# gonewest818/raytrace-clj

Measured on AMD Instinct MI355X. Metric: Msamples/sec (nx*ny*ns), higher is better.
Workload: dtype f64; 1 GPU; C3: 1920x1080x256spp Shirley cover scene n=50 (10001 spheres), depth 50, thin-lens camera, seeded counter RNG; accel=bvh; 8x8 tiles dealt round-robin to 1 GPU(s); nx=1920, ny=1080, ns=256, spheres=10001, depth=50, accel=bvh, accel_ran=bvh, frames_in_flight=1, launch_form=one GPU

## Files before the change

### include/rtmi.h

```cpp
#ifndef RTMI_H
#define RTMI_H

#include <stdint.h>

#ifdef __cplusplus
extern "C" {
#endif

#define RTMI_OK 0
#define RTMI_E_ARG (-1)
#define RTMI_E_DEVICE (-2)
#define RTMI_E_UNSUPPORTED (-3)
#define RTMI_E_NOMEM (-4)
#define RTMI_E_STATE (-5)

enum { RTMI_PRIM_SPHERE = 0, RTMI_PRIM_UVSPHERE = 1, RTMI_PRIM_MOVING = 2,
       RTMI_PRIM_RECT_XY = 3, RTMI_PRIM_RECT_XZ = 4, RTMI_PRIM_RECT_YZ = 5, RTMI_PRIM_TRIANGLE = 6,
       RTMI_PRIM_MEDIUM = 7, RTMI_PRIM_BOUNDARY = 16 };
enum { RTMI_XFORM_TRANSLATE = 0, RTMI_XFORM_ROTATE_Y = 1 };
enum { RTMI_MAT_LAMBERTIAN = 0, RTMI_MAT_METAL = 1, RTMI_MAT_DIELECTRIC = 2, RTMI_MAT_DIFFUSE_LIGHT = 3,
       RTMI_MAT_ISOTROPIC = 4  };
enum { RTMI_TEX_CONSTANT = 0, RTMI_TEX_UVGRADIENT = 1, RTMI_TEX_CHECKER = 2,
       RTMI_TEX_PERLIN_NOISE = 3, RTMI_TEX_PERLIN_TURB = 4, RTMI_TEX_MARBLE = 5, RTMI_TEX_FLIP_U = 6, RTMI_TEX_FLIP_V = 7,
       RTMI_TEX_IMAGE = 8 };
// ... 174 lines not shown
                         const double *rays, const uint64_t *keys, uint64_t seed, uint32_t ctr0, int32_t depth,
                         int32_t n_lights, const int32_t *light_prims,
                         double *state, double *out_mean, double *out_stderr, double *out_rays, uint64_t *out_counters);
int rtmi_render_rays_nee_device(rtmi_scene *scene, int32_t precision, int32_t n_groups, int32_t group, int32_t g_first,
                                const void *d_rays, const void *d_keys, uint64_t seed, uint32_t ctr0, int32_t depth,
                                int32_t n_lights, const int32_t *light_prims,
                                void *d_state, void *d_out_mean, void *d_out_stderr, void *d_out_rays, void *d_out_counters, void *stream);
int rtmi_probe_paths_nee(rtmi_scene *scene, int32_t precision, int32_t n, const double *rays, const uint64_t *keys, uint64_t ctr0, int32_t depth,
                         int32_t n_lights, const int32_t *light_prims, double *out_rgb, uint64_t *out_nseg, int32_t *out_dropped,
                         double *log, int32_t max_seg, int32_t *out_nlog);

#define RTMI_MIS_REC 28
int rtmi_render_rays_mis(rtmi_scene *scene, int32_t precision, int32_t n_groups, int32_t group, int32_t g_first,
                         const double *rays, const uint64_t *keys, uint64_t seed, uint32_t ctr0, int32_t depth,
                         int32_t n_lights, const int32_t *light_prims, int32_t light_choice,
                         double *state, double *out_mean, double *out_stderr, double *out_rays, uint64_t *out_counters);
int rtmi_render_rays_mis_device(rtmi_scene *scene, int32_t precision, int32_t n_groups, int32_t group, int32_t g_first,
                                const void *d_rays, const void *d_keys, uint64_t seed, uint32_t ctr0, int32_t depth,
                                int32_t n_lights, const int32_t *light_prims, int32_t light_choice,
                                void *d_state, void *d_out_mean, void *d_out_stderr, void *d_out_rays, void *d_out_counters, void *stream);
int rtmi_probe_paths_mis(rtmi_scene *scene, int32_t precision, int32_t n, const double *rays, const uint64_t *keys, uint64_t ctr0, int32_t depth,
                         int32_t n_lights, const int32_t *light_prims, int32_t light_choice, double *out_rgb, uint64_t *out_nseg, double *out_weight,
                         double *log, int32_t max_seg, int32_t *out_nlog);

int rtmi_assemble_device(rtmi_ctx *ctx, int32_t nx, int32_t ny, int32_t world, int32_t tiles_per_rank,
                         const void *d_gathered, void *d_out_linear, void *d_out_rgb8, void *stream);

#define RTMI_PROG_REC 5
int rtmi_render_adaptive_tiles_device(rtmi_scene *scene, int32_t nx, int32_t ny, int32_t s_first, int32_t s_count,
                                      int32_t retire, double eps, int32_t depth, uint64_t seed, int32_t precision,
                                      int32_t tile_first, int32_t tile_stride, void *d_tiles_rec, void *d_out_counters, void *stream);
int rtmi_assemble_progressive_device(rtmi_ctx *ctx, int32_t nx, int32_t ny, int32_t world, int32_t tiles_per_rank,
                                     const void *d_gathered_rec, void *d_out_linear, void *d_out_rgb8, void *d_out_stderr, void *d_out_samples, void *stream);

int rtmi_scene_clone(rtmi_scene *scene, rtmi_ctx *ctx, rtmi_scene **out_scene);
int rtmi_render_multi(int32_t n, rtmi_scene *const *scenes, int32_t nx, int32_t ny, int32_t ns, int32_t depth, uint64_t seed,
                      int32_t precision, double *out_linear, uint8_t *out_rgb8, uint64_t *out_counters);
int rtmi_render_multi_device(int32_t n, rtmi_scene *const *scenes, int32_t nx, int32_t ny, int32_t ns, int32_t depth, uint64_t seed,
                             int32_t precision, void *d_out_linear, void *d_out_rgb8, void *d_out_counters);
int rtmi_render_multi_adaptive(int32_t n, rtmi_scene *const *scenes, int32_t nx, int32_t ny, int32_t s_first, int32_t s_count,
                               int32_t retire, double eps, int32_t depth, uint64_t seed, int32_t precision,
                               double *out_linear, uint8_t *out_rgb8, double *out_stderr, int32_t *out_samples, uint64_t *out_counters);
int rtmi_render_multi_adaptive_device(int32_t n, rtmi_scene *const *scenes, int32_t nx, int32_t ny, int32_t s_first, int32_t s_count,
                                      int32_t retire, double eps, int32_t depth, uint64_t seed, int32_t precision,
                                      void *d_out_linear, void *d_out_rgb8, void *d_out_stderr, void *d_out_samples, void *d_out_counters);
enum { RTMI_GATHER_NONE = 0,
       RTMI_GATHER_SAME_DEVICE = 1,
       RTMI_GATHER_PEER_COPY = 2,
       RTMI_GATHER_RCCL = 3 };
int rtmi_last_gather_path(rtmi_ctx *ctx0, int32_t *path);
int rtmi_rccl_probe(const char *soname);
int rtmi_stream_idle(rtmi_ctx *ctx, int32_t *idle);
int rtmi_last_passes(rtmi_ctx *ctx, int32_t *passes);
int rtmi_last_accel(rtmi_ctx *ctx, int32_t *accel);
int rtmi_last_gather_ms(rtmi_ctx *ctx0, double *ms);

int rtmi_last_traversal_counters(rtmi_ctx *ctx, uint64_t *out_aabb_tests, uint64_t *out_prim_tests);

int rtmi_last_trace_ms(rtmi_ctx *ctx, double *ms, int32_t *launches);
int rtmi_last_reduce_ms(rtmi_ctx *ctx, double *ms, int32_t *launches);

int rtmi_probe_hit(rtmi_scene *scene, int32_t precision, int32_t n, const double *rays, double t_min, double t_max, double *out);
int rtmi_probe_paths(rtmi_scene *scene, int32_t precision, int32_t n, const double *rays, const uint64_t *keys, uint64_t ctr0,
                     int32_t depth, double *out_rgb, uint64_t *out_nseg, double *log, int32_t max_seg, int32_t *out_nlog);
int rtmi_probe_camera(rtmi_scene *scene, int32_t precision, int32_t n, const double *uv, const uint64_t *keys, double *out);
int rtmi_probe_texture(rtmi_scene *scene, int32_t precision, int32_t tex, int32_t n, const double *uvp, double *out);
int rtmi_probe_scatter(rtmi_scene *scene, int32_t precision, int32_t mat, int32_t n, const double *rays, const double *hits,
                       const uint64_t *keys, double *out);
int rtmi_probe_rng(rtmi_ctx *ctx, int32_t precision, uint64_t key, uint64_t d0, int32_t n, uint64_t *out_bits, double *out_real);
uint64_t rtmi_sample_key(uint64_t seed, uint64_t pixel, uint64_t sample);
int rtmi_probe_arith(rtmi_ctx *ctx, int32_t n, const double *abc, double *out);
#define RTMI_PROBE_MATH_SLOTS 12
int rtmi_probe_math2(rtmi_ctx *ctx, int32_t n, const double *abc, double tmin, double tmax, int32_t n_slots, double *out);
int rtmi_probe_math(rtmi_ctx *ctx, int32_t n, const double *abc, double tmin, double tmax, double *out);

int rtmi_test_build_tree(int32_t n, const double *geom, const double *cam, int32_t threads, uint64_t *out_hash, int32_t *out_info, double *out_ms);
int rtmi_test_camera_fixed(int32_t cam_kind, const double *cam);
int rtmi_test_half_outward(double x, int32_t up);
int rtmi_test_pack_materials(int32_t n_prims, const int32_t *prim_kind, const double *prim_geom, const int32_t *prim_mat,
                             int32_t n_mats, const int32_t *mat_kind, const int32_t *mat_tex, const double *mat_param,
                             int32_t n_tex, const int32_t *tex_kind, const double *tex_param, const int32_t *tex_child,
                             int32_t cam_kind, const double *cam, const int32_t *prim_flip, const int32_t *prim_xform,
                             int32_t n_xforms, const int32_t *xform_kind, const double *xform_param, int32_t through_creation,
                             uint64_t *out_hash, int32_t *out_facts);
int rtmi_test_pack_geometry(int32_t n_prims, const int32_t *prim_kind, const double *prim_geom, const int32_t *prim_mat,
                            int32_t n_mats, const int32_t *mat_kind, const int32_t *mat_tex, const double *mat_param,
                            int32_t n_tex, const int32_t *tex_kind, const double *tex_param, const int32_t *tex_child,
                            int32_t cam_kind, const double *cam, const int32_t *prim_flip, const int32_t *prim_xform,
                            int32_t n_xforms, const int32_t *xform_kind, const double *xform_param, int32_t through_creation, uint64_t *out_hash);
int rtmi_test_refit(int32_t n_prims, const int32_t *prim_kind, const int32_t *prim_flip, const int32_t *prim_xform, int32_t n_xforms, const int32_t *xform_kind,
                    int32_t cam_kind, const double *cam, int32_t n_steps, const double *geoms, const double *xforms,
                    void *out_nodes, int64_t capacity, int64_t *out_bytes, int32_t *out_info, int32_t *out_big,
                    int32_t *out_cells, int64_t cells_capacity, void *out_leaf_box);
int rtmi_test_refit_half(double x, int32_t up);
int rtmi_test_scene_nodes(rtmi_scene *scene, void *buf, int64_t capacity, int64_t *out_bytes);
int rtmi_test_stage_layout(int32_t n, const uint64_t *elem_bytes, const uint64_t *counts, const int32_t *present, uint64_t *out_offsets, uint64_t *out_total);

#ifdef __cplusplus
}
#endif
#endif
```

### raytrace_clj_amd/_ffi.py

```python
import ctypes as C
import os

import numpy as np

try:
    import torch
except ImportError:
    torch = None

_HERE = os.path.dirname(os.path.abspath(__file__))
LIB_PATH = os.environ.get("RTMI_LIB") or os.path.join(_HERE, "lib", "librtmi.so")

SYMBOLS = [
    "rtmi_last_error", "rtmi_backend_name", "rtmi_version", "rtmi_init", "rtmi_shutdown", "rtmi_set_option",
    "rtmi_device_info", "rtmi_scene_create", "rtmi_scene_create_ex", "rtmi_scene_set_perlin", "rtmi_scene_set_images", "rtmi_scene_set_media_calls", "rtmi_scene_set_media_mode", "rtmi_scene_set_media_calls_narrowed", "rtmi_scene_device_bytes", "rtmi_scene_destroy", "rtmi_render", "rtmi_render_device",
    "rtmi_render_tiles_device", "rtmi_local_tiles", "rtmi_assemble_device", "rtmi_last_trace_ms", "rtmi_last_reduce_ms", "rtmi_probe_hit",
    "rtmi_probe_paths", "rtmi_probe_camera", "rtmi_probe_texture", "rtmi_probe_scatter", "rtmi_probe_rng",
    "rtmi_sample_key", "rtmi_test_half_outward", "rtmi_test_camera_fixed", "rtmi_test_build_tree", "rtmi_probe_arith", "rtmi_probe_math", "rtmi_probe_math2", "rtmi_last_traversal_counters",
    "rtmi_scene_clone", "rtmi_render_multi", "rtmi_render_multi_device", "rtmi_last_gather_ms",
    "rtmi_last_gather_path", "rtmi_rccl_probe", "rtmi_stream_idle", "rtmi_last_passes", "rtmi_last_accel",
    "rtmi_render_progressive", "rtmi_render_progressive_device", "rtmi_progressive_samples", "rtmi_progressive_release",
    "rtmi_render_adaptive", "rtmi_render_adaptive_device", "rtmi_adaptive_status", "rtmi_adaptive_active_tiles",
    "rtmi_render_features", "rtmi_render_features_device", "rtmi_denoise", "rtmi_denoise_device",
    "rtmi_adaptive_retire", "rtmi_adaptive_retire_device",
    "rtmi_render_adaptive_tiles_device", "rtmi_assemble_progressive_device", "rtmi_render_multi_adaptive", "rtmi_render_multi_adaptive_device",
    "rtmi_scene_set_camera", "rtmi_scene_set_camera_stream", "rtmi_scene_camera",
    "rtmi_reproject", "rtmi_reproject_device",
    "rtmi_scene_tree_info",
    "rtmi_scene_set_materials", "rtmi_scene_set_materials_stream", "rtmi_test_pack_materials",
    "rtmi_scene_set_geometry", "rtmi_scene_last_refit_ms", "rtmi_test_pack_geometry", "rtmi_test_refit", "rtmi_test_refit_half", "rtmi_test_scene_nodes",
    "rtmi_render_rays", "rtmi_render_rays_device",
    "rtmi_test_stage_layout",
    "rtmi_query_hits", "rtmi_query_hits_device", "rtmi_query_occluded", "rtmi_query_occluded_device",
    "rtmi_occlusion_hemisphere", "rtmi_occlusion_hemisphere_device", "rtmi_occlusion_targets", "rtmi_occlusion_targets_device",
    "rtmi_ambient_occlusion", "rtmi_ambient_occlusion_device",
    "rtmi_scene_lights", "rtmi_test_scene_lights", "rtmi_direct_irradiance", "rtmi_direct_irradiance_device", "rtmi_render_direct", "rtmi_render_direct_device",
    "rtmi_render_rays_nee", "rtmi_render_rays_nee_device", "rtmi_probe_paths_nee",
    "rtmi_render_rays_mis", "rtmi_render_rays_mis_device", "rtmi_probe_paths_mis",
]

F64, F32 = 0, 1
ACCEL_FLAT, ACCEL_BVH = 0, 1
FLAG_TIMING = 1
GATHER_PATHS = {0: "none", 1: "same-device", 2: "peer-copy", 3: "rccl"}
SEG_REC = 12
TILE = 8
PROG_REC = 5
FEATURES = 8
HIT_REC = 12
RAYS_REC = 10
DIRECT_REC = 4
NEE_REC = 24
MIS_REC = 28
DIRECT_MAX_LIGHTS = 32
EDIT_STREAM_MAX_BYTES = 32768


class RtmiError(RuntimeError):
    def __init__(self, code, msg):
        super().__init__("rtmi error %d: %s" % (code, msg))
        self.code = code


_lib = None


def lib():
    global _lib
    if _lib is not None:
        return _lib
    if not os.path.exists(LIB_PATH):
        raise RtmiError(-2, "HIP extension %s is missing; build it with `make -C raytrace_clj_amd/csrc` "
                            "(there is no CPU fallback)" % LIB_PATH)
    L = C.CDLL(LIB_PATH)
    vp, i32, i64, u64, dbl = C.c_void_p, C.c_int32, C.c_int64, C.c_uint64, C.c_double
    L.rtmi_last_error.restype = C.c_char_p
    L.rtmi_backend_name.restype = C.c_char_p
    L.rtmi_version.restype = C.c_int
    L.rtmi_init.argtypes = [C.c_int, C.c_uint32, C.POINTER(vp)]
    L.rtmi_shutdown.argtypes = [vp]
    L.rtmi_set_option.argtypes = [vp, C.c_char_p, i64]
    L.rtmi_device_info.argtypes = [vp, C.POINTER(i32), C.POINTER(i32), C.POINTER(i64), C.c_char_p, i32]
    L.rtmi_scene_create.argtypes = [vp, i32, vp, vp, vp, i32, vp, vp, vp, i32, vp, vp, vp, i32, vp, C.POINTER(vp)]
    L.rtmi_scene_create_ex.argtypes = [vp, i32, vp, vp, vp, i32, vp, vp, vp, i32, vp, vp, vp, i32, vp, vp, vp, i32, vp, vp, C.POINTER(vp)]
    L.rtmi_scene_set_perlin.argtypes = [vp, vp, vp]
    L.rtmi_scene_set_images.argtypes = [vp, i32, vp, vp]
    L.rtmi_scene_set_media_calls.argtypes = [vp, i32, vp]
    L.rtmi_scene_set_media_mode.argtypes = [vp, i32]
    L.rtmi_scene_set_media_calls_narrowed.argtypes = [vp, i32, vp, vp]
    L.rtmi_scene_device_bytes.argtypes = [vp, C.POINTER(C.c_int64)]
    L.rtmi_scene_destroy.argtypes = [vp]
    L.rtmi_render.argtypes = [vp, i32, i32, i32, i32, u64, i32, i32, i32, i32, i32, vp, vp, vp]
    L.rtmi_render_device.argtypes = [vp, i32, i32, i32, i32, u64, i32, vp, vp, vp, vp]
    L.rtmi_render_tiles_device.argtypes = [vp, i32, i32, i32, i32, u64, i32, i32, i32, vp, vp, vp]
    L.rtmi_local_tiles.argtypes = [i32, i32, i32, i32]
    L.rtmi_local_tiles.restype = i32
    L.rtmi_assemble_device.argtypes = [vp, i32, i32, i32, i32, vp, vp, vp, vp]
    L.rtmi_last_trace_ms.argtypes = [vp, C.POINTER(dbl), C.POINTER(i32)]
    L.rtmi_last_reduce_ms.argtypes = [vp, C.POINTER(dbl), C.POINTER(i32)]
    L.rtmi_probe_hit.argtypes = [vp, i32, i32, vp, dbl, dbl, vp]
    L.rtmi_probe_paths.argtypes = [vp, i32, i32, vp, vp, u64, i32, vp, vp, vp, i32, vp]
    L.rtmi_probe_camera.argtypes = [vp, i32, i32, vp, vp, vp]
    L.rtmi_probe_texture.argtypes = [vp, i32, i32, i32, vp, vp]
    L.rtmi_probe_scatter.argtypes = [vp, i32, i32, i32, vp, vp, vp, vp]
    L.rtmi_probe_rng.argtypes = [vp, i32, u64, u64, i32, vp, vp]
    L.rtmi_sample_key.argtypes = [u64, u64, u64]
    L.rtmi_sample_key.restype = u64
    L.rtmi_probe_arith.argtypes = [vp, i32, vp, vp]
    L.rtmi_test_build_tree.argtypes = [i32, vp, vp, i32, vp, vp, vp]
    L.rtmi_test_half_outward.argtypes = [C.c_double, i32]
    L.rtmi_test_camera_fixed.argtypes = [i32, vp]
    L.rtmi_probe_math.argtypes = [vp, i32, vp, C.c_double, C.c_double, vp]
    L.rtmi_probe_math2.argtypes = [vp, i32, vp, C.c_double, C.c_double, i32, vp]
    L.rtmi_last_traversal_counters.argtypes = [vp, C.POINTER(u64), C.POINTER(u64)]
    L.rtmi_scene_clone.argtypes = [vp, vp, C.POINTER(vp)]
    L.rtmi_render_multi.argtypes = [i32, C.POINTER(vp), i32, i32, i32, i32, u64, i32, vp, vp, vp]
    L.rtmi_render_multi_device.argtypes = [i32, C.POINTER(vp), i32, i32, i32, i32, u64, i32, vp, vp, vp]
    L.rtmi_last_gather_ms.argtypes = [vp, C.POINTER(dbl)]
    L.rtmi_last_gather_path.argtypes = [vp, C.POINTER(i32)]
    L.rtmi_rccl_probe.argtypes = [C.c_char_p]
    L.rtmi_stream_idle.argtypes = [vp, C.POINTER(i32)]
    L.rtmi_last_passes.argtypes = [vp, C.POINTER(i32)]
    L.rtmi_last_accel.argtypes = [vp, C.POINTER(i32)]
    L.rtmi_render_progressive.argtypes = [vp, i32, i32, i32, i32, i32, u64, i32, i32, i32, i32, i32, vp, vp, vp, vp]
    L.rtmi_render_progressive_device.argtypes = [vp, i32, i32, i32, i32, i32, u64, i32, vp, vp, vp, vp, vp]
    L.rtmi_progressive_samples.argtypes = [vp, C.POINTER(i32)]
    L.rtmi_progressive_release.argtypes = [vp]
    L.rtmi_render_adaptive.argtypes = [vp, i32, i32, i32, i32, dbl, i32, u64, i32, i32, i32, i32, i32, vp, vp, vp, vp, vp]
    L.rtmi_render_adaptive_device.argtypes = [vp, i32, i32, i32, i32, dbl, i32, u64, i32, vp, vp, vp, vp, vp, vp]
    L.rtmi_adaptive_status.argtypes = [vp, C.POINTER(i32), C.POINTER(i32), C.POINTER(i64)]
    L.rtmi_adaptive_active_tiles.argtypes = [vp, i32, vp, C.POINTER(i32)]
    L.rtmi_adaptive_retire.argtypes = [vp, i32, i32, vp, dbl, C.POINTER(i32)]
    L.rtmi_adaptive_retire_device.argtypes = [vp, i32, i32, vp, dbl, C.POINTER(i32), vp]
    L.rtmi_render_features.argtypes =[vp, i32, i32, i32, u64, i32, i32, i32, i32, i32, vp, vp]
    L.rtmi_render_features_device.argtypes = [vp, i32, i32, i32, u64, i32, vp, vp, vp]
    L.rtmi_denoise.argtypes = [vp, i32, i32, vp, vp, vp, i32, dbl, dbl, dbl, dbl, vp, vp, vp]
    L.rtmi_denoise_device.argtypes = [vp, i32, i32, vp, vp, vp, i32, dbl, dbl, dbl, dbl, vp, vp, vp, vp]
    L.rtmi_render_adaptive_tiles_device.argtypes = [vp, i32, i32, i32, i32, i32, dbl, i32, u64, i32, i32, i32, vp, vp, vp]
    L.rtmi_assemble_progressive_device.argtypes = [vp, i32, i32, i32, i32, vp, vp, vp, vp, vp, vp]
    L.rtmi_render_multi_adaptive.argtypes = [i32, C.POINTER(vp), i32, i32, i32, i32, i32, dbl, i32, u64, i32, vp, vp, vp, vp, vp]
    L.rtmi_render_multi_adaptive_device.argtypes = [i32, C.POINTER(vp), i32, i32, i32, i32, i32, dbl, i32, u64, i32, vp, vp, vp, vp, vp]
    L.rtmi_scene_set_camera.argtypes = [vp, i32, vp, C.POINTER(i32)]
    L.rtmi_scene_set_camera_stream.argtypes = [vp, i32, vp, vp]
    L.rtmi_scene_camera.argtypes = [vp, C.POINTER(i32), vp, C.POINTER(dbl), C.POINTER(dbl)]
    L.rtmi_scene_tree_info.argtypes = [vp, vp]
    L.rtmi_scene_set_materials.argtypes = [vp, i32, vp, vp, vp, i32, vp, vp, vp, vp, C.POINTER(i32)]
    L.rtmi_scene_set_materials_stream.argtypes = [vp, i32, vp, vp, vp, i32, vp, vp, vp, vp, vp]
    L.rtmi_test_pack_materials.argtypes = [i32, vp, vp, vp, i32, vp, vp, vp, i32, vp, vp, vp, i32, vp, vp, vp, i32, vp, vp, i32, vp, vp]
    L.rtmi_scene_set_geometry.argtypes = [vp, i32, vp, i32, vp, i32, vp]
    L.rtmi_scene_last_refit_ms.argtypes = [vp, C.POINTER(dbl)]
    L.rtmi_test_pack_geometry.argtypes = [i32, vp, vp, vp, i32, vp, vp, vp, i32, vp, vp, vp, i32, vp, vp, vp, i32, vp, vp, i32, vp]
    L.rtmi_test_refit.argtypes = [i32, vp, vp, vp, i32, vp, i32, vp, i32, vp, vp, vp, i64, vp, vp, vp, vp, i64, vp]
    L.rtmi_test_refit_half.argtypes = [C.c_double, i32]
    L.rtmi_test_scene_nodes.argtypes = [vp, vp, i64, C.POINTER(i64)]
    L.rtmi_reproject.argtypes = [vp, i32, i32, i32, vp, i32, vp] + [vp] * 7 + [dbl] * 5 + [vp] * 5
    L.rtmi_reproject_device.argtypes = [vp, i32, i32, i32, vp, i32, vp] + [vp] * 7 + [dbl] * 5 + [vp] * 6
    L.rtmi_render_rays.argtypes = [vp, i32, i32, i32, i32, vp, vp, u64, C.c_uint32, i32, vp, vp, vp, vp, vp]
    L.rtmi_render_rays_device.argtypes = [vp, i32, i32, i32, i32, vp, vp, u64, C.c_uint32, i32, vp, vp, vp, vp, vp, vp]
    L.rtmi_test_stage_layout.argtypes = [i32, vp, vp, vp, vp, vp]
    L.rtmi_query_hits.argtypes = [vp, i32, i32, vp, vp, dbl, dbl, vp, C.c_uint32, vp, vp]
    L.rtmi_query_hits_device.argtypes = [vp, i32, i32, vp, vp, dbl, dbl, vp, C.c_uint32, vp, vp, vp]
    L.rtmi_query_occluded.argtypes = [vp, i32, i32, i32, vp, vp, dbl, dbl, vp, C.c_uint32, vp, vp, vp]
    L.rtmi_query_occluded_device.argtypes = [vp, i32, i32, i32, vp, vp, dbl, dbl, vp, C.c_uint32, vp, vp, vp, vp]
    L.rtmi_occlusion_hemisphere.argtypes = [vp, i32, i32, vp, vp, i32, i32, u64, dbl, dbl, dbl, vp, vp, vp, vp]
    L.rtmi_occlusion_hemisphere_device.argtypes = [vp, i32, i32, vp, vp, i32, i32, u64, dbl, dbl, dbl, vp, vp, vp, vp, vp]
    L.rtmi_occlusion_targets.argtypes = [vp, i32, i32, vp, vp, i32, vp, dbl, dbl, dbl, vp, vp, vp, vp]
    L.rtmi_occlusion_targets_device.argtypes = [vp, i32, i32, vp, vp, i32, vp, dbl, dbl, dbl, vp, vp, vp, vp, vp]
    L.rtmi_ambient_occlusion.argtypes = [vp, i32, i32, i32, i32, i32, dbl, u64, vp, vp, vp, vp]
    L.rtmi_ambient_occlusion_device.argtypes = [vp, i32, i32, i32, i32, i32, dbl, u64, vp, vp, vp, vp, vp]
    L.rtmi_scene_lights.argtypes = [vp, i32, vp, vp]
    L.rtmi_test_scene_lights.argtypes = [i32, vp, vp, vp, i32, vp, vp, i32, vp, vp, i32, vp, vp]
    L.rtmi_direct_irradiance.argtypes = [vp, i32, i32, vp, vp, i32, vp, i32, i32, u64, dbl, i32, vp, vp, vp, vp, vp, vp]
    L.rtmi_direct_irradiance_device.argtypes = [vp, i32, i32, vp, vp, i32, vp, i32, i32, u64, dbl, i32, vp, vp, vp, vp, vp, vp, vp]
    L.rtmi_render_direct.argtypes = [vp, i32, i32, i32, i32, i32, u64, vp, vp, vp, vp, vp]
    L.rtmi_render_direct_device.argtypes = [vp, i32, i32, i32, i32, i32, u64, vp, vp, vp, vp, vp, vp]
# ... 30 lines not shown
```

### raytrace_clj_amd/csrc/rtmi.hip

```cpp
#include <hip/hip_runtime.h>
#include <rccl/rccl.h>
#include <dlfcn.h>

#include <algorithm>
#include <atomic>
#include <chrono>
#include <condition_variable>
#include <functional>
#include <thread>
#include <cmath>
#include <cmath>
#include <cstdarg>
#include <cstdio>
#include <cstdlib>
#include <cstring>
#include <array>
#include <map>
#include <mutex>
#include <new>
#include <string>
#include <vector>

#include "rtmi.h"
#include "rtmi_device.h"

using namespace rtmi;

#define RTMI_EXPORT extern "C" __attribute__((visibility("default")))

namespace {

constexpr int kBlock = RTMI_TRACE_BLOCK;
constexpr int kTraceBlock = RTMI_TRACE_BLOCK;
#ifdef RTMI_STAMPS
__device__ unsigned long long g_wg_t[2][4096];
__device__ inline unsigned long long real_now() { unsigned long long t; asm volatile("s_memrealtime %0\n\ts_waitcnt lgkmcnt(0)" : "=s"(t)::"memory"); return t; }
#define RTMI_STAMP_DECL const unsigned long long st_wg0 = real_now(); \
    if (lane == 0) for (int k_ = 0; k_ < 3 * PH_SLOTS + 2; ++k_) g_ph[threadIdx.x >> 6][k_] = 0; \
    ph_stamp(-1); for (int k_ = 0; k_ < 32; ++k_) ph_stamp(PH_CAL);
#define RTMI_STAMP_FLUSH(cnt) if (lane == 0) for (int k_ = 0; k_ < 3 * PH_SLOTS; ++k_) if (g_ph[threadIdx.x >> 6][k_]) atomicAdd(&g_phase[k_], g_ph[threadIdx.x >> 6][k_]); \
    __syncthreads(); if (threadIdx.x == 0 && blockIdx.x < 4096) { g_wg_t[0][blockIdx.x] = st_wg0; g_wg_t[1][blockIdx.x] = real_now(); }
#else
#define RTMI_STAMP_DECL
#define RTMI_STAMP_FLUSH(cnt)
#endif
#ifndef RTMI_MIN_WAVES
#define RTMI_MIN_WAVES 4
#endif
#ifndef RTMI_EXT_MIN_WAVES
#define RTMI_EXT_MIN_WAVES RTMI_MIN_WAVES
#endif

struct TraceParams {
    int nx, ny, depth;
    u64 seed;
    int tiles_x;
    int n_local_tiles;
    const int *tile_ids;
    int s_begin, s_count;
    void *samples;
    u64 *counters;
    int prims_per_tile;
    int n_ptiles;
    unsigned *queue;
    unsigned total_items;
    unsigned qblock;
    int suspend_lanes;
    int rx0, ry0, rx1, ry1;
    u64 *trav;
    int susp_off;
    int stash_off;
    double rnx, rny;
    int fixed_rays;
};
#ifndef RTMI_QUEUE_BLOCK
#define RTMI_QUEUE_BLOCK 256
#endif
#ifndef RTMI_EXT_NO_STASH
#define RTMI_EXT_NO_STASH 0
#endif
#ifndef RTMI_EXT_LDS_STASH
#define RTMI_EXT_LDS_STASH 1
#endif
#ifndef RTMI_STASH
#define RTMI_STASH 1
#endif
constexpr unsigned kQueueBlock = RTMI_QUEUE_BLOCK;

template <typename R> __device__ inline const R *stat4_of(SceneRef sc);
template <typename R> __device__ inline void stage_prims(SceneRef sc, Prim4<R> *lds, int first, int count) {
    for (int i = threadIdx.x; i < count; i += blockDim.x) {
        const R *g = stat4_of<R>(sc) + (size_t)(first + i) * 4;
        Prim4<R> p;
        p.cx = g[0]; p.cy = g[1]; p.cz = g[2]; p.r2 = g[3];
        lds[i] = p;
    }
}

template <typename R> __device__ inline const R *stat4_of(SceneRef sc);
template <> __device__ inline const double *stat4_of<double>(SceneRef sc) { return sc.stat4_d; }
template <> __device__ inline const float *stat4_of<float>(SceneRef sc) { return sc.stat4_f; }

template <bool ANY = false>
__device__ inline void scan_cull_dispatch(SceneRef sc, const Path<double> &P, double a, double tmin, double &best_t, int &best_i) {
    scan_all_cull<ANY>(sc, P, a, tmin, best_t, best_i);
}
template <bool ANY = false>
__device__ inline void scan_cull_dispatch(SceneRef sc, const Path<float> &P, float a, float tmin, float &best_t, int &best_i) {
    scan_static_pipe<float, false, ANY>(ScalarPrims<float>(sc.stat4_f), sc.n_static, 0, P, a, tmin, best_t, best_i);
    if (best_i >= 0) best_i = sc.stat_orig[best_i];
    if (ANY && best_i >= 0) return;
    if (sc.n_moving > 0) {
        int best_orig = best_i >= 0 ? best_i : 0x7fffffff, scan_i = -1;
        scan_moving<float>(sc, P, a, tmin, best_t, scan_i, best_orig);
        if (scan_i >= 0) best_i = best_orig;
    }
}


template <bool SLICED = false, bool COUNT = false, int MSEQ = 0, bool ANY = false>
__device__ inline void intersect_ext(SceneRef sc, int *stack, bool bvh, Path<double> &P, bool active, double tmin, double tmax, double &best_t, int &best_i,
                                     bool *mid = nullptr, int min_lanes = 0, unsigned *cnt = nullptr, int susp_off = RTMI_BVH_STACK * RTMI_BVH_STRIDE) {
    best_t = tmax; best_i = -1;
    if (!active) return;
    const double a = dot3(P.dx, P.dy, P.dz, P.dx, P.dy, P.dz);
    ExtHit H = {tmax, 0x7fffffff, -1};
    if (MSEQ == 2) {
        MediumChord chord = medium_chord_begin(P);
        ExtHit Hrun = {tmax, 0x7fffffff, -1};
        int cur_lo = -1, scanned_to = 0;
        for (int k = 0; k < sc.n_media; ++k) {
            const int m = sc.media_idx[k], lo = sc.media_lo[k];
            if (lo >= m) { ext_medium_test(sc, m, P, tmin, tmax, H, chord, COUNT ? cnt : nullptr); continue; }
            if (lo != cur_lo) { Hrun.t = tmax; Hrun.F = 0x7fffffff; Hrun.W = -1; cur_lo = lo; scanned_to = lo; }
            if (m > scanned_to) scan_all_cull_ext(sc, P, a, tmin, Hrun, scanned_to, m);
            double tm = 0.0;
            if (ext_medium_test(sc, m, P, tmin, Hrun.any() ? Hrun.t : tmax, Hrun, chord, COUNT ? cnt : nullptr, &tm)) ext_update(H, tm, m, true);
            scanned_to = m + 1;
        }
        if (bvh) scan_bvh_ext<false, COUNT>(sc, stack, P, a, tmin, H, nullptr, false, 0, cnt);
// ... 90 lines not shown
            int best_orig = best_i >= 0 ? best_i : 0x7fffffff, scan_i = -1;
            scan_moving<R>(sc, P, a, tmin, best_t, scan_i, best_orig);
            if (scan_i >= 0) best_i = best_orig;
        }
    }
}

template <typename R> __device__ inline void start_sample(SceneRef sc, const TraceParams &tp, int i, int j, int s, Path<R> &P) {
    seed_stream(P, sample_key(tp.seed, (u64)j * (u64)tp.nx + (u64)i, (u64)s), 0u);
    const R u = ((R)(float)i + next_uniform(P)) / (R)tp.nx;
    const R v = ((R)(float)j + next_uniform(P)) / (R)tp.ny;
    RTMI_PH(PH_GEN_KEY)
    get_ray<R>(sc, u, v, P);
    P.ar = P.ag = P.ab = R(1);
    P.depth = tp.depth;
}

__device__ inline double pixel_quot(double x, int n, double rn) { return div_const(x, (double)n, rn); }
__device__ inline float pixel_quot(float x, int n, double) { return x / (float)n; }

#ifndef RTMI_GEN_PLAIN
#define RTMI_GEN_PLAIN 0
#endif
struct GenTile { int tile, x0, y0; u64 hpix; };
template <typename R, bool KEEP> __device__ inline bool generate_camera_rays(SceneRef sc, const TraceParams &tp, unsigned chunk, int lane, GenTile &g, Path<R> &Q) {
    const int tile_local = (int)(chunk / (unsigned)tp.s_count);
    const int s = tp.s_begin + (int)(chunk - (unsigned)tile_local * (unsigned)tp.s_count);
#if RTMI_GEN_PLAIN
    const int gtile = tp.tile_ids[tile_local];
    const int x = (gtile % tp.tiles_x) * RTMI_TILE + (lane & 7), y = (gtile / tp.tiles_x) * RTMI_TILE + (lane >> 3);
    const bool has = x >= tp.rx0 && x < tp.rx1 && y >= tp.ry0 && y < tp.ry1;
    if (has) start_sample<R>(sc, tp, x, tp.ny - 1 - y, s, Q);
    return has;
#else
    if (!KEEP || tile_local != g.tile) {
        const int gtile = tp.tile_ids[tile_local];
        g.x0 = (gtile % tp.tiles_x) * RTMI_TILE; g.y0 = (gtile / tp.tiles_x) * RTMI_TILE;
        const int i = g.x0 + (lane & 7), j = tp.ny - 1 - (g.y0 + (lane >> 3));
        g.hpix = mix64(tp.seed ^ (RTMI_GOLD * ((u64)j * (u64)tp.nx + (u64)i + 1)));
        g.tile = tile_local;
    }
    const int x = g.x0 + (lane & 7), y = g.y0 + (lane >> 3), j = tp.ny - 1 - y;
    const bool has = x >= tp.rx0 && x < tp.rx1 && y >= tp.ry0 && y < tp.ry1;
    seed_stream(Q, mix64(g.hpix + 0xD1B54A32D192ED03ULL * ((u64)s + 1)), 0u);
    const R ju = next_uniform(Q), jv = next_uniform(Q);
    const R u = pixel_quot((R)(float)x + ju, tp.nx, tp.rnx);
    const R v = pixel_quot((R)(float)j + jv, tp.ny, tp.rny);
    RTMI_PH(PH_GEN_KEY)
    get_ray_wave<R>(sc, tp.fixed_rays != 0, has, u, v, Q);
    return has;
#endif
}

template <typename R, bool MULTI, int VARIANT, bool EXT = false, bool COUNT = false, bool SLICE = true, int MSEQ = 0, bool LST = false>
__global__ void __launch_bounds__(kTraceBlock, EXT ? ((MSEQ != 0 || COUNT) ? 3 : RTMI_EXT_MIN_WAVES) : RTMI_MIN_WAVES) trace_kernel(ScenePtr scp, TraceParams tp) {
    SceneRef sc = *scp;
    extern __shared__ __attribute__((aligned(16))) char smem[];
    Prim4<R> *lds = reinterpret_cast<Prim4<R> *>(smem);
    const int lane = threadIdx.x & 63;
    if (!MULTI && VARIANT < SCAN_SGPR) stage_prims<R>(sc, lds, 0, sc.n_static);
    __syncthreads();

    const unsigned total_items = tp.total_items;
    unsigned w_cur = 0, w_end = 0;
    Path<R> P;
    P.ox = P.oy = P.oz = P.dx = P.dy = P.dz = P.time = R(0);
    P.ar = P.ag = P.ab = R(0);
    seed_stream(P, 0ull, 0u); P.depth = 0;
    bool alive = false;
    bool exhausted = (total_items == 0);
    unsigned out_item = 0;
    constexpr bool LSTASH = (EXT && RTMI_STASH && RTMI_EXT_LDS_STASH && !RTMI_EXT_NO_STASH) || LST;
    constexpr bool STASH = RTMI_STASH && !(EXT && RTMI_EXT_NO_STASH) && !LSTASH;
    int *const lst = reinterpret_cast<int *>(smem) + tp.stash_off + (threadIdx.x & ~63);
    R st_ox = R(0), st_oy = R(0), st_oz = R(0), st_dx = R(0), st_dy = R(0), st_dz = R(0), st_time = R(0);
    u64 st_rs = 0;
    unsigned st_item = 0xffffffffu;
    unsigned s_head = 64u;
    constexpr bool KEEP = LST;
    GenTile gen = {-1, 0, 0, 0ull};
    unsigned nrays = 0;
    unsigned ntrav[2] = {0u, 0u};
    const R tmin = R(0.001), tmax = Real<R>::tmax();
    constexpr bool SLICED = SLICE && VARIANT == SCAN_BVH && !MULTI;
    bool mid = false;

    RTMI_STAMP_DECL
    for (;;) {
        RTMI_PH(PH_LOOP)
        if (LSTASH) {
        for (;;) {
            const u64 dead = __ballot(!alive);
            if (dead == 0) break;
            if (s_head == 64u) {
                if (exhausted) break;
                if (w_cur == w_end) {
                    unsigned base = 0;
                    if (lane == 0) base = atomicAdd(tp.queue, tp.qblock);
                    base = __builtin_amdgcn_readfirstlane(base);
                    if (base >= total_items) { exhausted = true; break; }
                    w_cur = base;
                    w_end = min(base + tp.qblock, total_items);
                }
                const unsigned m = w_cur + (unsigned)lane;
                Path<R> Q;
                const bool has = generate_camera_rays<R, KEEP>(sc, tp, w_cur >> 6, lane, gen, Q);
                w_cur += 64u;
// ... 76 lines not shown
            const unsigned f_item = __shfl(st_item, src);
            if (take && f_item != 0xffffffffu) {
                P.ox = f_ox; P.oy = f_oy; P.oz = f_oz; P.dx = f_dx; P.dy = f_dy; P.dz = f_dz; P.time = f_time; P.rs = f_rs;
                P.ar = P.ag = P.ab = R(1);
                P.depth = tp.depth;
                out_item = f_item;
                alive = true;
            }
            s_head += min(nd, avail);
        }
        } else
        while (!exhausted) {
            const u64 dead = __ballot(!alive);
            if (dead == 0) break;
            if (w_cur == w_end) {
                unsigned base = 0;
                if (lane == 0) base = atomicAdd(tp.queue, kQueueBlock);
                base = __builtin_amdgcn_readfirstlane(base);
                if (base >= total_items) { exhausted = true; break; }
                w_cur = base;
                w_end = min(base + kQueueBlock, total_items);
            }
            const unsigned avail = w_end - w_cur;
            const unsigned rank = (unsigned)__popcll(dead & ((1ull << lane) - 1ull));
            if (!alive && rank < avail) {
                const unsigned m = w_cur + rank;
                const unsigned chunk = m >> 6;
                const int l = (int)(m & 63u);
                const int tile_local = (int)(chunk / (unsigned)tp.s_count);
                const int s = tp.s_begin + (int)(chunk - (unsigned)tile_local * (unsigned)tp.s_count);
                const int gtile = tp.tile_ids[tile_local];
                const int x = (gtile % tp.tiles_x) * RTMI_TILE + (l & 7);
                const int y = (gtile / tp.tiles_x) * RTMI_TILE + (l >> 3);
                if (x >= tp.rx0 && x < tp.rx1 && y >= tp.ry0 && y < tp.ry1) {
                    start_sample<R>(sc, tp, x, tp.ny - 1 - y, s, P);
                    out_item = m;
                    alive = true;
                }
            }
            w_cur += min((unsigned)__popcll(dead), avail);
        }
        if (MULTI) { if (!__syncthreads_or(alive ? 1 : 0)) break; }
        else { if (!__any(alive ? 1 : 0)) break; }
        RTMI_PH(PH_REFILL_DEAL)

        R best_t; int best_i;
        intersect_world<R, MULTI, VARIANT, EXT, COUNT, SLICED, MSEQ, !SLICED>(sc, lds, tp.prims_per_tile, tp.n_ptiles, P, alive, tmin, tmax, best_t, best_i, ntrav,
                                                                     &mid, exhausted ? 0 : tp.suspend_lanes, (EXT || LST) ? tp.susp_off : RTMI_BVH_STACK * RTMI_BVH_STRIDE);
        RTMI_PH(PH_BVH_POST)
        if (!SLICED || __any(alive && !mid)) {
        if (alive) {
            if (!mid) ++nrays;
            R emit[3];
            const bool scat = shade_segment<R, EXT>(sc, P, best_t, best_i, nullptr, emit, mid);
            if (!mid && !scat) {
                R *out = reinterpret_cast<R *>(tp.samples) + (size_t)out_item * 3;
                out[0] = emit[0]; out[1] = emit[1]; out[2] = emit[2];
                alive = false;
                RTMI_PH(PH_STORE)
            }
        }
        }
        RTMI_PH(PH_STORE)
    }
    RTMI_STAMP_FLUSH(tp.counters)
    unsigned n = nrays;
    for (int off = 32; off > 0; off >>= 1) n += __shfl_down(n, off);
    if (lane == 0 && n) atomicAdd(tp.counters, (u64)n);
    if (COUNT) {
        u64 a = ntrav[0], b = ntrav[1];
        for (int off = 32; off > 0; off >>= 1) { a += __shfl_down(a, off); b += __shfl_down(b, off); }
        if (lane == 0) { atomicAdd(tp.trav, a); atomicAdd(tp.trav + 1, b); }
    }
}

template <typename R>
__global__ void __launch_bounds__(kBlock) reduce_kernel(const R *__restrict__ samples, R *__restrict__ accum, double *__restrict__ tiles_linear,
                                                        const int *__restrict__ tile_ids, int tiles_x, int nx, int ny, int n_local_tiles,
                                                        int s_begin, int s_count, int ns, u64 *counters, u64 n_valid_pixels,
                                                        int rx0, int ry0, int rx1, int ry1) {
    const long long gid = (long long)blockIdx.x * blockDim.x + threadIdx.x;
    if (gid == 0 && counters && s_begin + s_count >= ns) counters[1] = n_valid_pixels;
    if (gid >= (long long)n_local_tiles * 64) return;
    const int tile_local = (int)(gid >> 6), l = (int)(gid & 63);
    const int gtile = tile_ids[tile_local];
    const int tx = (gtile % tiles_x) * RTMI_TILE, ty = (gtile / tiles_x) * RTMI_TILE;
    R acc[3];
    bool valid[3];
    const size_t tile_base = (size_t)tile_local * 192;
#pragma unroll
    for (int k = 0; k < 3; ++k) {
        const int p = (l + 64 * k) / 3;
        const int x = tx + (p & 7), y = ty + (p >> 3);
        valid[k] = x >= rx0 && x < rx1 && y >= ry0 && y < ry1;
        acc[k] = (valid[k] && s_begin > 0) ? accum[tile_base + l + 64 * k] : R(0);
    }
    const R *row = samples + (size_t)tile_local * s_count * 192 + l;
    for (int s = 0; s < s_count; ++s, row += 192) {
        const R v0 = row[0], v1 = row[64], v2 = row[128];
        if (s_begin + s == 0) { acc[0] = v0; acc[1] = v1; acc[2] = v2; }
        else { acc[0] = acc[0] + v0; acc[1] = acc[1] + v1; acc[2] = acc[2] + v2; }
    }
#pragma unroll
    for (int k = 0; k < 3; ++k) {
        const size_t o = tile_base + l + 64 * k;
        if (s_begin + s_count < ns) accum[o] = valid[k] ? acc[k] : R(0);
        else tiles_linear[o] = valid[k] ? (double)(acc[k] * (R(1.0) / (R)ns)) : 0.0;
    }
}

template <typename R>
__global__ void __launch_bounds__(kBlock) assemble_kernel(const double *__restrict__ gathered, int world, size_t rank_stride, int tiles_x,
                                                          int nx, int ny, double *__restrict__ out_linear, unsigned char *__restrict__ out_rgb8) {
    const long long gid = (long long)blockIdx.x * blockDim.x + threadIdx.x;
    if (gid >= (long long)nx * ny) return;
    const int x = (int)(gid % nx), y = (int)(gid / nx);
    const int gtile = (y / RTMI_TILE) * tiles_x + (x / RTMI_TILE);
    const int r = gtile % world, k = gtile / world;
    const int l = (y % RTMI_TILE) * RTMI_TILE + (x % RTMI_TILE);
    const double *p = gathered + (size_t)r * rank_stride + ((size_t)k * 64 + l) * 3;
    for (int c = 0; c < 3; ++c) {
        const double m = p[c];
        if (out_linear) out_linear[gid * 3 + c] = m;
        if (out_rgb8) {
            const R q = Real<R>::sqrt_((R)m) * R(255.99);
            unsigned char o = 0;
            if (q == q) { const R mq = q < R(255.99) ? q : R(255.99); o = (unsigned char)(int)mq; }
            out_rgb8[gid * 3 + c] = o;
        }
    }
}

template <typename R>
__global__ void __launch_bounds__(kBlock) assemble_region_kernel(const double *__restrict__ tiles, int tx0, int ty0, int wtx, int x0, int y0, int w, int h,
                                                                 double *__restrict__ out_linear, unsigned char *__restrict__ out_rgb8) {
    const long long gid = (long long)blockIdx.x * blockDim.x + threadIdx.x;
    if (gid >= (long long)w * h) return;
    const int x = x0 + (int)(gid % w), y = y0 + (int)(gid / w);
    const int k = (y / RTMI_TILE - ty0) * wtx + (x / RTMI_TILE - tx0);
    const int l = (y % RTMI_TILE) * RTMI_TILE + (x % RTMI_TILE);
    const double *p = tiles + ((size_t)k * 64 + l) * 3;
    for (int c = 0; c < 3; ++c) {
        const double m = p[c];
        if (out_linear) out_linear[gid * 3 + c] = m;
        if (out_rgb8) {
            const R q = Real<R>::sqrt_((R)m) * R(255.99);
            unsigned char o = 0;
            if (q == q) { const R mq = q < R(255.99) ? q : R(255.99); o = (unsigned char)(int)mq; }
            out_rgb8[gid * 3 + c] = o;
        }
    }
}

__global__ void sum_counters_kernel(const u64 *gathered, int world, size_t rank_stride_u64, size_t off_u64, u64 *out) {
    if (threadIdx.x < 2) {
        u64 acc = 0;
        for (int r = 0; r < world; ++r) acc += gathered[(size_t)r * rank_stride_u64 + off_u64 + threadIdx.x];
        out[threadIdx.x] = acc;
// ... 118 lines not shown
}

}

#include "scene_build.h"

namespace {

thread_local std::string g_err;

int fail(int code, const char *fmt, ...) {
    char buf[512];
    va_list ap;
    va_start(ap, fmt);
    vsnprintf(buf, sizeof buf, fmt, ap);
    va_end(ap);
    g_err = buf;
    return code;
}

#define HIP_TRY(expr)                                                                      \
    do {                                                                                   \
        hipError_t e_ = (expr);                                                            \
        if (e_ != hipSuccess) return fail(RTMI_E_DEVICE, "%s: %s", #expr, hipGetErrorString(e_)); \
    } while (0)

struct DeviceGuard {
    int prev = -1;
    DeviceGuard() { if (hipGetDevice(&prev) != hipSuccess) prev = -1; }
    ~DeviceGuard() { if (prev >= 0) (void)hipSetDevice(prev); }
};

struct DevBuf {
    void *p = nullptr;
    size_t bytes = 0;
    int ensure(size_t need) {
        if (need <= bytes) return RTMI_OK;
        if (p) { (void)hipFree(p); p = nullptr; bytes = 0; }
        if (hipMalloc(&p, need) != hipSuccess) { p = nullptr; return fail(RTMI_E_NOMEM, "hipMalloc(%zu bytes) failed", need); }
        bytes = need;
        return RTMI_OK;
    }
    void release() { if (p) (void)hipFree(p); p = nullptr; bytes = 0; }
};


struct FoldRetire {
    const int *act_slots = nullptr;
    int last = 0;
    double eps = 0.0;
    int *keep = nullptr, *n_t = nullptr;
};

template <typename R, bool RETIRE>
__global__ void __launch_bounds__(kBlock) frame_fold_kernel(const R *__restrict__ samples, R *__restrict__ sums, double *__restrict__ mean,
                                                            double *__restrict__ m2, const int *__restrict__ tiles, int tiles_x, int n_entries, int s_begin,
                                                            int s_count, u64 *counters, u64 n_valid_pixels, int rx0, int ry0, int rx1, int ry1, FoldRetire rt) {
    const long long gid = (long long)blockIdx.x * blockDim.x + threadIdx.x;
    if (gid == 0) counters[1] = n_valid_pixels;
    if (gid >= (long long)n_entries * 64) return;
    const int entry = (int)(gid >> 6), l = (int)(gid & 63);
    const int gtile = tiles[entry];
    int slot = entry;
    if constexpr (RETIRE) slot = rt.act_slots[entry];
    const int tx = (gtile % tiles_x) * RTMI_TILE, ty = (gtile / tiles_x) * RTMI_TILE;
    R acc[3];
    double mu[3], q[3];
    bool valid[3];
    const size_t tile_base = (size_t)slot * 192;
#pragma unroll
    for (int k = 0; k < 3; ++k) {
        const int p = (l + 64 * k) / 3;
        const int x = tx + (p & 7), y = ty + (p >> 3);
        valid[k] = x >= rx0 && x < rx1 && y >= ry0 && y < ry1;
        const bool carry = valid[k] && s_begin > 0;
        const size_t o = tile_base + l + 64 * k;
        acc[k] = carry ? sums[o] : R(0);
        mu[k] = carry ? mean[o] : 0.0;
        q[k] = carry ? m2[o] : 0.0;
    }
    const R *row = samples + (size_t)entry * s_count * 192 + l;
    for (int s = 0; s < s_count; ++s, row += 192) {
        const R v[3] = {row[0], row[64], row[128]};
        if (s_begin + s == 0) {
#pragma unroll
            for (int k = 0; k < 3; ++k) { acc[k] = v[k]; mu[k] = (double)v[k]; q[k] = 0.0; }
        } else {
            const double n = (double)(s_begin + s + 1);
#pragma unroll
            for (int k = 0; k < 3; ++k) {
                acc[k] = acc[k] + v[k];
                const double x = (double)v[k], d = x - mu[k];
                mu[k] = mu[k] + d / n;
                q[k] = q[k] + d * (x - mu[k]);
            }
        }
    }
#pragma unroll
    for (int k = 0; k < 3; ++k) {
        const size_t o = tile_base + l + 64 * k;
        sums[o] = valid[k] ? acc[k] : R(0);
        mean[o] = valid[k] ? mu[k] : 0.0;
        m2[o] = valid[k] ? q[k] : 0.0;
    }
    if constexpr (RETIRE) {
        if (!rt.last) return;
        const int kk = s_begin + s_count;
        bool noisy = false;
        if (kk > 1) {
#pragma unroll
            for (int k = 0; k < 3; ++k) {
                const double se = ::sqrt((q[k] / (double)(kk - 1)) / (double)kk);
                noisy = noisy || (valid[k] && !(se <= rt.eps));
            }
        }
        const u64 any = __ballot(noisy);
        if (l == 0) { rt.keep[entry] = (kk < 2 || any != 0ull) ? 1 : 0; rt.n_t[slot] = kk; }
    }
}

struct PixelEstimate { double m[3], err; int k; };
template <typename R>
__device__ inline PixelEstimate pixel_estimate(const R *__restrict__ sums, const double *__restrict__ m2, size_t e, int k) {
    PixelEstimate p;
    p.k = k;
    p.err = k > 1 ? 0.0 : INFINITY;
    for (int c = 0; c < 3; ++c) {
        p.m[c] = (double)(sums[e + c] * (R(1.0) / (R)k));
        if (k > 1) {
            const double se = ::sqrt((m2[e + c] / (double)(k - 1)) / (double)k);
            p.err = se > p.err ? se : p.err;
        }
    }
    return p;
}

__device__ inline unsigned char quantise8(double m) {
    const double q = Real<double>::sqrt_(m) * 255.99;
    unsigned char o = 0;
    if (q == q) { const double mq = q < 255.99 ? q : 255.99; o = (unsigned char)(int)mq; }
    return o;
}

template <typename R>
__global__ void __launch_bounds__(kBlock) frame_resolve_kernel(const R *__restrict__ sums, const double *__restrict__ m2, const int *__restrict__ n_t,
                                                               int k_uniform, int tx0, int ty0, int wtx, int x0, int y0, int w, int h,
                                                               double *__restrict__ out_linear, unsigned char *__restrict__ out_rgb8,
                                                               double *__restrict__ out_stderr, int *__restrict__ out_samples) {
    const long long gid = (long long)blockIdx.x * blockDim.x + threadIdx.x;
    if (gid >= (long long)w * h) return;
    const int x = x0 + (int)(gid % w), y = y0 + (int)(gid / w);
    const int t = (y / RTMI_TILE - ty0) * wtx + (x / RTMI_TILE - tx0);
    const int l = (y % RTMI_TILE) * RTMI_TILE + (x % RTMI_TILE);
// ... 1086 lines not shown
    int first = 0, stride = 1;
};

struct ProgFrame {
    DevBuf sums, mean, m2, counters;
    DevBuf act_tiles[2], act_slots[2], n_t, keep, meta;
    ProgKey key;
    int k = 0;
    bool adaptive = false;
    int cur = 0, n_tiles = 0, n_active = 0;
    long long valid_pixels = 0, active_pixels = 0, pixel_samples = 0;
    int *meta_host = nullptr;
    bool meta_pending = false;
    void release() {
        sums.release(); mean.release(); m2.release(); counters.release();
        for (int i = 0; i < 2; ++i) { act_tiles[i].release(); act_slots[i].release(); }
        n_t.release(); keep.release(); meta.release();
        if (meta_host) (void)hipHostFree(meta_host);
        meta_host = nullptr; meta_pending = false;
        k = 0; adaptive = false; cur = n_tiles = n_active = 0; valid_pixels = active_pixels = pixel_samples = 0;
    }
};

struct AdaptiveCall {
    double eps = 0.0;
    int k_before = 0;
};

}

struct rtmi_ctx {
    uint32_t magic = 0x52544d49u;
    int device = 0;
    uint32_t flags = 0;
    hipStream_t stream = nullptr;
    int cus = 0;
    int lds_per_cu = 0;
    size_t hbm = 0;
    std::string arch;
    int blocks_per_cu = 8;
    int64_t workspace_bytes = (int64_t)64 << 30;
    int accel = RTMI_ACCEL_BVH;
    int scan_variant = SCAN_SGPR_CULL;
    int max_lds_bytes = 64 * 1024 - 64;
    DevBuf samples, accum, tiles, tile_ids, counters;
    DevBuf io;
    DevBuf multi;
    hipEvent_t ev_done = nullptr, ev_g0 = nullptr, ev_g1 = nullptr;
    bool have_gather = false;
    int last_gather_path = RTMI_GATHER_NONE;
    hipEvent_t ev_consumed = nullptr;
    int ev_consumed_device = -1;
    bool consume_pending = false;
    int fail_next_render = 0;
    int fail_allocs = 0;
    int last_accel = -1;
    int last_passes = 0;
    int last_grid = 0;
    std::map<std::pair<const void *, size_t>, int> occupancy;
    std::vector<int> tile_ids_host;
    int tile_key[8] = {-1, -1, -1, -1, -1, -1, -1, -1};
    std::vector<hipEvent_t> events_r;
    double last_reduce_ms = 0.0;
    int last_reduce_launches = 0;
    int count_traversal = 0;
    int flat_below = 24;
    bool suspend_lanes_set = false;
    int suspend_lanes = 8;
    hipStream_t last_stream = nullptr;
    long long tile_valid_pixels = 0;
    ProgFrame prog;
    DevBuf feat_cnt;
    DevBuf dn_planes;
    DevBuf rays_ws;
    DevBuf occ_ws;
    DevBuf nee_ws;
    DevBuf direct_ws;
    std::vector<std::pair<hipEvent_t, hipEvent_t>> events;
    int events_used = 0;
};

struct rtmi_scene {
    uint32_t magic = 0x52545343u;
    rtmi_ctx *ctx = nullptr;
    DevScene dev{};
    ScenePtr d_dev = nullptr;
    std::vector<void *> allocs;
    std::vector<void *> table_allocs;
    size_t table_bytes = 0;
    size_t device_bytes = 0;
    int n_prims = 0, n_mats = 0, n_tex = 0;
    int bvh_node_count = 0;
    int bvh_depth = 0;
    bool uses_perlin = false;
    int max_image = -1;
    bool have_perlin = false;
    uint64_t serial = 0;
    uint64_t revision = 0;
    std::vector<int> host_kind;
    bool has_moving = false;
    std::map<int, std::array<double, 5>> media_fast_of;
    PackedMaterials mat;
    bool geom_ext = false;
    TreeBuild tree;
    struct GeoEdit {
        bool ready = false;
        PackedScene tab;
        GeomExtras X;
        std::vector<char> displaced;
        std::vector<int> level_off;
// ... 103 lines not shown
    *e1 = nullptr;
    if (!(c->flags & RTMI_FLAG_TIMING) || c->events_used >= 8192) return RTMI_OK;
    const int rc = next_event_pair(c, &e0, e1);
    if (rc) return rc;
    HIP_TRY(hipEventRecord(e0, st));
    return RTMI_OK;
}
int close_timed_fold(rtmi_ctx *c, hipStream_t st) {
    const size_t k = (size_t)c->events_used - 1;
    while (c->events_r.size() <= k) { hipEvent_t e; HIP_TRY(hipEventCreate(&e)); c->events_r.push_back(e); }
    HIP_TRY(hipEventRecord(c->events_r[k], st));
    return RTMI_OK;
}

int resident_blocks(rtmi_ctx *c, const void *kern, int block, size_t lds_bytes, int *resident) {
    const std::pair<const void *, size_t> key(kern, lds_bytes);
    auto it = c->occupancy.find(key);
    if (it == c->occupancy.end()) {
        HIP_TRY(hipOccupancyMaxActiveBlocksPerMultiprocessor(resident, kern, block, lds_bytes));
        c->occupancy.emplace(key, *resident);
    } else *resident = it->second;
    return RTMI_OK;
}

struct NoFold { void operator()() const {} };
template <typename Launch, typename Fold = NoFold>
int queue_launch(rtmi_ctx *c, hipStream_t st, const void *kern, size_t lds, unsigned *queue, long long items, Launch launch, Fold fold = Fold{}) {
    int resident = 0;
    const int rc = resident_blocks(c, kern, kBlock, lds, &resident);
    if (rc) return rc;
    const long long persistent = (long long)c->cus * std::max(1, std::min(c->blocks_per_cu, resident));
    const long long per_wave = items / std::max(1, c->cus * 16);
    unsigned qb = 64u;
    while (qb < 1024u && per_wave >= (long long)qb * 16) qb *= 2;
    hipEvent_t e1 = nullptr;
    const int rce = open_timed(c, st, &e1);
    if (rce) return rce;
    HIP_TRY(hipMemsetAsync(queue, 0, sizeof(unsigned), st));
    launch(dim3((unsigned)std::max<long long>(1, std::min<long long>(persistent, (items + kBlock - 1) / kBlock))), (unsigned)items, qb);
    HIP_TRY(hipGetLastError());
    if (e1) HIP_TRY(hipEventRecord(e1, st));
    fold();
    HIP_TRY(hipGetLastError());
    return e1 ? close_timed_fold(c, st) : RTMI_OK;
}

hipStream_t stream_of(const rtmi_ctx *c, void *stream) { return stream ? reinterpret_cast<hipStream_t>(stream) : c->stream; }

int check_region(int nx, int ny, int x0, int y0, int x1, int y1) {
    if (x0 < 0 || y0 < 0 || x1 > nx || y1 > ny || x1 <= x0 || y1 <= y0) return fail(RTMI_E_ARG, "region [%d,%d)x[%d,%d) outside %dx%d", x0, x1, y0, y1, nx, ny);
    return RTMI_OK;
}

struct LaunchKnobs { const char *flat_below, *suspend_lanes, *sphere_stash; };
LaunchKnobs read_launch_knobs() { return {std::getenv("RTMI_FLAT_BELOW"), std::getenv("RTMI_SUSPEND_LANES"), std::getenv("RTMI_SPHERE_LDS_STASH")}; }

struct LdsLayout { int susp_off, stash_off; size_t bytes; };
LdsLayout lds_layout(int levels, int susp_words, int stash_words) {
    return {levels * RTMI_BVH_STRIDE, (levels + susp_words) * RTMI_BVH_STRIDE, (size_t)(levels + susp_words + stash_words) * kTraceBlock * sizeof(int)};
}

struct TracePlan {
    void (*kern)(ScenePtr, TraceParams) = nullptr;
    LdsLayout lds{RTMI_BVH_STACK * RTMI_BVH_STRIDE, 0, 0};
    int suspend_lanes = 0;
    int accel = RTMI_ACCEL_BVH;
};

template <typename R>
TracePlan choose_trace_kernel(const rtmi_scene *s, const rtmi_ctx *c, const LaunchKnobs &k, bool multi, size_t lds_bytes) {
    const DevScene &d = s->dev;
    TracePlan p;
    int variant = c->accel == RTMI_ACCEL_BVH ? SCAN_BVH : c->scan_variant;
    const int below = k.flat_below ? std::atoi(k.flat_below) : c->flat_below;
    if (variant == SCAN_BVH && d.has_ext && !c->count_traversal && d.n_all < below) variant = SCAN_SGPR_CULL;
    p.accel = variant == SCAN_BVH ? RTMI_ACCEL_BVH : RTMI_ACCEL_FLAT;
    const bool bvh = variant == SCAN_BVH, count = c->count_traversal != 0;
    p.suspend_lanes = c->suspend_lanes;
    if (d.has_ext && !c->suspend_lanes_set) p.suspend_lanes = 12;
    if (k.suspend_lanes) p.suspend_lanes = std::max(0, std::min(64, std::atoi(k.suspend_lanes)));
    const int levels = std::max(4, std::min(RTMI_BVH_STACK, s->bvh_depth + 2));
    const int stash_words = d.cam_fixed_origin ? 11 : 17;
    constexpr bool kExtLdsStash = RTMI_STASH && RTMI_EXT_LDS_STASH && !RTMI_EXT_NO_STASH;
    if (d.has_ext && d.media_seq) {
        const bool nar = d.media_seq == 2;
        if (bvh && nar) p.kern = count ? trace_kernel<double, false, SCAN_BVH, true, true, false, 2> : trace_kernel<double, false, SCAN_BVH, true, false, false, 2>;
        else if (bvh) p.kern = count ? trace_kernel<double, false, SCAN_BVH, true, true, false, 1> : trace_kernel<double, false, SCAN_BVH, true, false, false, 1>;
        else p.kern = nar ? trace_kernel<double, false, SCAN_SGPR_CULL, true, false, true, 2> : trace_kernel<double, false, SCAN_SGPR_CULL, true, false, true, 1>;
        p.lds = lds_layout(bvh ? levels : 0, 0, kExtLdsStash ? stash_words : 0);
    } else if (d.has_ext) {
        const bool slice = bvh && s->bvh_node_count >= 128 && p.suspend_lanes > 0;
        if (bvh && count) p.kern = slice ? trace_kernel<double, false, SCAN_BVH, true, true> : trace_kernel<double, false, SCAN_BVH, true, true, false>;
        else if (bvh) p.kern = slice ? trace_kernel<double, false, SCAN_BVH, true> : trace_kernel<double, false, SCAN_BVH, true, false, false>;
        else p.kern = trace_kernel<double, false, SCAN_SGPR_CULL, true>;
        p.lds = lds_layout(bvh ? levels : 0, slice ? RTMI_BVH_SUSPEND_WORDS_EXT : 0, kExtLdsStash ? stash_words : 0);
    } else if (bvh) {
        const bool slice = (p.suspend_lanes > 0 && s->bvh_node_count >= 128) || d.grid_n > 0;
        p.lds.bytes = (size_t)(RTMI_BVH_STACK + RTMI_BVH_SUSPEND_WORDS) * kTraceBlock * sizeof(int);
        const LdsLayout stash = lds_layout(levels, RTMI_BVH_SUSPEND_WORDS, stash_words);
        if (slice) p.kern = count ? trace_kernel<R, false, SCAN_BVH, false, true> : trace_kernel<R, false, SCAN_BVH>;
        else p.kern = count ? trace_kernel<R, false, SCAN_BVH, false, true, false> : trace_kernel<R, false, SCAN_BVH, false, false, false>;
        if (slice && !count && !(k.sphere_stash && k.sphere_stash[0] == '0') && stash.bytes <= 40 * 1024) { p.kern = trace_kernel<R, false, SCAN_BVH, false, false, true, false, true>; p.lds = stash; }
    } else if (variant == SCAN_SGPR_CULL) p.kern = trace_kernel<R, false, SCAN_SGPR_CULL>;
    else if (variant == SCAN_SGPR) p.kern = trace_kernel<R, false, SCAN_SGPR>;
    else {
        p.kern = variant == SCAN_LDS_PIPE ? (multi ? trace_kernel<R, true, SCAN_LDS_PIPE> : trace_kernel<R, false, SCAN_LDS_PIPE>)
                                          : (multi ? trace_kernel<R, true, SCAN_LDS_LITERAL> : trace_kernel<R, false, SCAN_LDS_LITERAL>);
        p.lds.bytes = lds_bytes;
    }
    return p;
}

#ifdef RTMI_STAMPS
int report_phase_stamps(rtmi_ctx *c, hipStream_t st) {
    const int grid_trace_dbg = c->last_grid;
    HIP_TRY(hipStreamSynchronize(st));
    unsigned long long h[3 * PH_SLOTS] = {0}, z[3 * PH_SLOTS] = {0};
    HIP_TRY(hipMemcpyFromSymbol(h, HIP_SYMBOL(g_phase), sizeof(h)));
    HIP_TRY(hipMemcpyToSymbol(HIP_SYMBOL(g_phase), z, sizeof(z)));
    {
        static unsigned long long wt[2][4096];
        HIP_TRY(hipMemcpyFromSymbol(wt, HIP_SYMBOL(g_wg_t), sizeof(wt)));
        const int g = std::min(4096, grid_trace_dbg);
        unsigned long long t0 = ~0ull; for (int k = 0; k < g; ++k) t0 = std::min(t0, wt[0][k]);
        std::vector<double> e(g), b(g); for (int k = 0; k < g; ++k) { e[k] = (wt[1][k] - t0) * 1e-5; b[k] = (wt[0][k] - t0) * 1e-5; }
        std::sort(e.begin(), e.end()); std::sort(b.begin(), b.end());
        fprintf(stderr, "[stamps] workgroup start (ms after first): median %.3f max %.3f | end: min %.3f p10 %.3f median %.3f p90 %.3f max %.3f (last pass, %d workgroups)\n",
                b[g / 2], b[g - 1], e[0], e[g / 10], e[g / 2], e[g * 9 / 10], e[g - 1], g);
    }
    static const char *names[PH_N] = {"loop/tail", "refill: generate (stash write)", "refill: claim + deal", "bvh: ray setup / resume", "bvh: big primitives (exact)",
                                      "bvh: descent (node visits)", "bvh: leaf exact tests", "bvh: loop control / park", "shade: hit record", "shade: |d| normalise",
                                      "shade: rand-in-unit-sphere", "shade: material record + directions", "shade: texture", "shade: store / rest", "shade: sphere uv", "(stamp calibration)",
                                      "bvh: grid entry / next piece of the walk", "media: chords, draws, log", "generate: key, jitter, u v", "generate: lens disk rounds",
                                      "generate: camera arithmetic"};
    const double per_stamp = h[2 * PH_SLOTS + PH_CAL] ? (double)h[PH_CAL] / (double)h[2 * PH_SLOTS + PH_CAL] : 0.0;
    double tk[PH_N], lk[PH_N], tot = 0, totl = 0, raw = 0;
    for (int k = 0; k < PH_N; ++k) {
        raw += (double)h[k];
        const double t = (double)h[k], c = std::min(t, per_stamp * (double)h[2 * PH_SLOTS + k]);
        tk[k] = k == PH_CAL ? 0.0 : t - c;
        lk[k] = t > 0 ? (double)h[PH_SLOTS + k] * (tk[k] / t) : 0.0;
        tot += tk[k]; totl += lk[k];
    }
    fprintf(stderr, "[phases] one stamp = %.0f ticks; stamps took %.1f %% of the %.4g wave-ticks of this (diagnostic) launch and are subtracted below\n", per_stamp, 100 * (raw - tot) / raw, raw);
    fprintf(stderr, "[phases] %-36s %8s %8s %10s %10s %12s\n", "phase", "ticks %", "lanes", "masked %", "useful %", "stamps");
    for (int k = 0; k < PH_N; ++k) {
        if (!h[k] || k == PH_CAL) continue;
        const double t = tk[k], l = lk[k];
        fprintf(stderr, "[phases] %-36s %8.2f %8.1f %10.2f %10.2f %12llu\n", names[k], 100 * t / tot, t > 0 ? l / t : 0.0, 100 * (64 * t - l) / (64 * tot), 100 * l / (64 * tot), h[2 * PH_SLOTS + k]);
    }
    fprintf(stderr, "[phases] %-36s %8.2f %8.1f %10.2f %10.2f   (%.4g wave-ticks)\n", "total", 100.0, totl / tot, 100 * (64 * tot - totl) / (64 * tot), 100 * totl / (64 * tot), tot);
    return RTMI_OK;
}
#endif

// ... 2 lines not shown
struct Region { int x0, y0, x1, y1; };
Region clip_region(const int *rg, int nx, int ny) { return {std::max(rg[0], 0), std::max(rg[1], 0), std::min(rg[2], nx), std::min(rg[3], ny)}; }

hipError_t launch_compact(ProgFrame &f, const int *tile_ids, int n, int init_n_t, int tiles_x, const Region &r, hipStream_t st) {
    const bool start = tile_ids != nullptr;
    const int to = start ? 0 : 1 - f.cur;
    hipLaunchKernelGGL(adaptive_compact_kernel, dim3(1), dim3(kCompactBlock), 0, st, start ? nullptr : reinterpret_cast<const int *>(f.keep.p),
                       start ? tile_ids : reinterpret_cast<const int *>(f.act_tiles[f.cur].p),
                       start ? nullptr : reinterpret_cast<const int *>(f.act_slots[f.cur].p), n, reinterpret_cast<int *>(f.act_tiles[to].p),
                       reinterpret_cast<int *>(f.act_slots[to].p), reinterpret_cast<int *>(f.meta.p), start ? init_n_t : -1,
                       start ? reinterpret_cast<int *>(f.n_t.p) : nullptr, tiles_x, r.x0, r.y0, r.x1, r.y1);
    const hipError_t e = hipGetLastError();
    if (e == hipSuccess) f.cur = to;
    return e;
}

int ensure_tile_state(ProgFrame &f, const int *tile_ids, int n_local, int k, int tiles_x, const Region &r, hipStream_t st, const char *what) {
    const size_t ints = (size_t)std::max(n_local, 1) * sizeof(int);
    int rc = RTMI_OK;
    for (int i = 0; i < 2 && !rc; ++i) { rc = f.act_tiles[i].ensure(ints); if (!rc) rc = f.act_slots[i].ensure(ints); }
    if (!rc) rc = f.n_t.ensure(ints);
    if (!rc) rc = f.keep.ensure(ints);
    if (!rc) rc = f.meta.ensure(2 * sizeof(int));
    if (rc) return rc;
    const hipError_t e = launch_compact(f, tile_ids, n_local, k, tiles_x, r, st);
    if (e != hipSuccess) return fail(RTMI_E_DEVICE, "%s: %s", what, hipGetErrorString(e));
    f.adaptive = true;
    f.n_active = n_local; f.active_pixels = f.valid_pixels;
    f.pixel_samples = f.valid_pixels * (long long)k;
    return RTMI_OK;
}

int prepare_frame(rtmi_ctx *c, ProgFrame *prog, const AdaptiveCall *ad, int n_local, int s_first, size_t real_bytes, int tiles_x, const Region &r,
                  hipStream_t st) {
    prog->k = 0;
    const size_t elems = (size_t)std::max(n_local, 1) * 192;
    if (s_first == 0) {
        int rc = prog->sums.ensure(elems * real_bytes);
        if (!rc) rc = prog->mean.ensure(elems * sizeof(double));
        if (!rc) rc = prog->m2.ensure(elems * sizeof(double));
        if (!rc) rc = prog->counters.ensure(2 * sizeof(u64));
        if (rc) return rc;
        HIP_TRY(hipMemsetAsync(prog->counters.p, 0, 2 * sizeof(u64), st));
    } else if (prog->sums.bytes < elems * real_bytes || prog->m2.bytes < elems * sizeof(double)) {
        return fail(RTMI_E_STATE, "progressive frame buffers do not match the frame");
    }
    if (s_first == 0 || !ad) prog->adaptive = false;
    prog->n_tiles = n_local; prog->valid_pixels = c->tile_valid_pixels;
    if (ad && !prog->adaptive)
        return ensure_tile_state(*prog, reinterpret_cast<const int *>(c->tile_ids.p), n_local, ad->k_before, tiles_x, r, st, "hipGetLastError()");
    return RTMI_OK;
}

int size_sample_passes(rtmi_ctx *c, int n_local, int ns, size_t real_bytes, int *out_s_per_pass) {
    const size_t per_sample = (size_t)n_local * 64 * 3 * real_bytes;
    int s_per_pass = (int)std::max<int64_t>(1, std::min<int64_t>(ns, c->workspace_bytes / (int64_t)per_sample));
    while (s_per_pass > 1 && (long long)n_local * s_per_pass * 64 >= 0xf0000000ll) s_per_pass /= 2;
    if ((long long)n_local * s_per_pass * 64 >= 0xf0000000ll) return fail(RTMI_E_ARG, "frame too large for one pass: %d tiles per rank", n_local);
    if (per_sample * (size_t)s_per_pass > c->samples.bytes) {
        constexpr double kFreeShare = 0.8;
        size_t free_b = 0, total_b = 0;
        if (hipMemGetInfo(&free_b, &total_b) == hipSuccess) {
            const double avail = kFreeShare * (double)free_b + (double)c->samples.bytes;
            const int fit = (int)std::max<double>(1.0, std::min<double>((double)s_per_pass, avail / (double)per_sample));
            s_per_pass = std::min(s_per_pass, fit);
        }
        for (;;) {
            int rc;
            if (c->fail_allocs > 0) { c->fail_allocs--; c->samples.release(); rc = fail(RTMI_E_NOMEM, "hipMalloc(%zu bytes) failed (injected by the test hook)", per_sample * (size_t)s_per_pass); }
            else rc = c->samples.ensure(per_sample * (size_t)s_per_pass);
            if (!rc) break;
            (void)hipGetLastError();
            if (s_per_pass == 1) return rc;
            s_per_pass = (s_per_pass + 1) / 2;
        }
    }
    *out_s_per_pass = s_per_pass;
    return RTMI_OK;
}

int launch_trace_pass(rtmi_scene *s, const TracePlan &plan, TraceParams &tp, int s_begin, int s_count, hipStream_t st, hipEvent_t *out_e1) {
    rtmi_ctx *c = s->ctx;
    tp.s_begin = s_begin; tp.s_count = s_count;
    hipEvent_t e1 = nullptr;
    int rc = open_timed(c, st, &e1);
    if (rc) return rc;
    tp.total_items = (unsigned)((long long)tp.n_local_tiles * s_count * 64);
    {
        const long long per_wave = (long long)tp.total_items / std::max(1, c->cus * 16);
        unsigned qb = s->dev.has_ext ? 192u : kQueueBlock;
        while (qb < 1024u && per_wave >= (long long)qb * 128) qb *= 2;
        if (const char *e = std::getenv("RTMI_QUEUE_BLOCK_RT")) qb = std::max(64, std::atoi(e) / 64 * 64);
        tp.qblock = qb;
    }
    HIP_TRY(hipMemsetAsync(tp.queue, 0, sizeof(unsigned), st));
    int resident = 0;
    rc = resident_blocks(c, reinterpret_cast<const void *>(plan.kern), kTraceBlock, plan.lds.bytes, &resident);
    if (rc) return rc;
    const int grid_trace = std::max(1, c->cus * std::max(1, std::min(c->blocks_per_cu * (256 / kTraceBlock), resident)));
    if (c->last_grid != grid_trace && std::getenv("RTMI_DEBUG"))
        fprintf(stderr, "[rtmi] trace launch: %d workgroups of %d threads (%d resident per CU by the occupancy query, cap %d), %zu B LDS each\n",
                grid_trace, kTraceBlock, resident, c->blocks_per_cu * (256 / kTraceBlock), plan.lds.bytes);
    c->last_grid = grid_trace;
    hipLaunchKernelGGL(plan.kern, dim3(grid_trace), dim3(kTraceBlock), plan.lds.bytes, st, s->d_dev, tp);
    HIP_TRY(hipGetLastError());
    if (e1) HIP_TRY(hipEventRecord(e1, st));
    *out_e1 = e1;
    return RTMI_OK;
}

template <typename R>
int launch_fold(rtmi_ctx *c, const TraceParams &tp, int ns, int s_end, void *d_tiles_linear, bool count_pixels, ProgFrame *prog, const AdaptiveCall *ad,
                hipEvent_t e1, hipStream_t st) {
    const long long npx = (long long)tp.n_local_tiles * 64;
    const dim3 grid((unsigned)((npx + kBlock - 1) / kBlock));
    const R *samples = reinterpret_cast<const R *>(c->samples.p);
    if (ad) {
        FoldRetire rt;
        rt.act_slots = reinterpret_cast<const int *>(prog->act_slots[prog->cur].p);
        rt.last = tp.s_begin + tp.s_count == s_end ? 1 : 0; rt.eps = ad->eps;
        rt.keep = reinterpret_cast<int *>(prog->keep.p); rt.n_t = reinterpret_cast<int *>(prog->n_t.p);
        hipLaunchKernelGGL((frame_fold_kernel<R, true>), grid, dim3(kBlock), 0, st, samples, reinterpret_cast<R *>(prog->sums.p),
                           reinterpret_cast<double *>(prog->mean.p), reinterpret_cast<double *>(prog->m2.p), tp.tile_ids, tp.tiles_x, tp.n_local_tiles,
                           tp.s_begin, tp.s_count, tp.counters, (u64)c->tile_valid_pixels, tp.rx0, tp.ry0, tp.rx1, tp.ry1, rt);
    } else if (prog)
        hipLaunchKernelGGL((frame_fold_kernel<R, false>), grid, dim3(kBlock), 0, st, samples, reinterpret_cast<R *>(prog->sums.p),
                           reinterpret_cast<double *>(prog->mean.p), reinterpret_cast<double *>(prog->m2.p), tp.tile_ids, tp.tiles_x, tp.n_local_tiles,
                           tp.s_begin, tp.s_count, tp.counters, (u64)c->tile_valid_pixels, tp.rx0, tp.ry0, tp.rx1, tp.ry1, FoldRetire{});
    else
        hipLaunchKernelGGL((reduce_kernel<R>), grid, dim3(kBlock), 0, st, samples, reinterpret_cast<R *>(c->accum.p),
                           reinterpret_cast<double *>(d_tiles_linear), tp.tile_ids, tp.tiles_x, tp.nx, tp.ny, tp.n_local_tiles, tp.s_begin, tp.s_count, ns,
                           count_pixels ? tp.counters : nullptr, (u64)c->tile_valid_pixels, tp.rx0, tp.ry0, tp.rx1, tp.ry1);
    HIP_TRY(hipGetLastError());
    return e1 ? close_timed_fold(c, st) : RTMI_OK;
}

template <typename R>
int render_passes(rtmi_scene *s, int nx, int ny, int s_first, int s_end, int depth, uint64_t seed, int first, int stride, const int *rg, void *d_tiles_linear,
                  void *d_counters, hipStream_t st, ProgFrame *prog, const AdaptiveCall *ad = nullptr) {
    rtmi_ctx *c = s->ctx;
    int n_local = 0;
    const int whole[4] = {0, 0, nx, ny};
    if (!rg) rg = whole;
    const Region region = clip_region(rg, nx, ny);
    int rc = ensure_tile_ids(c, nx, ny, first, stride, rg, st, &n_local);
    if (rc) return rc;
    c->last_stream = st;
    if (c->fail_next_render) { c->fail_next_render = 0; return fail(RTMI_E_DEVICE, "render failed (injected by the test hook test_fail_next_render)"); }
    if (prog) {
        rc = prepare_frame(c, prog, ad, n_local, s_first, sizeof(R), tiles_x_of(nx), region, st);
        if (rc) return rc;
        d_counters = prog->counters.p;
    }
    rc = c->counters.ensure(8 * sizeof(u64));
    if (rc) return rc;
    if (d_counters && !prog) HIP_TRY(hipMemsetAsync(d_counters, 0, 2 * sizeof(u64), st));
    HIP_TRY(hipMemsetAsync(reinterpret_cast<u64 *>(c->counters.p) + 3, 0, 2 * sizeof(u64), st));
    if (n_local == 0) { if (prog) { prog->k = s_end; c->last_passes = 0; } return RTMI_OK; }
    if (ad) n_local = prog->n_active;
    if (n_local == 0) { prog->k = s_end; c->last_passes = 0; return RTMI_OK; }

    const int ns = s_end - s_first;
    int s_per_pass = 0;
    rc = size_sample_passes(c, n_local, ns, sizeof(R), &s_per_pass);
    if (rc) return rc;
    c->last_passes = (ns + s_per_pass - 1) / s_per_pass;
    if (!prog && s_per_pass < ns) {
        rc = c->accum.ensure((size_t)n_local * 64 * 3 * sizeof(R));
        if (rc) return rc;
    }
    int ppt, nptiles;
    size_t lds_bytes;
    lds_plan(c, s->dev.n_static, sizeof(R), &ppt, &nptiles, &lds_bytes);
    const TracePlan plan = choose_trace_kernel<R>(s, c, read_launch_knobs(), nptiles > 1, lds_bytes);
    c->last_accel = plan.accel;

    TraceParams tp;
    tp.nx = nx; tp.ny = ny; tp.depth = depth; tp.seed = seed; tp.tiles_x = tiles_x_of(nx);
    tp.n_local_tiles = n_local;
    tp.tile_ids = ad ? reinterpret_cast<const int *>(prog->act_tiles[prog->cur].p) : reinterpret_cast<const int *>(c->tile_ids.p);
    tp.samples = c->samples.p;
    tp.counters = d_counters ? reinterpret_cast<u64 *>(d_counters) : reinterpret_cast<u64 *>(c->counters.p);
    tp.prims_per_tile = (c->scan_variant >= SCAN_SGPR || s->dev.has_ext) ? 0 : ppt; tp.n_ptiles = nptiles;
    tp.queue = reinterpret_cast<unsigned *>(reinterpret_cast<u64 *>(c->counters.p) + 2);
    tp.rx0 = region.x0; tp.ry0 = region.y0; tp.rx1 = region.x1; tp.ry1 = region.y1;
    tp.trav = reinterpret_cast<u64 *>(c->counters.p) + 3;
    tp.suspend_lanes = plan.suspend_lanes; tp.susp_off = plan.lds.susp_off; tp.stash_off = plan.lds.stash_off;
    tp.rnx = 1.0 / (double)nx; tp.rny = 1.0 / (double)ny; tp.fixed_rays = camera_fixed_rays(s->dev.cam_kind, s->dev.cam_fixed_origin, s->dev.cam);
    for (int s_begin = s_first; s_begin < s_end; s_begin += s_per_pass) {
        hipEvent_t e1 = nullptr;
        rc = launch_trace_pass(s, plan, tp, s_begin, std::min(s_per_pass, s_end - s_begin), st, &e1);
        if (!rc) rc = launch_fold<R>(c, tp, ns, s_end, d_tiles_linear, d_counters != nullptr, prog, ad, e1, st);
        if (rc) return rc;
    }
#ifdef RTMI_STAMPS
    rc = report_phase_stamps(c, st);
#endif
    if (!rc && ad)
        HIP_TRY(launch_compact(*prog, nullptr, n_local, -1, tiles_x_of(nx), region, st));
    if (!rc && prog) prog->k = s_end;
    return rc;
}

template <typename R>
int render_tiles_impl(rtmi_scene *s, int nx, int ny, int ns, int depth, uint64_t seed, int first, int stride, const int *rg, void *d_tiles_linear,
                      void *d_counters, hipStream_t st) {
    return render_passes<R>(s, nx, ny, 0, ns, depth, seed, first, stride, rg, d_tiles_linear, d_counters, st, nullptr);
}

int check_render_args(rtmi_scene *s, int nx, int ny, int ns, int depth, int precision) {
    if (!scene_ok(s)) return fail(RTMI_E_STATE, "invalid scene handle");
    if (nx <= 0 || ny <= 0 || ns <= 0 || depth < 0) return fail(RTMI_E_ARG, "nx, ny, ns must be > 0 and depth >= 0 (got %d %d %d %d)", nx, ny, ns, depth);
    if ((long long)nx * ny > (1ll << 30)) return fail(RTMI_E_ARG, "frame too large");
    if (precision != RTMI_F64 && precision != RTMI_F32) return fail(RTMI_E_ARG, "precision must be RTMI_F64 or RTMI_F32");
    if (precision == RTMI_F32 && s->dev.has_ext) return fail(RTMI_E_UNSUPPORTED, "rectangles / triangles / instances / procedural textures are rendered by the FP64 kernels only");
    if (s->uses_perlin && !s->have_perlin) return fail(RTMI_E_STATE, "the scene holds a Perlin texture: call rtmi_scene_set_perlin first");
    if (s->max_image >= s->dev.n_images) return fail(RTMI_E_STATE, "the scene holds an ImageMap with index %d: call rtmi_scene_set_images first", s->max_image);
    return RTMI_OK;
}

struct IoPlane { size_t elem, count; bool present; const void *up; void *down; void **dev; size_t off; };

size_t io_layout(IoPlane *pl, int n) {
    size_t at = 0;
    for (int i = 0; i < n; ++i) { pl[i].off = at; if (pl[i].present) at += (pl[i].elem * pl[i].count + 15) & ~(size_t)15; }
    return at;
}

struct HostIo {
    rtmi_ctx *c;
    IoPlane pl[16];
    int n = 0;
    explicit HostIo(rtmi_ctx *ctx) : c(ctx) {}
    template <typename T> void plane(T **dev, size_t count, bool present, const void *up, void *down) { pl[n++] = {sizeof(T), count, present, up, down, reinterpret_cast<void **>(dev), 0}; }
    template <typename T> void in(T **dev, size_t count, const void *host) { plane(dev, count, host != nullptr, host, nullptr); }
    template <typename T> void out(T **dev, size_t count, void *host) { plane(dev, count, host != nullptr, nullptr, host); }
    template <typename T> void work(T **dev, size_t count, void *host) { plane(dev, count, true, nullptr, host); }
    int reserve() {
        const int rc = c->io.ensure(io_layout(pl, n));
        for (int i = 0; i < n && !rc; ++i) *pl[i].dev = pl[i].present ? static_cast<char *>(c->io.p) + pl[i].off : nullptr;
        return rc;
    }
    hipError_t copy(bool up) const {
        hipError_t e = hipStreamSynchronize(c->stream);
        for (int i = 0; i < n && e == hipSuccess; ++i) {
// ... 89 lines not shown
    int ndev = 0;
    if (hipGetDeviceCount(&ndev) != hipSuccess || ndev <= 0) return fail(RTMI_E_DEVICE, "no HIP device visible (this library has no CPU fallback)");
    if (device < 0 || device >= ndev) return fail(RTMI_E_ARG, "device %d out of range (0..%d)", device, ndev - 1);
    HIP_TRY(hipSetDevice(device));
    hipDeviceProp_t prop;
    HIP_TRY(hipGetDeviceProperties(&prop, device));
    if (std::strncmp(prop.gcnArchName, "gfx950", 6) != 0)
        return fail(RTMI_E_DEVICE, "device %d is %s; this library carries gfx950 (MI355X) code objects only", device, prop.gcnArchName);
    rtmi_ctx *c = new (std::nothrow) rtmi_ctx();
    if (!c) return fail(RTMI_E_NOMEM, "out of host memory");
    c->device = device;
    c->flags = flags;
    c->cus = prop.multiProcessorCount;
    c->lds_per_cu = (int)prop.maxSharedMemoryPerMultiProcessor;
    c->hbm = prop.totalGlobalMem;
    c->arch = prop.gcnArchName;
    if (const char *e = std::getenv("RTMI_BLOCKS_PER_CU")) c->blocks_per_cu = std::max(1, std::atoi(e));
    if (const char *e = std::getenv("RTMI_SCAN_VARIANT")) c->scan_variant = std::min(3, std::max(0, std::atoi(e)));
    if (const char *e = std::getenv("RTMI_LDS_TILE_BYTES")) c->max_lds_bytes = std::min(64 * 1024 - 64, std::max(1024, std::atoi(e)));
    if (hipStreamCreateWithFlags(&c->stream, hipStreamNonBlocking) != hipSuccess) { delete c; return fail(RTMI_E_DEVICE, "hipStreamCreate failed"); }
    *out_ctx = c;
    return RTMI_OK;
}

RTMI_EXPORT int rtmi_shutdown(rtmi_ctx *c) {
    if (!ctx_ok(c)) return fail(RTMI_E_STATE, "invalid context handle");
    (void)hipSetDevice(c->device);
    (void)hipStreamSynchronize(c->stream);
#ifdef RTMI_HIST
    { unsigned long long h[200]; if (hipMemcpyFromSymbol(h, HIP_SYMBOL(rtmi::g_hist), sizeof h) == hipSuccess) { for (int k = 0; k < 3; ++k) { fprintf(stderr, "HIST%d", k); for (int i = 0; i <= 64; ++i) fprintf(stderr, " %llu", h[64 * k + i]); fprintf(stderr, "\n"); } } }
#endif
    c->samples.release(); c->accum.release(); c->tiles.release(); c->tile_ids.release(); c->counters.release(); c->io.release(); c->multi.release();
    c->prog.release();
    c->feat_cnt.release(); c->dn_planes.release(); c->rays_ws.release(); c->occ_ws.release(); c->direct_ws.release(); c->nee_ws.release();
    for (hipEvent_t e : {c->ev_done, c->ev_g0, c->ev_g1}) if (e) (void)hipEventDestroy(e);
    if (c->ev_consumed) { (void)hipSetDevice(c->ev_consumed_device); (void)hipEventDestroy(c->ev_consumed); (void)hipSetDevice(c->device); }
    for (auto &e : c->events) { (void)hipEventDestroy(e.first); (void)hipEventDestroy(e.second); }
    for (hipEvent_t e : c->events_r) (void)hipEventDestroy(e);
    (void)hipStreamDestroy(c->stream);
    c->magic = 0;
    delete c;
    return RTMI_OK;
}

RTMI_EXPORT int rtmi_set_option(rtmi_ctx *c, const char *name, int64_t value) {
    if (!ctx_ok(c)) return fail(RTMI_E_STATE, "invalid context handle");
    if (!name) return fail(RTMI_E_ARG, "name is NULL");
    if (!std::strcmp(name, "blocks_per_cu")) { if (value < 1 || value > 64) return fail(RTMI_E_ARG, "blocks_per_cu must be 1..64"); c->blocks_per_cu = (int)value; return RTMI_OK; }
    if (!std::strcmp(name, "workspace_bytes")) { if (value < (1 << 20)) return fail(RTMI_E_ARG, "workspace_bytes must be >= 1 MiB"); c->workspace_bytes = value; return RTMI_OK; }
    if (!std::strcmp(name, "lds_tile_bytes")) { if (value < 1024 || value > 64 * 1024 - 64) return fail(RTMI_E_ARG, "lds_tile_bytes out of range"); c->max_lds_bytes = (int)value; return RTMI_OK; }
    if (!std::strcmp(name, "timing")) { if (value) c->flags |= RTMI_FLAG_TIMING; else c->flags &= ~RTMI_FLAG_TIMING; return RTMI_OK; }
    if (!std::strcmp(name, "scan_variant")) { if (value < 0 || value > 3) return fail(RTMI_E_ARG, "scan_variant must be 0..3"); c->scan_variant = (int)value; return RTMI_OK; }
    if (!std::strcmp(name, "count_traversal")) { c->count_traversal = value ? 1 : 0; return RTMI_OK; }
    if (!std::strcmp(name, "test_fail_next_render")) { c->fail_next_render = value ? 1 : 0; return RTMI_OK; }
    if (!std::strcmp(name, "test_fail_allocs")) { c->fail_allocs = (int)std::max<int64_t>(0, std::min<int64_t>(value, 64)); return RTMI_OK; }
    if (!std::strcmp(name, "flat_below")) { if (value < 0 || value > (1 << 20)) return fail(RTMI_E_ARG, "flat_below must be 0..2^20"); c->flat_below = (int)value; return RTMI_OK; }
    if (!std::strcmp(name, "suspend_lanes")) { if (value < 0 || value > 64) return fail(RTMI_E_ARG, "suspend_lanes must be 0..64"); c->suspend_lanes = (int)value; c->suspend_lanes_set = true; return RTMI_OK; }
    if (!std::strcmp(name, "accel")) {
        if (value == RTMI_ACCEL_FLAT || value == RTMI_ACCEL_BVH) { c->accel = (int)value; return RTMI_OK; }
        return fail(RTMI_E_UNSUPPORTED, "accel %lld is not available in this build", (long long)value);
    }
    return fail(RTMI_E_ARG, "unknown option '%s'", name);
}

RTMI_EXPORT int rtmi_device_info(rtmi_ctx *c, int32_t *cus, int32_t *lds, int64_t *hbm, char *arch, int32_t arch_len) {
    if (!ctx_ok(c)) return fail(RTMI_E_STATE, "invalid context handle");
    if (cus) *cus = c->cus;
    if (lds) *lds = c->lds_per_cu;
    if (hbm) *hbm = (int64_t)c->hbm;
    if (arch && arch_len > 0) { std::strncpy(arch, c->arch.c_str(), (size_t)arch_len - 1); arch[arch_len - 1] = 0; }
    return RTMI_OK;
}

RTMI_EXPORT int rtmi_scene_create(rtmi_ctx *c, int32_t n_prims, const int32_t *prim_kind, const double *prim_geom, const int32_t *prim_mat,
                                  int32_t n_mats, const int32_t *mat_kind, const int32_t *mat_tex, const double *mat_param,
                                  int32_t n_tex, const int32_t *tex_kind, const double *tex_param, const int32_t *tex_child,
                                  int32_t cam_kind, const double *cam, rtmi_scene **out_scene) {
    return rtmi_scene_create_ex(c, n_prims, prim_kind, prim_geom, prim_mat, n_mats, mat_kind, mat_tex, mat_param, n_tex, tex_kind, tex_param, tex_child,
                                cam_kind, cam, nullptr, nullptr, 0, nullptr, nullptr, out_scene);
}

static void fill_media_fast(DevScene &d, const std::map<int, std::array<double, 5>> &media_fast_of) {
    for (int k = 0; k < 8; ++k) {
        double *q = d.media_fast[k];
        for (int j = 0; j < 8; ++j) q[j] = 0.0;
        if (k >= d.n_media) continue;
        const auto it = media_fast_of.find(d.media_idx[k]);
        if (it == media_fast_of.end()) continue;
        q[0] = 1.0;
        for (int j = 0; j < 5; ++j) q[1 + j] = it->second[(size_t)j];
    }
}
static void fill_media_fast(rtmi_scene *s) { fill_media_fast(s->dev, s->media_fast_of); }
namespace {
int check_material_tables(const SceneArrays &a) {
    const int n_mats = a.n_mats, n_tex = a.n_tex;
    const int32_t *mat_kind = a.mat_kind, *mat_tex = a.mat_tex, *tex_kind = a.tex_kind, *tex_child = a.tex_child;
    for (int t = 0; t < n_tex; ++t) {
        if (tex_kind[t] < RTMI_TEX_CONSTANT || tex_kind[t] > RTMI_TEX_IMAGE) return fail(RTMI_E_UNSUPPORTED, "texture %d: kind %d unsupported on GPU path", t, tex_kind[t]);
        if (tex_kind[t] == RTMI_TEX_FLIP_U || tex_kind[t] == RTMI_TEX_FLIP_V) {
            const int ch = tex_child[2 * t];
            if (ch < 0 || ch >= n_tex || ch == t) return fail(RTMI_E_ARG, "texture %d: wrapped texture %d invalid", t, ch);
        }
        if (tex_kind[t] == RTMI_TEX_CHECKER)
            for (int k = 0; k < 2; ++k) {
                const int ch = tex_child[2 * t + k];
// ... 359 lines not shown
constexpr int kMatTables = 11;
std::array<MatTable, kMatTables> material_tables(const PackedMaterials &M, const DevScene &d) {
    auto tab = [](const auto &v, size_t row_elems, const void *dev) { return MatTable{v.data(), v.size() * sizeof(v[0]), row_elems * sizeof(v[0]), dev}; };
    return {tab(M.mat_rec, 12, d.mat_rec), tab(M.mat_grad, 12, d.mat_grad), tab(M.mat_kind, 1, d.mat_kind), tab(M.mat_tex, 1, d.mat_tex),
            tab(M.mat_param, 1, d.mat_param), tab(M.tex_kind, 1, d.tex_kind), tab(M.tex_param, RTMI_TEX_STRIDE, d.tex_param), tab(M.tex_child, 2, d.tex_child),
            tab(M.prim_mat, 1, d.prim_mat), tab(M.prim_kind, 1, d.prim_kind), tab(M.prim_km, 2, d.prim_km)};
}

constexpr int kPatchRows = 64, kPatchWords = 704;
struct PatchRow { unsigned *dst; unsigned short src, n; unsigned pad; };
struct PatchArgs { PatchRow row[kPatchRows]; unsigned word[kPatchWords]; int n_rows, pad; };
static_assert(sizeof(PatchArgs) <= 4096, "one launch's rows fit the kernel-argument space");
static_assert(RTMI_EDIT_STREAM_MAX_BYTES % 4 == 0 && 96 / 4 <= kPatchWords, "the largest row (MatRec, a texture's parameters: twelve doubles) fits one launch");

__global__ void __launch_bounds__(64) set_materials_kernel(PatchArgs a) {
    const int l = (int)threadIdx.x;
    if (l >= a.n_rows) return;
    unsigned *dst = a.row[l].dst;
    const int src = a.row[l].src, n = a.row[l].n;
    for (int k = 0; k < n; ++k) dst[k] = a.word[src + k];
}

int check_material_arrays(int n_mats, const int32_t *mat_kind, const int32_t *mat_tex, const double *mat_param, int n_tex, const int32_t *tex_kind,
                          const double *tex_param, const int32_t *tex_child) {
    if (n_mats < 0 || n_tex < 0) return fail(RTMI_E_ARG, "negative count");
    if (n_mats > 0 && (!mat_kind || !mat_tex || !mat_param)) return fail(RTMI_E_ARG, "material arrays are NULL");
    if (n_tex > 0 && (!tex_kind || !tex_param || !tex_child)) return fail(RTMI_E_ARG, "texture arrays are NULL");
    return RTMI_OK;
}
int check_material_edit(const SceneArrays &a) {
    int rc = check_material_tables(a);
    for (int i = 0; i < a.n_prims && !rc; ++i) {
        rc = check_prim_material(a, i);
        if (!rc && (a.prim_kind[i] & ~RTMI_PRIM_BOUNDARY) == RTMI_PRIM_MEDIUM) rc = check_medium_material(a, i);
    }
    return rc;
}
bool materials_fit(const rtmi_scene *s, const SceneArrays &a, const PackedMaterials &M, std::string *why) {
    char buf[160] = "";
    const int has_ext = (s->geom_ext || M.has_ext) ? 1 : 0;
    if (a.n_mats != s->n_mats) snprintf(buf, sizeof buf, "the edit has %d materials, the scene %d", a.n_mats, s->n_mats);
    else if (a.n_tex != s->n_tex) snprintf(buf, sizeof buf, "the edit has %d textures, the scene %d", a.n_tex, s->n_tex);
    else if (has_ext != s->dev.has_ext)
        snprintf(buf, sizeof buf, "the edit %s a texture or material that only the EXT kernels hold (has_ext %d -> %d)", has_ext ? "brings in" : "removes the last use of", s->dev.has_ext, has_ext);
    else {
        const auto was = material_tables(s->mat, s->dev), now = material_tables(M, s->dev);
        for (int t = 0; t < kMatTables; ++t) if (was[(size_t)t].bytes != now[(size_t)t].bytes) snprintf(buf, sizeof buf, "table %d changes its size", t);
    }
    if (why) *why = buf;
    return buf[0] == 0;
}
void adopt_materials(rtmi_scene *s, const SceneArrays &a, PackedMaterials *M) {
    rtmi_scene::Args &A = s->args;
    if (M) { s->uses_perlin = M->uses_perlin; s->max_image = M->max_image; s->mat = std::move(*M); }
    if (a.prim_mat != A.prim_mat.data()) A.prim_mat.assign(a.prim_mat, a.prim_mat + a.n_prims);
    A.mat_kind.assign(a.mat_kind, a.mat_kind + a.n_mats); A.mat_tex.assign(a.mat_tex, a.mat_tex + a.n_mats); A.mat_param.assign(a.mat_param, a.mat_param + a.n_mats);
    A.tex_kind.assign(a.tex_kind, a.tex_kind + a.n_tex); A.tex_param.assign(a.tex_param, a.tex_param + (size_t)a.n_tex * RTMI_TEX_STRIDE);
    A.tex_child.assign(a.tex_child, a.tex_child + 2 * (size_t)a.n_tex);
    s->revision++;
}
int prepare_material_edit(rtmi_scene *s, int n_mats, const int32_t *mat_kind, const int32_t *mat_tex, const double *mat_param, int n_tex, const int32_t *tex_kind,
                          const double *tex_param, const int32_t *tex_child, const int32_t *prim_mat, SceneArrays &a, PackedMaterials &M) {
    int rc = check_material_arrays(n_mats, mat_kind, mat_tex, mat_param, n_tex, tex_kind, tex_param, tex_child);
    if (rc) return rc;
    if (!scene_ok(s)) return fail(RTMI_E_STATE, "invalid scene handle");
    a = kept_arrays(s);
    a.n_mats = n_mats; a.mat_kind = mat_kind; a.mat_tex = mat_tex; a.mat_param = mat_param;
    a.n_tex = n_tex; a.tex_kind = tex_kind; a.tex_param = tex_param; a.tex_child = tex_child;
    if (prim_mat) a.prim_mat = prim_mat;
    rc = check_material_edit(a);
    if (rc) return rc;
    M = pack_materials(a);
    return RTMI_OK;
}
}

RTMI_EXPORT int rtmi_scene_set_materials(rtmi_scene *s, int32_t n_mats, const int32_t *mat_kind, const int32_t *mat_tex, const double *mat_param,
                                         int32_t n_tex, const int32_t *tex_kind, const double *tex_param, const int32_t *tex_child,
                                         const int32_t *prim_mat, int32_t *out_rebuilt) {
    SceneArrays a;
    PackedMaterials M;
    int rc = prepare_material_edit(s, n_mats, mat_kind, mat_tex, mat_param, n_tex, tex_kind, tex_param, tex_child, prim_mat, a, M);
    if (rc) return rc;
    HIP_TRY(hipSetDevice(s->ctx->device));
    if (!materials_fit(s, a, M, nullptr)) {
        rc = rebuild_scene(s, a, "rtmi_scene_set_materials");
        if (rc) return rc;
        adopt_materials(s, a, nullptr);
        if (out_rebuilt) *out_rebuilt = 1;
        return RTMI_OK;
    }
    HIP_TRY(hipStreamSynchronize(s->ctx->stream));
    const auto was = material_tables(s->mat, s->dev), now = material_tables(M, s->dev);
    for (int t = 0; t < kMatTables; ++t) {
        const MatTable &o = was[(size_t)t], &n = now[(size_t)t];
        if (n.bytes == 0 || std::memcmp(o.host, n.host, n.bytes) == 0) continue;
        HIP_TRY(hipMemcpy(const_cast<void *>(n.dev), n.host, n.bytes, hipMemcpyHostToDevice));
    }
    adopt_materials(s, a, &M);
    if (out_rebuilt) *out_rebuilt = 0;
    return RTMI_OK;
}

RTMI_EXPORT int rtmi_scene_set_materials_stream(rtmi_scene *s, int32_t n_mats, const int32_t *mat_kind, const int32_t *mat_tex, const double *mat_param,
                                                int32_t n_tex, const int32_t *tex_kind, const double *tex_param, const int32_t *tex_child,
                                                const int32_t *prim_mat, void *stream) {
    SceneArrays a;
    PackedMaterials M;
    int rc = prepare_material_edit(s, n_mats, mat_kind, mat_tex, mat_param, n_tex, tex_kind, tex_param, tex_child, prim_mat, a, M);
    if (rc) return rc;
    std::string why;
    if (!materials_fit(s, a, M, &why))
        return fail(RTMI_E_UNSUPPORTED, "%s: rtmi_scene_set_materials rebuilds the scene for such an edit, the stream form does not", why.c_str());
    const auto was = material_tables(s->mat, s->dev), now = material_tables(M, s->dev);
    std::vector<PatchArgs> batches;
    size_t payload = 0;
    int words_used = 0;
    for (int t = 0; t < kMatTables; ++t) {
        const MatTable &o = was[(size_t)t], &n = now[(size_t)t];
        const char *ob = (const char *)o.host, *nb = (const char *)n.host;
        for (size_t off = 0; off + n.row <= n.bytes; off += n.row) {
            if (std::memcmp(ob + off, nb + off, n.row) == 0) continue;
            payload += n.row;
            if (payload > RTMI_EDIT_STREAM_MAX_BYTES)
                return fail(RTMI_E_UNSUPPORTED, "the edit changes more than RTMI_EDIT_STREAM_MAX_BYTES = %d bytes of table rows: rtmi_scene_set_materials copies whole tables, "
                                                "the stream form is for the few records an interactive edit touches", RTMI_EDIT_STREAM_MAX_BYTES);
            const int nw = (int)(n.row / 4);
            if (batches.empty() || batches.back().n_rows == kPatchRows || words_used + nw > kPatchWords) {
                batches.emplace_back();
                std::memset(&batches.back(), 0, sizeof(PatchArgs));
                words_used = 0;
            }
            PatchArgs &b = batches.back();
            PatchRow &r = b.row[b.n_rows++];
            r.dst = reinterpret_cast<unsigned *>(const_cast<char *>((const char *)n.dev + off));
            r.src = (unsigned short)words_used; r.n = (unsigned short)nw;
            std::memcpy(&b.word[words_used], nb + off, n.row);
            words_used += nw;
        }
    }
    HIP_TRY(hipSetDevice(s->ctx->device));
    hipStream_t st = stream ? (hipStream_t)stream : s->ctx->stream;
    for (const PatchArgs &b : batches) {
        hipLaunchKernelGGL(set_materials_kernel, dim3(1), dim3(64), 0, st, b);
        HIP_TRY(hipGetLastError());
    }
    adopt_materials(s, a, &M);
    return RTMI_OK;
}

RTMI_EXPORT int rtmi_test_pack_materials(int32_t n_prims, const int32_t *prim_kind, const double *prim_geom, const int32_t *prim_mat,
                                         int32_t n_mats, const int32_t *mat_kind, const int32_t *mat_tex, const double *mat_param,
                                         int32_t n_tex, const int32_t *tex_kind, const double *tex_param, const int32_t *tex_child,
                                         int32_t cam_kind, const double *cam, const int32_t *prim_flip, const int32_t *prim_xform,
                                         int32_t n_xforms, const int32_t *xform_kind, const double *xform_param, int32_t through_creation,
                                         uint64_t *out_hash, int32_t *out_facts) {
    if (!out_hash || !out_facts) return fail(RTMI_E_ARG, "bad arguments");
    const SceneArrays a{n_prims, prim_kind, prim_geom, prim_mat, n_mats, mat_kind, mat_tex, mat_param, n_tex, tex_kind, tex_param, tex_child,
                        cam_kind, cam, prim_flip, prim_xform, n_xforms, xform_kind, xform_param};
    PackedMaterials M;
    if (through_creation) {
        rtmi_scene *none = nullptr;
        const int rc = check_scene_args(a, &none);
        if (rc) return rc;
        M = pack_scene(a, read_build_knobs()).M;
    } else {
        int rc = check_material_arrays(n_mats, mat_kind, mat_tex, mat_param, n_tex, tex_kind, tex_param, tex_child);
        if (!rc && (n_prims < 0 || (n_prims > 0 && (!prim_kind || !prim_mat)))) rc = fail(RTMI_E_ARG, "primitive arrays are NULL");
        if (!rc) rc = check_material_edit(a);
        if (rc) return rc;
        M = pack_materials(a);
    }
    uint64_t h = 1469598103934665603ull;
    DevScene none{};
    for (const MatTable &t : material_tables(M, none)) {
        const unsigned char *q = (const unsigned char *)t.host;
        for (size_t k = 0; k < t.bytes; ++k) { h ^= q[k]; h *= 1099511628211ull; }
        h ^= (uint64_t)t.bytes; h *= 1099511628211ull;
    }
    *out_hash = h;
    out_facts[0] = M.has_ext ? 1 : 0; out_facts[1] = M.uses_perlin ? 1 : 0; out_facts[2] = M.max_image;
    return RTMI_OK;
}

namespace {
__host__ __device__ inline int refit_key32(unsigned u) { const int v = (int)u; return v ^ ((v >> 31) & 0x7fffffff); }
__host__ __device__ inline int refit_key16(unsigned h) { const int v = (int)(short)(unsigned short)h; return v ^ ((v >> 31) & 0x7fff); }
__host__ __device__ inline unsigned refit_half_outward(unsigned u, bool up) {
    const unsigned sign = u >> 31, a = u & 0x7fffffffu;
    if (a > 0x7f800000u) return 0x7e00u | (sign << 15);
    const bool away = up != (sign != 0);
    unsigned m;
    bool inexact;
    if (a >= 0x47800000u) { m = a == 0x7f800000u ? 0x7c00u : 0x7bffu; inexact = a != 0x7f800000u; }
    else if (a >= 0x38800000u) { m = (((a >> 23) - 112u) << 10) | ((a & 0x7fffffu) >> 13); inexact = (a & 0x1fffu) != 0; }
    else {
        const unsigned e = a >> 23, mant = (a & 0x7fffffu) | 0x800000u, sh = 126u - e;
        if (e == 0 || sh >= 25u) { m = 0; inexact = a != 0; }
        else { m = mant >> sh; inexact = (mant & ((1u << sh) - 1u)) != 0; }
    }
    if (inexact && away) m += 1;
    return m | (sign << 15);
}
template <bool H> __host__ __device__ inline unsigned refit_get(const unsigned *w, int side, int k, int hi) {
    if (H) { const int h = side * 6 + k * 2 + hi; return (w[h >> 1] >> ((h & 1) * 16)) & 0xffffu; }
    return k < 2 ? w[side * 4 + hi * 2 + k] : w[8 + side * 2 + hi];
}
template <bool H> __host__ __device__ inline void refit_put(unsigned *w, int side, int k, int hi, unsigned v) {
    if (H) { const int h = side * 6 + k * 2 + hi; w[h >> 1] = (h & 1) ? ((w[h >> 1] & 0xffffu) | (v << 16)) : ((w[h >> 1] & 0xffff0000u) | v); }
    else w[k < 2 ? side * 4 + hi * 2 + k : 8 + side * 2 + hi] = v;
}
template <bool H> __host__ __device__ inline void refit_load(const unsigned *p, unsigned *w) {
#if defined(__HIP_DEVICE_COMPILE__)
    const uint4 *q = reinterpret_cast<const uint4 *>(p);
#pragma unroll
    for (int k = 0; k < (H ? 2 : 4); ++k) { const uint4 v = q[k]; w[4 * k] = v.x; w[4 * k + 1] = v.y; w[4 * k + 2] = v.z; w[4 * k + 3] = v.w; }
#else
    for (int k = 0; k < (H ? 8 : 16); ++k) w[k] = p[k];
#endif
}
template <bool H> __host__ __device__ inline void refit_node(unsigned *nodes, const float *leaf_box, int n) {
    constexpr int REC = H ? 8 : 16, CODE = H ? 6 : 12;
    unsigned own[16], out[12];
    refit_load<H>(nodes + (size_t)n * REC, own);
// ... 1249 lines not shown
                           reinterpret_cast<u64 *>(d_out_counters));
        HIP_BAIL(hipGetLastError());
    }
#undef HIP_BAIL
    for (int r = n - 1; r >= 0; --r) {
        rtmi_ctx *cr = scenes[r]->ctx;
        if (hipSetDevice(cr->device) != hipSuccess) return bail(fail(RTMI_E_DEVICE, "hipSetDevice(%d) failed", cr->device), true);
        rc = dealt_finish(cr, s_count, retire, cr->stream);
        if (rc) return bail(rc, true);
    }
    for (int r = 1; r < n; ++r) scenes[r]->ctx->consume_pending = false;
    return RTMI_OK;
}

RTMI_EXPORT int rtmi_render_multi_adaptive(int32_t n, rtmi_scene *const *scenes, int32_t nx, int32_t ny, int32_t s_first, int32_t s_count, int32_t retire,
                                           double eps, int32_t depth, uint64_t seed, int32_t precision, double *out_linear, uint8_t *out_rgb8,
                                           double *out_stderr, int32_t *out_samples, uint64_t *out_counters) {
    if (n <= 0 || !scenes || !scene_ok(scenes[0])) return fail(RTMI_E_ARG, "bad replica list");
    if (nx <= 0 || ny <= 0 || (long long)nx * ny > (1ll << 30)) return fail(RTMI_E_ARG, "nx, ny must be > 0 and the frame at most 2^30 pixels (got %d %d)", nx, ny);
    DeviceGuard guard;
    rtmi_ctx *c0 = scenes[0]->ctx;
    HIP_TRY(hipSetDevice(c0->device));
    HostIo io(c0);
    FramePlanes d;
    int rc = d.reserve(io, (size_t)nx * (size_t)ny, true, true, true, out_linear, out_rgb8, out_stderr, out_samples, out_counters);
    if (rc) return rc;
    rc = rtmi_render_multi_adaptive_device(n, scenes, nx, ny, s_first, s_count, retire, eps, depth, seed, precision, d.lin, d.q, d.err, d.smp, d.cnt);
    if (rc) return rc;
    HIP_TRY(hipSetDevice(c0->device));
    const hipError_t e = io.download();
    if (e != hipSuccess) {
        for (int r = 0; r < n; ++r) scenes[r]->ctx->prog.k = 0;
        return fail(RTMI_E_DEVICE, "multi-device adaptive render: %s", hipGetErrorString(e));
    }
    return RTMI_OK;
}

RTMI_EXPORT int rtmi_last_gather_path(rtmi_ctx *c, int32_t *path) {
    if (!ctx_ok(c)) return fail(RTMI_E_STATE, "invalid context handle");
    if (!c->have_gather) return fail(RTMI_E_STATE, "no multi-device render on this context yet");
    if (path) *path = c->last_gather_path;
    return RTMI_OK;
}

RTMI_EXPORT int rtmi_stream_idle(rtmi_ctx *c, int32_t *idle) {
    if (!ctx_ok(c)) return fail(RTMI_E_STATE, "invalid context handle");
    HIP_TRY(hipSetDevice(c->device));
    const hipError_t e = hipStreamQuery(c->stream);
    if (e != hipSuccess && e != hipErrorNotReady) return fail(RTMI_E_DEVICE, "hipStreamQuery: %s", hipGetErrorString(e));
    if (idle) *idle = e == hipSuccess ? 1 : 0;
    return RTMI_OK;
}

RTMI_EXPORT int rtmi_last_passes(rtmi_ctx *c, int32_t *passes) {
    if (!ctx_ok(c)) return fail(RTMI_E_STATE, "invalid context handle");
    if (passes) *passes = c->last_passes;
    return RTMI_OK;
}

RTMI_EXPORT int rtmi_last_accel(rtmi_ctx *c, int32_t *accel) {
    if (!ctx_ok(c)) return fail(RTMI_E_STATE, "invalid context handle");
    if (c->last_accel < 0) return fail(RTMI_E_STATE, "no render on this context yet");
    if (accel) *accel = c->last_accel;
    return RTMI_OK;
}

RTMI_EXPORT int rtmi_last_gather_ms(rtmi_ctx *c, double *ms) {
    if (!ctx_ok(c)) return fail(RTMI_E_STATE, "invalid context handle");
    if (!c->have_gather) return fail(RTMI_E_STATE, "no multi-device render on this context yet");
    HIP_TRY(hipSetDevice(c->device));
    HIP_TRY(hipEventSynchronize(c->ev_g1));
    float t = 0.f;
    HIP_TRY(hipEventElapsedTime(&t, c->ev_g0, c->ev_g1));
    if (ms) *ms = t;
    return RTMI_OK;
}

RTMI_EXPORT int rtmi_last_traversal_counters(rtmi_ctx *c, uint64_t *out_aabb_tests, uint64_t *out_prim_tests) {
    if (!ctx_ok(c)) return fail(RTMI_E_STATE, "invalid context handle");
    if (!c->count_traversal) return fail(RTMI_E_STATE, "set option count_traversal = 1 before the render");
    if (!c->counters.p) return fail(RTMI_E_STATE, "no render on this context yet");
    HIP_TRY(hipSetDevice(c->device));
    HIP_TRY(hipStreamSynchronize(c->last_stream ? c->last_stream : c->stream));
    u64 v[2] = {0, 0};
    HIP_TRY(hipMemcpy(v, reinterpret_cast<u64 *>(c->counters.p) + 3, sizeof v, hipMemcpyDeviceToHost));
    if (out_aabb_tests) *out_aabb_tests = v[0];
    if (out_prim_tests) *out_prim_tests = v[1];
    return RTMI_OK;
}

RTMI_EXPORT int rtmi_last_trace_ms(rtmi_ctx *c, double *ms, int32_t *launches) {
    if (!ctx_ok(c)) return fail(RTMI_E_STATE, "invalid context handle");
    if (!(c->flags & RTMI_FLAG_TIMING)) return fail(RTMI_E_STATE, "context was not created with RTMI_FLAG_TIMING");
    double total = 0.0, reduce = 0.0;
    for (int k = 0; k < c->events_used; ++k) {
        HIP_TRY(hipEventSynchronize(c->events[(size_t)k].second));
        float t = 0.f;
        HIP_TRY(hipEventElapsedTime(&t, c->events[(size_t)k].first, c->events[(size_t)k].second));
        total += t;
        if ((size_t)k < c->events_r.size()) {
            HIP_TRY(hipEventSynchronize(c->events_r[(size_t)k]));
            HIP_TRY(hipEventElapsedTime(&t, c->events[(size_t)k].second, c->events_r[(size_t)k]));
            reduce += t;
        }
    }
    if (ms) *ms = total;
// ... 1386 lines not shown
```

### raytrace_clj_amd/csrc/rtmi_device.h

```cpp
#pragma once
#include <hip/hip_runtime.h>
#include <stdint.h>

#include "rtmi.h"

namespace rtmi {

typedef unsigned long long u64;

struct DevScene {
    int n_static;
    int n_moving;
    const double *stat_geom;
    const double *stat4_d;
    const float *stat4_f;
    int n_all;
    const float *cull20;
    const double *exact12;
    double cull_t_lo, cull_t_hi;
    const float *bvh_nodes;
    int bvh_root;
    int n_big;
    int big_idx[16];
    int bvh_node16;
    float bvh_obound;
    float bvh_cbound;
    int n_moving_all;
    const int *moving_all;
    int grid_n;
    int grid_kmax;
    int grid_walk;
    int grid_tall;
    float grid_lo_x, grid_lo_z, grid_inv_x, grid_inv_z;
    float grid_box[6];
    float grid_tall_box[6];
    float grid_eps;
    unsigned grid_box_h[3], grid_tall_box_h[3];
    const int *grid_cells;
    int has_ext;
    int small_scan;
    const double *leaf_rec;
    const int *ext_info;
    const double *ext_xf;
    int n_mloc;
    int mloc_root[4];
    float mloc_box[4][6];
    int media_lo[32];
    int media_seq;
    int n_media;
    int media_idx[32];
    double media_fast[8][8];
    const double *perlin_vec;
    const int *perlin_perm;
    int n_images;
    const int *image_wh;
    const long long *image_off;
    const unsigned char *image_rgb;
    const int *stat_orig;
    const double *mov_geom;
    const int *mov_orig;
    const int *prim_kind;
    const int *prim_mat;
    const int *prim_km;
    const double *mat_rec;
    const double *mat_grad;
    const int *mat_kind;
    const int *mat_tex;
    const double *mat_param;
    int n_tex;
    const int *tex_kind;
    const double *tex_param;
    const int *tex_child;
    int cam_kind;
    int cam_fixed_origin;
    double cam[24];
};
typedef const __attribute__((address_space(4))) DevScene &SceneRef;
typedef const __attribute__((address_space(4))) DevScene *ScenePtr;

#define RTMI_GOLD 0x9E3779B97F4A7C15ULL
__host__ __device__ inline u64 mix64(u64 z) {
    z ^= z >> 32; z *= 0xD6E8FEB86659FD93ULL;
    z ^= z >> 32; z *= 0xD6E8FEB86659FD93ULL;
    z ^= z >> 32;
    return z;
}
__host__ __device__ inline u64 sample_key(u64 seed, u64 pix, u64 s) {
    return mix64(mix64(seed ^ (RTMI_GOLD * (pix + 1))) + 0xD1B54A32D192ED03ULL * (s + 1));
}
__host__ __device__ inline u64 draw_bits(u64 key, u64 d) { return mix64(key + RTMI_GOLD * (d + 1)); }

#ifdef RTMI_STAMPS
enum { PH_LOOP = 0, PH_REFILL_GEN, PH_REFILL_DEAL, PH_BVH_SETUP, PH_BIG, PH_DESCENT, PH_LEAF, PH_BVH_POST, PH_HITREC, PH_DNORM, PH_SAMPLER, PH_DIRS, PH_TEXTURE, PH_STORE, PH_UV, PH_CAL, PH_GRID, PH_MEDIA, PH_GEN_KEY, PH_GEN_DISK, PH_GEN_CAM, PH_N };
#define PH_SLOTS 24
__shared__ unsigned long long g_ph[4][3 * PH_SLOTS + 2];
__device__ inline void ph_stamp(int k, unsigned lane_trips = 0, unsigned trips = 0) {
    __builtin_amdgcn_sched_barrier(0);
    unsigned long long t;
    asm volatile("s_memtime %0\n\ts_waitcnt lgkmcnt(0)" : "=s"(t)::"memory");
    const unsigned long long ex = __ballot(1);
    const int w = threadIdx.x >> 6;
    if ((int)(threadIdx.x & 63) == __ffsll((long long)ex) - 1) {
        const unsigned long long dt = t - g_ph[w][3 * PH_SLOTS];
        if (k >= 0) {
            g_ph[w][2 * PH_SLOTS + k] += 1;
            g_ph[w][k] += dt;
            g_ph[w][PH_SLOTS + k] += trips ? dt * (unsigned long long)lane_trips / (unsigned long long)trips : dt * (unsigned long long)__popcll(ex);
        }
        g_ph[w][3 * PH_SLOTS] = t;
    }
    __builtin_amdgcn_sched_barrier(0);
}
#define RTMI_PH(k) ph_stamp(k);
#define RTMI_PH_LANES(k, lt, tr) ph_stamp(k, lt, tr);
#elif defined(RTMI_MARKERS)
#define RTMI_PH(k) asm volatile("; PHASE_END " #k);
#define RTMI_PH_LANES(k, lt, tr) asm volatile("; PHASE_END " #k);
#else
#define RTMI_PH(k)
#define RTMI_PH_LANES(k, lt, tr)
#endif
__device__ inline double rt_sqrt(double x) {
// ... 1578 lines not shown
        sw[2 * stride] = (int)(reinterpret_cast<char *>(cur.top) - reinterpret_cast<char *>(stack));
        sw[3 * stride] = __double2loint(H.t); sw[4 * stride] = __double2hiint(H.t);
        sw[5 * stride] = H.F; sw[6 * stride] = H.W;
        return false;
    }
    if (!r.time_ok) {
        if (COUNT) cnt[1] += (unsigned)sc.n_moving_all;
        for (int k = 0; k < sc.n_moving_all; ++k) {
            if (sc.moving_all[k] >= lo && sc.moving_all[k] < hi) ext_prim_test<true>(sc, sc.moving_all[k], P, tmin, H);
            if (ANY && H.any()) break;
        }
    }
    return true;
}

template <typename R>
__device__ inline void scan_moving(SceneRef sc, const Path<R> &P, R a, R tmin, R &best_t, int &best_i, int &best_orig) {
    const R a2 = R(2.0) * a, a4 = R(4.0) * a;
    for (int m = 0; m < sc.n_moving; ++m) {
        const double *g = sc.mov_geom + (size_t)m * RTMI_PRIM_STRIDE;
        const R t0 = (R)g[7], t1 = (R)g[8];
        const R f = (P.time - t0) / (t1 - t0), omf = R(1.0) - f;
        const R cx = (R)g[0] * omf + (R)g[4] * f, cy = (R)g[1] * omf + (R)g[5] * f, cz = (R)g[2] * omf + (R)g[6] * f;
        const R rad = (R)g[3];
        const R ocx = P.ox - cx, ocy = P.oy - cy, ocz = P.oz - cz;
        const R b = R(2.0) * dot3(ocx, ocy, ocz, P.dx, P.dy, P.dz);
        const R c = dot3(ocx, ocy, ocz, ocx, ocy, ocz) - rad * rad;
        const R disc = b * b - a4 * c;
        if (disc >= R(0)) {
            const R sq = Real<R>::sqrt_(disc);
            const int orig = sc.mov_orig[m];
            R t = (-b - sq) / a2;
            bool ok = (t > tmin) && ((t < best_t) || (t == best_t && orig < best_orig));
            if (!ok) {
                t = (-b + sq) / a2;
                ok = (t > tmin) && ((t < best_t) || (t == best_t && orig < best_orig));
            }
            if (ok) { best_t = t; best_i = sc.n_static + m; best_orig = orig; }
        }
    }
}

struct SegLog { double *rec; int max_seg; int n; };

template <typename R> struct HitRec { R t, px, py, pz, nx, ny, nz, u, v; int orig, kind, mat; };

#define RTMI_TEX_CHECKER2 100
#define RTMI_TEX_GRADIENT_REC 101
struct __attribute__((aligned(16))) MatRec { int mat_kind, tex, tex_kind, pad; double param, r, g, b; double scale, c1r, c1g, c1b; double inv_ri, r0; };

#define RTMI_PRIM_NEEDS_U 32
#define RTMI_PRIM_NEEDS_V 64
#define RTMI_PRIM_NEEDS_UV (RTMI_PRIM_NEEDS_U | RTMI_PRIM_NEEDS_V)
template <typename R> __device__ inline void resolve_hit(SceneRef sc, const Path<R> &P, R t, int orig, HitRec<R> &h, bool all_uv = true) {
    const double *g = sc.exact12 + (size_t)orig * 12;
    R cx = (R)g[0], cy = (R)g[1], cz = (R)g[2];
    h.orig = orig;
    const int2 km = reinterpret_cast<const int2 *>(sc.prim_km)[orig];
    if ((km.x & 15) == RTMI_PRIM_MOVING) {
        const R t0 = (R)g[7], t1 = (R)g[8];
        const R f = (P.time - t0) / (t1 - t0), omf = R(1.0) - f;
        cx = (R)g[0] * omf + (R)g[4] * f; cy = (R)g[1] * omf + (R)g[5] * f; cz = (R)g[2] * omf + (R)g[6] * f;
    }
    const int kind_flags = km.x;
    h.kind = kind_flags & 15;
    h.mat = km.y;
    h.t = t;
    h.px = P.dx * t + P.ox; h.py = P.dy * t + P.oy; h.pz = P.dz * t + P.oz;
    R nx = h.px - cx, ny = h.py - cy, nz = h.pz - cz;
    const R len = Real<R>::sqrt_(dot3(nx, ny, nz, nx, ny, nz));
    if (len > R(0)) { const R inv = R(1.0) / len; nx = nx * inv; ny = ny * inv; nz = nz * inv; }
    h.nx = nx; h.ny = ny; h.nz = nz;
    h.u = R(0); h.v = R(0);
    RTMI_PH(PH_HITREC)
    if (h.kind == RTMI_PRIM_UVSPHERE && (all_uv || (kind_flags & RTMI_PRIM_NEEDS_UV))) {
        h.u = h.v = R(0.5);
        if (all_uv || (kind_flags & RTMI_PRIM_NEEDS_U)) h.u = Real<R>::sphere_u(nx, nz);
        if (all_uv || (kind_flags & RTMI_PRIM_NEEDS_V)) h.v = Real<R>::sphere_v(ny);
        RTMI_PH(PH_UV)
    }
}

__device__ inline void leaf_xform_back(int xk, double a, double b, double c, double &px, double &py, double &pz, double &nx, double &nz) {
    if (xk == 1) { px = px + a; py = py + b; pz = pz + c; }
    else if (xk == 2) {
        const double rx = b * px + a * pz, rz = (-(a * px)) + b * pz;
        const double mx = b * nx + a * nz, mz = (-(a * nx)) + b * nz;
        px = rx; pz = rz; nx = mx; nz = mz;
    }
}
__device__ inline void resolve_hit_ext(SceneRef sc, const Path<double> &P, double t, int orig, HitRec<double> &h, bool all_uv = true) {
#if RTMI_LEAF_RECORDS
    {
        const double2 *q = reinterpret_cast<const double2 *>(sc.leaf_rec + (size_t)orig * RTMI_LEAF_REC_DOUBLES);
        const int4 hdr = *reinterpret_cast<const int4 *>(q);
        if (!hdr.y) {
            const double2 q1 = q[1], q2 = q[2], q3 = q[3], q4 = q[4], q5 = q[5], q6 = q[6];
            const int kind = hdr.x & 0xff;
            h.orig = orig; h.kind = kind; h.mat = sc.prim_mat[orig]; h.t = t;
            const bool want_uv = all_uv || (sc.prim_kind[orig] & RTMI_PRIM_NEEDS_UV);
            LocalRay r = {P.ox, P.oy, P.oz, P.dx, P.dy, P.dz};
            if (hdr.z | hdr.w) {
                leaf_xform(hdr.z, q3.y, q4.x, q4.y, r);
                leaf_xform(hdr.w, q5.x, q5.y, q6.x, r);
            }
            double px = r.dx * t + r.ox, py = r.dy * t + r.oy, pz = r.dz * t + r.oz;
            double nx, ny, nz;
            h.u = 0.0; h.v = 0.0;
            if (kind <= RTMI_PRIM_UVSPHERE) {
                nx = px - q1.x; ny = py - q1.y; nz = pz - q2.x;
                const double len = rt_sqrt(dot3(nx, ny, nz, nx, ny, nz));
                if (len > 0.0) { const double inv = 1.0 / len; nx = nx * inv; ny = ny * inv; nz = nz * inv; }
                if (kind == RTMI_PRIM_UVSPHERE && want_uv) Real<double>::sphere_uv(nx, ny, nz, &h.u, &h.v);
            } else {
                int ax, ua, va;
                rect_axes(kind, ax, ua, va);
                if (want_uv) {
                    const double x = pick3(ua, r.ox, r.oy, r.oz) + t * pick3(ua, r.dx, r.dy, r.dz), y = pick3(va, r.ox, r.oy, r.oz) + t * pick3(va, r.dx, r.dy, r.dz);
                    h.u = (x - q1.x) / (q2.x - q1.x); h.v = (y - q1.y) / (q2.y - q1.y);
                }
                nx = ax == 0 ? 1.0 : 0.0; ny = ax == 1 ? 1.0 : 0.0; nz = ax == 2 ? 1.0 : 0.0;
            }
            if (hdr.x & 0x100) { nx = -nx; ny = -ny; nz = -nz; }
            if (hdr.z | hdr.w) {
                leaf_xform_back(hdr.w, q5.x, q5.y, q6.x, px, py, pz, nx, nz);
                leaf_xform_back(hdr.z, q3.y, q4.x, q4.y, px, py, pz, nx, nz);
            }
            h.px = px; h.py = py; h.pz = pz; h.nx = nx; h.ny = ny; h.nz = nz;
            return;
        }
    }
#endif
    const int4 info = reinterpret_cast<const int4 *>(sc.ext_info)[orig];
    const LocalRay r = ext_local_ray(sc, info.z, info.w, P);
    const double *g = sc.exact12 + (size_t)orig * 12;
    const int kind = info.x;
    h.orig = orig; h.kind = kind; h.mat = sc.prim_mat[orig]; h.t = t;
    double px = r.dx * t + r.ox, py = r.dy * t + r.oy, pz = r.dz * t + r.oz;
    double nx, ny, nz;
    h.u = 0.0; h.v = 0.0;
    if (kind <= RTMI_PRIM_MOVING) {
        double cx = g[0], cy = g[1], cz = g[2];
        if (kind == RTMI_PRIM_MOVING) {
            const double t0 = g[7], t1 = g[8];
            const double f = (P.time - t0) / (t1 - t0), omf = 1.0 - f;
            cx = g[0] * omf + g[4] * f; cy = g[1] * omf + g[5] * f; cz = g[2] * omf + g[6] * f;
        }
        nx = px - cx; ny = py - cy; nz = pz - cz;
        const double len = rt_sqrt(dot3(nx, ny, nz, nx, ny, nz));
        if (len > 0.0) { const double inv = 1.0 / len; nx = nx * inv; ny = ny * inv; nz = nz * inv; }
        if (kind == RTMI_PRIM_UVSPHERE && (all_uv || (sc.prim_kind[orig] & RTMI_PRIM_NEEDS_UV))) {
            Real<double>::sphere_uv(nx, ny, nz, &h.u, &h.v);
        }
    } else if (kind == RTMI_PRIM_MEDIUM) {
        nx = 1.0; ny = 0.0; nz = 0.0;
    } else if (kind <= RTMI_PRIM_RECT_YZ) {
        int ax, ua, va;
        rect_axes(kind, ax, ua, va);
        if (all_uv || (sc.prim_kind[orig] & RTMI_PRIM_NEEDS_UV)) {
            const double x = pick3(ua, r.ox, r.oy, r.oz) + t * pick3(ua, r.dx, r.dy, r.dz), y = pick3(va, r.ox, r.oy, r.oz) + t * pick3(va, r.dx, r.dy, r.dz);
            h.u = (x - g[0]) / (g[2] - g[0]); h.v = (y - g[1]) / (g[3] - g[1]);
        }
        nx = ax == 0 ? 1.0 : 0.0; ny = ax == 1 ? 1.0 : 0.0; nz = ax == 2 ? 1.0 : 0.0;
    } else {
        if (all_uv || (sc.prim_kind[orig] & RTMI_PRIM_NEEDS_UV)) {
            double u = 0.0, v = 0.0, tt;
            tri_mt(g[0], g[1], g[2], g[3], g[4], g[5], g[6], g[7], g[8], r, u, v, tt);
            h.u = u; h.v = v;
        }
        cross3(g[3] - g[0], g[4] - g[1], g[5] - g[2], g[6] - g[0], g[7] - g[1], g[8] - g[2], nx, ny, nz);
    }
    if (info.y) { nx = -nx; ny = -ny; nz = -nz; }
    for (int k = info.w - 1; k >= 0; --k) {
        const double *q = sc.ext_xf + (size_t)(info.z + k) * 4;
        if (q[0] == 0.0) { px = px + q[1]; py = py + q[2]; pz = pz + q[3]; }
        else {
            const double sn = q[1], cs = q[2];
            const double rx = cs * px + sn * pz, rz = (-(sn * px)) + cs * pz;
            const double mx = cs * nx + sn * nz, mz = (-(sn * nx)) + cs * nz;
            px = rx; pz = rz; nx = mx; nz = mz;
        }
    }
    h.px = px; h.py = py; h.pz = pz; h.nx = nx; h.ny = ny; h.nz = nz;
}
template <typename R, bool EXT> __device__ inline void resolve_any(SceneRef sc, const Path<R> &P, R t, int orig, HitRec<R> &h, bool all_uv = true) { resolve_hit<R>(sc, P, t, orig, h, all_uv); }
template <> __device__ inline void resolve_any<double, true>(SceneRef sc, const Path<double> &P, double t, int orig, HitRec<double> &h, bool all_uv) { resolve_hit_ext(sc, P, t, orig, h, all_uv); }

template <typename R, bool F4 = false> __device__ inline bool scatter_emit(SceneRef sc, Path<R> &P, const HitRec<R> &h, R *att, R *emit, bool passenger = false) {
    const int mat = h.mat;
    const double2 *mq = reinterpret_cast<const double2 *>(sc.mat_rec + (size_t)mat * 12);
    const double2 m0 = mq[0], m1 = mq[1], m2 = mq[2];
    const int mk = (int)__double2loint(m0.x), mtex = (int)__double2hiint(m0.x), mtk = (int)__double2loint(m0.y);
    const R mparam = (R)m1.x;
    const R px = h.px, py = h.py, pz = h.pz, nx = h.nx, ny = h.ny, nz = h.nz;
    const bool is_light = !passenger && mk == RTMI_MAT_DIFFUSE_LIGHT;
    const bool live = !passenger && !is_light && P.depth > 0;
    const bool is_lamb = live && mk == RTMI_MAT_LAMBERTIAN, is_metal = live && mk == RTMI_MAT_METAL, is_diel = live && mk == RTMI_MAT_DIELECTRIC;
    const bool is_iso = F4 && live && mk == RTMI_MAT_ISOTROPIC;
    bool scat = false;
    emit[0] = emit[1] = emit[2] = R(0);
    R sdx = R(0), sdy = R(0), sdz = R(0);
    R atr = R(1), atg = R(1), atb = R(1);

    R dmag = R(0), ux = P.dx, uy = P.dy, uz = P.dz;
    if (is_metal || is_diel) {
        dmag = Real<R>::sqrt_(dot3(ux, uy, uz, ux, uy, uz));
        if (dmag > R(0)) { const R inv = R(1.0) / dmag; ux = ux * inv; uy = uy * inv; uz = uz * inv; }
        RTMI_PH(PH_DNORM)
    }
    R rx = R(0), ry = R(0), rz = R(0);
    RTMI_PH(PH_DIRS)
    rand_in_unit_sphere_wave(P, is_lamb || is_metal || is_iso, rx, ry, rz);
    RTMI_PH(PH_SAMPLER)
    if (is_lamb) {
        const R tx = (px + nx) + rx, ty = (py + ny) + ry, tz = (pz + nz) + rz;
        sdx = tx - px; sdy = ty - py; sdz = tz - pz;
        scat = true;
        RTMI_PH(PH_DIRS)
    } else if (is_iso) {
        sdx = rx; sdy = ry; sdz = rz;
        P.time = h.t;
        scat = true;
        RTMI_PH(PH_DIRS)
    } else if (is_metal) {
        const R fuzz = mparam;
        const R k = R(2.0) * dot3(ux, uy, uz, nx, ny, nz);
        const R rfx = ux - k * nx, rfy = uy - k * ny, rfz = uz - k * nz;
        sdx = rfx + fuzz * rx; sdy = rfy + fuzz * ry; sdz = rfz + fuzz * rz;
        scat = dot3(sdx, sdy, sdz, nx, ny, nz) > R(0);
        RTMI_PH(PH_DIRS)
    } else if (is_diel) {
        const R ri = mparam;
        const R dn = dot3(P.dx, P.dy, P.dz, nx, ny, nz);
        R onx, ony, onz, eta, cosine;
        if (dn > R(0)) { onx = -nx; ony = -ny; onz = -nz; eta = ri; cosine = ri * (dn / dmag); }
        else { onx = nx; ony = ny; onz = nz; eta = sizeof(R) == sizeof(double) ? (R)mq[5].x : R(1.0) / ri; cosine = -(dn / dmag); }
        const R dt = dot3(ux, uy, uz, onx, ony, onz);
        const R disc = R(1.0) - (eta * eta) * (R(1.0) - dt * dt);
        const R k = R(2.0) * dn;
        sdx = P.dx - k * nx; sdy = P.dy - k * ny; sdz = P.dz - k * nz;
        if (disc > R(0)) {
            R r0;
            if (sizeof(R) == sizeof(double)) r0 = (R)mq[5].y;
            else { r0 = (R(1.0) - ri) / (R(1.0) + ri); r0 = r0 * r0; }
            const R prob = r0 + (R(1.0) - r0) * pow5(R(1.0) - cosine);
            if (!(next_uniform(P) < prob)) {
                const R sq = Real<R>::sqrt_(disc);
                sdx = eta * (ux - onx * dt) - onx * sq;
                sdy = eta * (uy - ony * dt) - ony * sq;
                sdz = eta * (uz - onz * dt) - onz * sq;
            }
        }
        scat = true;
        RTMI_PH(PH_DIRS)
    }
    const bool want_tex = is_light || is_lamb || is_iso || (is_metal && scat);
    double turb = 0.0, turb_p0 = 0.0;
    bool turb_done = false;
    if (F4 && sizeof(R) == sizeof(double)) {
        const bool want_turb = want_tex && (mtk == RTMI_TEX_MARBLE || mtk == RTMI_TEX_PERLIN_TURB);
        const int n_turb = __popcll(__ballot(want_turb));
        if (n_turb > 0 && n_turb <= RTMI_TURB_WAVE_MAX) {
            double p1 = 0.0;
            if (want_turb) { const double *tp = sc.tex_param + (size_t)mtex * RTMI_TEX_STRIDE; turb_p0 = tp[0]; p1 = tp[1]; }
            const double s = mtk == RTMI_TEX_PERLIN_TURB ? turb_p0 : 1.0;
            turb = perlin_turbulence_wave(sc, want_turb, s * (double)px, s * (double)py, s * (double)pz, (int)p1);
            turb_done = want_turb;
        }
    }
    if (want_tex) {
        R tr, tg, tb;
        if (mtk == RTMI_TEX_CONSTANT) { tr = (R)m1.y; tg = (R)m2.x; tb = (R)m2.y; }
        else if (F4 && turb_done) {
            if (mtk == RTMI_TEX_PERLIN_TURB) tr = tg = tb = R(0.5) * ((R)turb + R(1.0));
            else tr = tg = tb = R(0.5) * (Real<R>::sin_((R)turb_p0 * pz + R(10.0) * (R)turb) + R(1.0));
        }
        else if (mtk == RTMI_TEX_CHECKER2) {
            const double2 m3 = mq[3], m4 = mq[4];
            const R scale = (R)m3.x;
            const int sx = sin_sign<R>(scale * px), sy = sin_sign<R>(scale * py), sz = sin_sign<R>(scale * pz);
            const bool neg = sx * sy * sz < 0;
            tr = neg ? (R)m1.y : (R)m3.y; tg = neg ? (R)m2.x : (R)m4.x; tb = neg ? (R)m2.y : (R)m4.y;
        } else if (mtk == RTMI_TEX_GRADIENT_REC) {
            const double2 *gq = reinterpret_cast<const double2 *>(sc.mat_grad + (size_t)mat * 12);
            const double2 g0 = gq[0], g1 = gq[1], g2 = gq[2], g3 = gq[3], g4 = gq[4], g5 = gq[5];
            const R u = h.u, v = h.v, omu = R(1.0) - u, omv = R(1.0) - v;
            const R a0 = (R)g1.y * omu + (R)g0.x * u, a1 = (R)g2.x * omu + (R)g0.y * u, a2 = (R)g2.y * omu + (R)g1.x * u;
            const R b0 = (R)g4.y * omu + (R)g3.x * u, b1 = (R)g5.x * omu + (R)g3.y * u, b2 = (R)g5.y * omu + (R)g4.x * u;
            tr = b0 * omv + a0 * v; tg = b1 * omv + a1 * v; tb = b2 * omv + a2 * v;
        } else tex_sample<R, F4>(sc, mtex, h.u, h.v, px, py, pz, tr, tg, tb);
        if (is_light) { emit[0] = R(0) + P.ar * tr; emit[1] = R(0) + P.ag * tg; emit[2] = R(0) + P.ab * tb; }
        else { atr = tr; atg = tg; atb = tb; }
        RTMI_PH(PH_TEXTURE)
    }
    if (!scat) return false;
    if (att) { att[0] = atr; att[1] = atg; att[2] = atb; }
    P.ox = px; P.oy = py; P.oz = pz; P.dx = sdx; P.dy = sdy; P.dz = sdz;
    P.ar = P.ar * atr; P.ag = P.ag * atg; P.ab = P.ab * atb;
    P.depth -= 1;
    return true;
}

template <typename R, bool EXT = false>
__device__ inline bool shade_segment(SceneRef sc, Path<R> &P, R t, int orig, SegLog *lg, R *emit, bool passenger = false) {
    emit[0] = emit[1] = emit[2] = R(0);
    if (!passenger && orig < 0) return false;
    HitRec<R> h;
    h.px = h.py = h.pz = h.nx = h.ny = h.nz = h.u = h.v = h.t = R(0); h.mat = 0; h.orig = 0; h.kind = 0;
    if (!passenger) {
        resolve_any<R, EXT>(sc, P, t, orig, h, false);
        RTMI_PH(PH_HITREC)
    }
    const bool scat = scatter_emit<R, EXT>(sc, P, h, nullptr, emit, passenger);
    if (lg && lg->n < lg->max_seg) {
        double *q = lg->rec + (size_t)lg->n * RTMI_SEG_REC;
        q[0] = h.orig; q[1] = h.t; q[2] = h.px; q[3] = h.py; q[4] = h.pz; q[5] = h.nx; q[6] = h.ny; q[7] = h.nz;
        q[8] = scat ? P.dx : 0; q[9] = scat ? P.dy : 0; q[10] = scat ? P.dz : 0; q[11] = scat ? 1.0 : 0.0;
        lg->n++;
    }
    return scat;
}

template <typename R, bool EXT = false>
__device__ inline bool shade_segment_nee(SceneRef sc, Path<R> &P, R t, int orig, R *emit, HitRec<R> &h, bool &lamb) {
    emit[0] = emit[1] = emit[2] = R(0);
    lamb = false;
    h.px = h.py = h.pz = h.nx = h.ny = h.nz = h.u = h.v = h.t = R(0); h.mat = 0; h.orig = 0; h.kind = 0;
    if (orig < 0) return false;
    resolve_any<R, EXT>(sc, P, t, orig, h, false);
    const bool scat = scatter_emit<R, EXT>(sc, P, h, nullptr, emit);
    lamb = scat && sc.mat_kind[h.mat] == RTMI_MAT_LAMBERTIAN;
    return scat;
}

}
```

### raytrace_clj_amd/csrc/scene_build.h

```cpp
#pragma once
#include <unistd.h>

namespace {

struct BuildKnobs {
    int sah_levels = 1 << 20;
    int sweep_max = 0;
    double min_frac = 0.0;
    bool grid_off = false;
    int grid_side = 0;
    int grid_kmax = 4;
    bool grid_walk = true;
    bool mloc = false;
    int node16 = -1;
    bool box_leaf = false;
    bool small_scan = true;
    bool debug = false;
};
inline BuildKnobs read_build_knobs() {
    BuildKnobs k;
    if (const char *e = std::getenv("RTMI_BVH_SAH_LEVELS")) k.sah_levels = std::atoi(e);
    if (const char *e = std::getenv("RTMI_BVH_SWEEP_MAX")) k.sweep_max = std::atoi(e);
    if (const char *e = std::getenv("RTMI_BVH_MIN_FRAC")) k.min_frac = std::atof(e);
    if (const char *e = std::getenv("RTMI_GRID")) { k.grid_off = e[0] == '0'; k.grid_side = std::atoi(e); }
// ... 527 lines not shown
        parallel_blocks(n_nodes, 2048, [&](size_t nb, size_t ne) {
            double a32 = 0.0, a16 = 0.0;
            for (size_t n = nb; n < ne; ++n) {
                const float *q = &B.nodes[n * 16];
                uint16_t h[12];
                for (int side = 0; side < 2; ++side) {
                    const float lo[3] = {q[side * 4], q[side * 4 + 1], q[8 + side * 2]}, hi[3] = {q[side * 4 + 2], q[side * 4 + 3], q[8 + side * 2 + 1]};
                    double e32[3], e16[3];
                    for (int k = 0; k < 3; ++k) {
                        h[side * 6 + k * 2] = half_outward(lo[k], false); h[side * 6 + k * 2 + 1] = half_outward(hi[k], true);
                        e32[k] = (double)hi[k] - lo[k]; e16[k] = half_val(h[side * 6 + k * 2 + 1]) - half_val(h[side * 6 + k * 2]);
                    }
                    if (e32[0] >= 0 && std::isfinite(e32[0] + e32[1] + e32[2])) {
                        a32 += e32[0] * e32[1] + e32[1] * e32[2] + e32[2] * e32[0];
                        a16 += std::isfinite(e16[0] + e16[1] + e16[2]) ? e16[0] * e16[1] + e16[1] * e16[2] + e16[2] * e16[0] : INFINITY;
                    }
                }
                int c[2];
                std::memcpy(c, &q[12], 8);
                for (int k = 0; k < 2; ++k) if (c[k] >= 0 && c[k] != RTMI_BVH_EMPTY) c[k] /= 2;
                std::memcpy(reinterpret_cast<char *>(&out[n * 8]), h, 24);
                std::memcpy(reinterpret_cast<char *>(&out[n * 8]) + 24, c, 8);
            }
            part32[nb / 2048] = a32; part16[nb / 2048] = a16;
        });
        for (size_t k = 0; k < part32.size(); ++k) { area32 += part32[k]; area16 += part16[k]; }
        const bool use16 = K.node16 >= 0 ? K.node16 == 1 : (area16 <= 1.25 * area32);
        if (use16) {
            d.bvh_node16 = 1;
            d.bvh_root = d.bvh_root >= 0 ? d.bvh_root / 2 : d.bvh_root;
            for (int &c : grid_cells) if (c >= 0) c /= 2;
            for (int k = 0; k < d.n_mloc; ++k) if (d.mloc_root[k] >= 0) d.mloc_root[k] /= 2;
            if (d.grid_tall >= 0) d.grid_tall /= 2;
            return out;
        }
    }
    return B.nodes;
}

struct SceneArrays {
    int n_prims; const int32_t *prim_kind; const double *prim_geom; const int32_t *prim_mat;
    int n_mats; const int32_t *mat_kind; const int32_t *mat_tex; const double *mat_param;
    int n_tex; const int32_t *tex_kind; const double *tex_param; const int32_t *tex_child;
    int cam_kind; const double *cam; const int32_t *prim_flip; const int32_t *prim_xform;
    int n_xforms; const int32_t *xform_kind; const double *xform_param;
};

struct PackedMaterials {
    std::vector<double> mat_rec, mat_grad, mat_param, tex_param;
    std::vector<int> prim_kind, prim_km, prim_mat, mat_kind, mat_tex, tex_kind, tex_child;
    bool has_ext = false;
    bool uses_perlin = false;
    int max_image = -1;
};

struct PackedScene {
    DevScene d{};
    std::vector<double> stat_geom, stat4_d, exact12, ext_xf, leaf_rec, mov_geom;
    std::vector<float> stat4_f, bvh_nodes, cull20;
    std::vector<int> stat_orig, grid_cells, moving_all, ext_info, mov_orig;
    PackedMaterials M;
    std::vector<int> host_kind;
    std::map<int, std::array<double, 5>> media_fast_of;
    int bvh_node_count = 0, bvh_depth = 0;
    TreeBuild tree;
    bool geom_ext = false;
    double t_tree0 = 0.0, t_tree1 = 0.0;
};

template <typename T> void pad_last(std::vector<T> &v, size_t rec) {
    const size_t n = v.size() / rec;
    if (n == 0) return;
    const std::vector<T> last(v.end() - (long)rec, v.end());
    while (v.size() < ((n + 7) / 8 * 8 + 8) * rec) v.insert(v.end(), last.begin(), last.end());
}

std::vector<char> texture_uv_use(const SceneArrays &a) {
    std::vector<char> uses((size_t)std::max(a.n_tex, 1), 0);
    bool changed = true;
    for (int pass = 0; pass <= a.n_tex && changed; ++pass) {
        changed = false;
        for (int t = 0; t < a.n_tex; ++t) {
            const int k = a.tex_kind[t];
            char u = k == RTMI_TEX_IMAGE ? 3 : 0;
            if (k == RTMI_TEX_UVGRADIENT) {
                const double *tp = a.tex_param + (size_t)t * RTMI_TEX_STRIDE;
                bool var_u = false, var_v = false;
                auto same = [&](int x, int y) { return std::memcmp(&tp[x], &tp[y], sizeof(double)) == 0; };
                for (int c = 0; c < 3; ++c) {
                    var_u = var_u || !same(c, 3 + c) || !same(6 + c, 9 + c);
                    var_v = var_v || !same(c, 6 + c) || !same(3 + c, 9 + c);
                }
                u = (char)((var_u ? 1 : 0) | (var_v ? 2 : 0));
            }
            if (k == RTMI_TEX_CHECKER || k == RTMI_TEX_FLIP_U || k == RTMI_TEX_FLIP_V)
                for (int c = 0; c < (k == RTMI_TEX_CHECKER ? 2 : 1); ++c) {
                    const int ch = a.tex_child[2 * (size_t)t + c];
                    if (ch >= 0 && ch < a.n_tex) u |= uses[(size_t)ch];
                }
            if (uses[(size_t)t] != u) { uses[(size_t)t] = u; changed = true; }
        }
    }
    return uses;
}

inline bool camera_component_plain(double v) { return std::isfinite(v) && std::isfinite((float)v) && !(std::signbit(v) && (float)v == 0.0f); }
inline int camera_fixed_origin(int cam_kind, const double *cam) {
    bool fixed = cam_kind == RTMI_CAM_PINHOLE || cam[21] == 0.0;
    for (int k = 0; k < 3; ++k) fixed = fixed && camera_component_plain(cam[k]);
    for (int k = 12; k < 18; ++k) fixed = fixed && std::isfinite(cam[k]) && std::isfinite((float)cam[k]);
    return fixed ? 1 : 0;
}
inline int camera_fixed_rays(int cam_kind, int fixed_origin, const double *cam) {
    bool fixed = cam_kind == RTMI_CAM_THINLENS && fixed_origin;
    for (int k = 3; k < 6; ++k) fixed = fixed && camera_component_plain(cam[k]);
    return fixed ? 1 : 0;
}
inline void camera_shutter(int cam_kind, const double *cam, double &t_lo, double &t_hi) {
    t_lo = cam_kind == RTMI_CAM_THINLENS ? std::min(cam[22], cam[23]) : 0.0;
    t_hi = cam_kind == RTMI_CAM_THINLENS ? std::max(cam[22], cam[23]) : 0.0;
}

PackedMaterials pack_materials(const SceneArrays &a) {
    PackedMaterials M;
    const int n_prims = a.n_prims;
    for (int t = 0; t < a.n_tex; ++t) {
        if (a.tex_kind[t] > RTMI_TEX_CHECKER) M.has_ext = true;
        if (a.tex_kind[t] >= RTMI_TEX_PERLIN_NOISE && a.tex_kind[t] <= RTMI_TEX_MARBLE) M.uses_perlin = true;
        if (a.tex_kind[t] == RTMI_TEX_IMAGE) M.max_image = std::max(M.max_image, (int)a.tex_param[(size_t)t * RTMI_TEX_STRIDE]);
    }
    for (int i = 0; i < n_prims; ++i)
        if (a.mat_kind[a.prim_mat[i]] == RTMI_MAT_ISOTROPIC) M.has_ext = true;
    const std::vector<char> uses = texture_uv_use(a);
    M.prim_mat.assign(a.prim_mat, a.prim_mat + n_prims);
    M.prim_kind.resize((size_t)n_prims);
    for (int i = 0; i < n_prims; ++i) {
        const int kind = a.prim_kind[i] & ~RTMI_PRIM_BOUNDARY;
        M.prim_kind[(size_t)i] = kind;
        const int m = M.prim_mat[(size_t)i], t = (m >= 0 && m < a.n_mats) ? a.mat_tex[m] : -1;
        if (kind == RTMI_PRIM_UVSPHERE) {
            const int bits = (t < 0 || t >= a.n_tex) ? 3 : uses[(size_t)t];
            if (bits & 1) M.prim_kind[(size_t)i] |= RTMI_PRIM_NEEDS_U;
            if (bits & 2) M.prim_kind[(size_t)i] |= RTMI_PRIM_NEEDS_V;
        } else if (kind >= RTMI_PRIM_RECT_XY && kind <= RTMI_PRIM_TRIANGLE) {
            if (t < 0 || t >= a.n_tex || uses[(size_t)t]) M.prim_kind[(size_t)i] |= RTMI_PRIM_NEEDS_UV;
        }
    }
    M.prim_km.assign((size_t)std::max(n_prims, 1) * 2, 0);
    for (int i = 0; i < n_prims; ++i) { M.prim_km[2 * (size_t)i] = M.prim_kind[(size_t)i]; M.prim_km[2 * (size_t)i + 1] = M.prim_mat[(size_t)i]; }
    M.mat_rec.assign((size_t)std::max(a.n_mats, 1) * 12, 0.0);
    M.mat_grad.assign((size_t)std::max(a.n_mats, 1) * 12, 0.0);
    for (int m = 0; m < a.n_mats; ++m) {
        MatRec r;
        std::memset(&r, 0, sizeof(r));
        r.mat_kind = a.mat_kind[m]; r.tex = a.mat_tex[m]; r.param = a.mat_param[m];
        if (a.mat_kind[m] == RTMI_MAT_DIELECTRIC) {
            const volatile double ri = a.mat_param[m];
            const volatile double inv = 1.0 / ri, num = 1.0 - ri, den = 1.0 + ri;
            const volatile double q = num / den;
            const volatile double r0 = q * q;
            r.inv_ri = inv; r.r0 = r0;
        }
        r.tex_kind = (r.tex >= 0 && r.tex < a.n_tex) ? a.tex_kind[r.tex] : -1;
        if (r.tex_kind == RTMI_TEX_CONSTANT) { const double *tp = a.tex_param + (size_t)r.tex * RTMI_TEX_STRIDE; r.r = tp[0]; r.g = tp[1]; r.b = tp[2]; }
        if (r.tex_kind == RTMI_TEX_UVGRADIENT) {
            std::memcpy(&M.mat_grad[(size_t)m * 12], a.tex_param + (size_t)r.tex * RTMI_TEX_STRIDE, 12 * sizeof(double));
            r.tex_kind = RTMI_TEX_GRADIENT_REC;
        }
        if (r.tex_kind == RTMI_TEX_CHECKER) {
            const int c0 = a.tex_child[2 * (size_t)r.tex], c1 = a.tex_child[2 * (size_t)r.tex + 1];
            if (c0 >= 0 && c0 < a.n_tex && c1 >= 0 && c1 < a.n_tex && a.tex_kind[c0] == RTMI_TEX_CONSTANT && a.tex_kind[c1] == RTMI_TEX_CONSTANT) {
                const double *t0 = a.tex_param + (size_t)c0 * RTMI_TEX_STRIDE, *t1 = a.tex_param + (size_t)c1 * RTMI_TEX_STRIDE;
                r.tex_kind = RTMI_TEX_CHECKER2;
                r.scale = a.tex_param[(size_t)r.tex * RTMI_TEX_STRIDE];
                r.r = t0[0]; r.g = t0[1]; r.b = t0[2]; r.c1r = t1[0]; r.c1g = t1[1]; r.c1b = t1[2];
            }
        }
        static_assert(sizeof(MatRec) == 96, "MatRec is twelve doubles");
        std::memcpy(&M.mat_rec[(size_t)m * 12], &r, sizeof(r));
    }
    M.mat_kind.assign(a.mat_kind, a.mat_kind + a.n_mats); M.mat_tex.assign(a.mat_tex, a.mat_tex + a.n_mats); M.mat_param.assign(a.mat_param, a.mat_param + a.n_mats);
    M.tex_kind.assign(a.tex_kind, a.tex_kind + a.n_tex); M.tex_child.assign(a.tex_child, a.tex_child + 2 * (size_t)a.n_tex);
    M.tex_param.assign(a.tex_param, a.tex_param + (size_t)a.n_tex * RTMI_TEX_STRIDE);
    return M;
}

struct GeomExtras {
    std::vector<BvhBox> wbox;
    std::vector<char> bounded, box_first;
    int n_world = 0, n_media = 0, media[16];
};
void pack_geometry(const SceneArrays &a, bool box_leaf, double t_lo, double t_hi, PackedScene &P, GeomExtras &X) {
    DevScene &d = P.d;
    const int n_prims = a.n_prims;
    int &n_world = X.n_world, &n_media = X.n_media, *media = X.media;
    for (int k = 0; k < a.n_xforms; ++k) {
        const double *p = a.xform_param + (size_t)k * 3;
        const double rec[4] = {a.xform_kind[k] == RTMI_XFORM_TRANSLATE ? 0.0 : 1.0, p[0], p[1], p[2]};
        P.ext_xf.insert(P.ext_xf.end(), rec, rec + 4);
    }
    std::vector<float> cull;
    std::vector<BvhBox> &wbox = X.wbox;
// ... 127 lines not shown
            for (int c = 0; c < 5; ++c) q[2 + c] = P.exact12[(size_t)i * 12 + c];
            for (int k = 0; k < xf_count; ++k) {
                const double *xp = a.xform_param + (size_t)(xf_first + k) * 3;
                hdr[2 + k] = a.xform_kind[xf_first + k] == RTMI_XFORM_TRANSLATE ? 1 : 2;
                q[7 + 3 * k] = xp[0]; q[8 + 3 * k] = xp[1]; q[9 + 3 * k] = xp[2];
            }
            if (box_first[(size_t)i]) q[13] = P.exact12[(size_t)i * 12 + 5];
        }
        std::memcpy(q, hdr, sizeof hdr);
    }
    P.ext_info.insert(P.ext_info.end(), {RTMI_PRIM_MEDIUM, 0, 0, 0});
    for (int k = 0; k < n_media; ++k) {
        const int m = media[k];
        const int fb = (int)a.prim_geom[(size_t)m * RTMI_PRIM_STRIDE + 1], nb = (int)a.prim_geom[(size_t)m * RTMI_PRIM_STRIDE + 2];
        if (nb != 1 || fb < 0 || fb >= n_prims) continue;
        if (pk[(size_t)fb] != RTMI_PRIM_SPHERE && pk[(size_t)fb] != RTMI_PRIM_UVSPHERE) continue;
        if (a.prim_xform && (a.prim_xform[2 * m + 1] != 0 || a.prim_xform[2 * fb + 1] != 0)) continue;
        const double *e = &P.exact12[0];
        P.media_fast_of[m] = {e[(size_t)m * 12], e[(size_t)fb * 12], e[(size_t)fb * 12 + 1], e[(size_t)fb * 12 + 2], e[(size_t)fb * 12 + 3]};
    }
}

void build_trees(const SceneArrays &a, const BuildKnobs &K, bool has_ext, const GeomExtras &X, PackedScene &P) {
    DevScene &d = P.d;
    const double *cam = a.cam;
    const std::vector<BvhBox> &wbox = X.wbox;
    const std::vector<char> &bounded = X.bounded, &box_first = X.box_first;
    const std::vector<int> &pk = P.host_kind;
    const int n_world = X.n_world, n_media = X.n_media, *media = X.media;
    P.t_tree0 = now_ms();
    std::vector<BvhBox> media_boxes;
    for (int k = 0; k < n_media; ++k) {
        const double *mg = a.prim_geom + (size_t)media[k] * RTMI_PRIM_STRIDE;
        const int fb = (int)mg[1], nb = (int)mg[2];
        BvhBox u = box_empty();
        bool ok = true;
        for (int q = fb; q < fb + nb; ++q) { ok = ok && bounded[(size_t)q]; if (ok) box_grow(u, wbox[(size_t)q]); }
        if (ok) media_boxes.push_back(u);
    }
    P.bvh_nodes = build_bvh(d, n_world, pk.data(), wbox, bounded, cam, !has_ext, P.grid_cells, box_first, K, &P.bvh_depth, &media_boxes, &P.tree);
    P.bvh_node_count = (int)(P.bvh_nodes.size() / (d.bvh_node16 ? 8 : 16));
    if (K.debug)
        fprintf(stderr, "[rtmi] tree: %d node records of %d bytes (%.2f MB), depth %d, %d big primitives, %d box leaves; entry grid %d x %d cells, %zu rectangle trees\n", P.bvh_node_count,
                d.bvh_node16 ? 32 : 64, P.bvh_node_count * (d.bvh_node16 ? 32.0 : 64.0) / 1e6, P.bvh_depth, d.n_big, (int)std::count(box_first.begin(), box_first.end(), (char)1), d.grid_n, d.grid_n, P.grid_cells.size());
    if (K.debug && d.n_mloc) fprintf(stderr, "[rtmi] %d medium neighbourhood tree(s)\n", d.n_mloc);
    P.t_tree1 = now_ms();
}

PackedScene pack_scene(const SceneArrays &a, const BuildKnobs &K) {
    PackedScene P;
    DevScene &d = P.d;
    std::memset(&d, 0, sizeof d);
    const double *cam = a.cam;
    P.M = pack_materials(a);
    d.n_tex = a.n_tex; d.cam_kind = a.cam_kind;
    std::memcpy(d.cam, cam, 24 * sizeof(double));
    d.cam_fixed_origin = camera_fixed_origin(a.cam_kind, cam);
    double t_lo, t_hi;
    camera_shutter(a.cam_kind, cam, t_lo, t_hi);
    GeomExtras X;
    pack_geometry(a, K.box_leaf, t_lo, t_hi, P, X);
    const int n_world = X.n_world;
    const bool has_ext = P.geom_ext || P.M.has_ext;
    build_trees(a, K, has_ext, X, P);
    d.has_ext = has_ext ? 1 : 0;
    d.small_scan = (has_ext && n_world <= RTMI_SMALL_SCAN_MAX && K.small_scan) ? 1 : 0;
    return P;
}

}
```

Baseline: 7956 Msamples/s.

## Defer sky-light gradient texture lookup from trace kernel to the fold/reduce pass

For scenes with exactly one diffuse-light material whose UV-gradient texture depends only on v and is used only on UV spheres (the sky), the trace kernel no longer evaluates that texture when a path terminates. It stores the throughput plus the hit normal y in a 4-wide record, and the reduce/fold kernels finish the gradient multiply. This cuts texture and material work and divergence from the hot trace loop. In exchange the sample buffer grows from 3 to 4 reals per sample, and a NaN tag marks records that were not deferred.

```diff
diff --git a/include/rtmi.h b/include/rtmi.h
--- a/include/rtmi.h
+++ b/include/rtmi.h
@@ -250,6 +250,7 @@
 int rtmi_rccl_probe(const char *soname);
 int rtmi_stream_idle(rtmi_ctx *ctx, int32_t *idle);
 int rtmi_last_passes(rtmi_ctx *ctx, int32_t *passes);
+int rtmi_last_record_reals(rtmi_ctx *ctx, int32_t *reals);
 int rtmi_last_accel(rtmi_ctx *ctx, int32_t *accel);
 int rtmi_last_gather_ms(rtmi_ctx *ctx0, double *ms);
 
diff --git a/raytrace_clj_amd/_ffi.py b/raytrace_clj_amd/_ffi.py
--- a/raytrace_clj_amd/_ffi.py
+++ b/raytrace_clj_amd/_ffi.py
@@ -18,7 +18,7 @@
     "rtmi_probe_paths", "rtmi_probe_camera", "rtmi_probe_texture", "rtmi_probe_scatter", "rtmi_probe_rng",
     "rtmi_sample_key", "rtmi_test_half_outward", "rtmi_test_camera_fixed", "rtmi_test_build_tree", "rtmi_probe_arith", "rtmi_probe_math", "rtmi_probe_math2", "rtmi_last_traversal_counters",
     "rtmi_scene_clone", "rtmi_render_multi", "rtmi_render_multi_device", "rtmi_last_gather_ms",
-    "rtmi_last_gather_path", "rtmi_rccl_probe", "rtmi_stream_idle", "rtmi_last_passes", "rtmi_last_accel",
+    "rtmi_last_gather_path", "rtmi_rccl_probe", "rtmi_stream_idle", "rtmi_last_passes", "rtmi_last_record_reals", "rtmi_last_accel",
     "rtmi_render_progressive", "rtmi_render_progressive_device", "rtmi_progressive_samples", "rtmi_progressive_release",
     "rtmi_render_adaptive", "rtmi_render_adaptive_device", "rtmi_adaptive_status", "rtmi_adaptive_active_tiles",
     "rtmi_render_features", "rtmi_render_features_device", "rtmi_denoise", "rtmi_denoise_device",
@@ -121,6 +121,7 @@
     L.rtmi_rccl_probe.argtypes = [C.c_char_p]
     L.rtmi_stream_idle.argtypes = [vp, C.POINTER(i32)]
     L.rtmi_last_passes.argtypes = [vp, C.POINTER(i32)]
+    L.rtmi_last_record_reals.argtypes = [vp, C.POINTER(i32)]
     L.rtmi_last_accel.argtypes = [vp, C.POINTER(i32)]
     L.rtmi_render_progressive.argtypes = [vp, i32, i32, i32, i32, i32, u64, i32, i32, i32, i32, i32, vp, vp, vp, vp]
     L.rtmi_render_progressive_device.argtypes = [vp, i32, i32, i32, i32, i32, u64, i32, vp, vp, vp, vp, vp]
diff --git a/raytrace_clj_amd/csrc/rtmi.hip b/raytrace_clj_amd/csrc/rtmi.hip
--- a/raytrace_clj_amd/csrc/rtmi.hip
+++ b/raytrace_clj_amd/csrc/rtmi.hip
@@ -72,6 +72,7 @@
     int stash_off;
     double rnx, rny;
     int fixed_rays;
+    int defer_mat;
 };
 #ifndef RTMI_QUEUE_BLOCK
 #define RTMI_QUEUE_BLOCK 256
@@ -86,6 +87,32 @@
 #define RTMI_STASH 1
 #endif
 constexpr unsigned kQueueBlock = RTMI_QUEUE_BLOCK;
+
+__device__ inline void store_record4(void *samples, unsigned item, const double *rgb, double w) {
+    double2 *o = reinterpret_cast<double2 *>(samples) + (size_t)item * 2;
+    o[0] = make_double2(rgb[0], rgb[1]); o[1] = make_double2(rgb[2], w);
+}
+__device__ inline void store_record4(void *samples, unsigned item, const float *rgb, float w) {
+    reinterpret_cast<float4 *>(samples)[item] = make_float4(rgb[0], rgb[1], rgb[2], w);
+}
+__device__ inline void load_record4(const double *rec, double *rgb, double &w) {
+    const double2 a = reinterpret_cast<const double2 *>(rec)[0], b = reinterpret_cast<const double2 *>(rec)[1];
+    rgb[0] = a.x; rgb[1] = a.y; rgb[2] = b.x; w = b.y;
+}
+__device__ inline void load_record4(const float *rec, float *rgb, float &w) {
+    const float4 a = *reinterpret_cast<const float4 *>(rec);
+    rgb[0] = a.x; rgb[1] = a.y; rgb[2] = a.z; w = a.w;
+}
+template <typename R> __device__ inline void fold_record4(const R *rec, const GradientU<R> &q, bool use, R *v) {
+    R w;
+    load_record4(rec, v, w);
+    const bool deferred = use && !SampleTag<R>::is(w);
+    if (__any(deferred ? 1 : 0)) {
+        if (deferred) finish_deferred<R>(q, w, v[0], v[1], v[2]);
+    }
+}
+template <bool DEFER> __device__ inline int fold_elem(int l, int k) { return DEFER ? 3 * l + k : l + 64 * k; }
+template <bool DEFER> __device__ inline int fold_pixel(int l, int k) { return DEFER ? l : (l + 64 * k) / 3; }
 
 template <typename R> __device__ inline const R *stat4_of(SceneRef sc);
 template <typename R> __device__ inline void stage_prims(SceneRef sc, Prim4<R> *lds, int first, int count) {
@@ -282,7 +309,7 @@
 #endif
 }
 
-template <typename R, bool MULTI, int VARIANT, bool EXT = false, bool COUNT = false, bool SLICE = true, int MSEQ = 0, bool LST = false>
+template <typename R, bool MULTI, int VARIANT, bool EXT = false, bool COUNT = false, bool SLICE = true, int MSEQ = 0, bool LST = false, bool DEFER = false>
 __global__ void __launch_bounds__(kTraceBlock, EXT ? ((MSEQ != 0 || COUNT) ? 3 : RTMI_EXT_MIN_WAVES) : RTMI_MIN_WAVES) trace_kernel(ScenePtr scp, TraceParams tp) {
     SceneRef sc = *scp;
     extern __shared__ __attribute__((aligned(16))) char smem[];
@@ -465,12 +492,23 @@
         if (alive) {
             if (!mid) ++nrays;
             R emit[3];
-            const bool scat = shade_segment<R, EXT>(sc, P, best_t, best_i, nullptr, emit, mid);
-            if (!mid && !scat) {
-                R *out = reinterpret_cast<R *>(tp.samples) + (size_t)out_item * 3;
-                out[0] = emit[0]; out[1] = emit[1]; out[2] = emit[2];
-                alive = false;
-                RTMI_PH(PH_STORE)
+            if constexpr (!DEFER) {
+                const bool scat = shade_segment<R, EXT>(sc, P, best_t, best_i, nullptr, emit, mid);
+                if (!mid && !scat) {
+                    R *out = reinterpret_cast<R *>(tp.samples) + (size_t)out_item * 3;
+                    out[0] = emit[0]; out[1] = emit[1]; out[2] = emit[2];
+                    alive = false;
+                    RTMI_PH(PH_STORE)
+                }
+            } else {
+                R dny;
+                bool deferred;
+                const bool scat = shade_segment<R, EXT, true>(sc, P, best_t, best_i, nullptr, emit, mid, tp.defer_mat, &deferred, &dny);
+                if (!mid && !scat) {
+                    store_record4(tp.samples, out_item, emit, deferred ? dny : SampleTag<R>::value());
+                    alive = false;
+                    RTMI_PH(PH_STORE)
+                }
             }
         }
         }
@@ -487,11 +525,11 @@
     }
 }
 
-template <typename R>
+template <typename R, bool DEFER = false>
 __global__ void __launch_bounds__(kBlock) reduce_kernel(const R *__restrict__ samples, R *__restrict__ accum, double *__restrict__ tiles_linear,
                                                         const int *__restrict__ tile_ids, int tiles_x, int nx, int ny, int n_local_tiles,
                                                         int s_begin, int s_count, int ns, u64 *counters, u64 n_valid_pixels,
-                                                        int rx0, int ry0, int rx1, int ry1) {
+                                                        int rx0, int ry0, int rx1, int ry1, const double *__restrict__ grad) {
     const long long gid = (long long)blockIdx.x * blockDim.x + threadIdx.x;
     if (gid == 0 && counters && s_begin + s_count >= ns) counters[1] = n_valid_pixels;
     if (gid >= (long long)n_local_tiles * 64) return;
@@ -503,20 +541,31 @@
     const size_t tile_base = (size_t)tile_local * 192;
 #pragma unroll
     for (int k = 0; k < 3; ++k) {
-        const int p = (l + 64 * k) / 3;
+        const int p = fold_pixel<DEFER>(l, k);
         const int x = tx + (p & 7), y = ty + (p >> 3);
         valid[k] = x >= rx0 && x < rx1 && y >= ry0 && y < ry1;
-        acc[k] = (valid[k] && s_begin > 0) ? accum[tile_base + l + 64 * k] : R(0);
-    }
+        acc[k] = (valid[k] && s_begin > 0) ? accum[tile_base + fold_elem<DEFER>(l, k)] : R(0);
+    }
+    if constexpr (DEFER) {
+        const GradientU<R> gu = gradient_rec_u<R>(grad, R(0.5));
+        const R *rec = samples + ((size_t)tile_local * s_count * 64 + l) * 4;
+        for (int s = 0; s < s_count; ++s, rec += 256) {
+            R v[3];
+            fold_record4<R>(rec, gu, valid[0], v);
+            if (s_begin + s == 0) { acc[0] = v[0]; acc[1] = v[1]; acc[2] = v[2]; }
+            else { acc[0] = acc[0] + v[0]; acc[1] = acc[1] + v[1]; acc[2] = acc[2] + v[2]; }
+        }
+    } else {
     const R *row = samples + (size_t)tile_local * s_count * 192 + l;
     for (int s = 0; s < s_count; ++s, row += 192) {
         const R v0 = row[0], v1 = row[64], v2 = row[128];
         if (s_begin + s == 0) { acc[0] = v0; acc[1] = v1; acc[2] = v2; }
         else { acc[0] = acc[0] + v0; acc[1] = acc[1] + v1; acc[2] = acc[2] + v2; }
     }
+    }
 #pragma unroll
     for (int k = 0; k < 3; ++k) {
-        const size_t o = tile_base + l + 64 * k;
+        const size_t o = tile_base + fold_elem<DEFER>(l, k);
         if (s_begin + s_count < ns) accum[o] = valid[k] ? acc[k] : R(0);
         else tiles_linear[o] = valid[k] ? (double)(acc[k] * (R(1.0) / (R)ns)) : 0.0;
     }
@@ -741,10 +790,11 @@
     int *keep = nullptr, *n_t = nullptr;
 };
 
-template <typename R, bool RETIRE>
+template <typename R, bool RETIRE, bool DEFER = false>
 __global__ void __launch_bounds__(kBlock) frame_fold_kernel(const R *__restrict__ samples, R *__restrict__ sums, double *__restrict__ mean,
                                                             double *__restrict__ m2, const int *__restrict__ tiles, int tiles_x, int n_entries, int s_begin,
-                                                            int s_count, u64 *counters, u64 n_valid_pixels, int rx0, int ry0, int rx1, int ry1, FoldRetire rt) {
+                                                            int s_count, u64 *counters, u64 n_valid_pixels, int rx0, int ry0, int rx1, int ry1, FoldRetire rt,
+                                                            const double *__restrict__ grad) {
     const long long gid = (long long)blockIdx.x * blockDim.x + threadIdx.x;
     if (gid == 0) counters[1] = n_valid_pixels;
     if (gid >= (long long)n_entries * 64) return;
@@ -759,18 +809,22 @@
     const size_t tile_base = (size_t)slot * 192;
 #pragma unroll
     for (int k = 0; k < 3; ++k) {
-        const int p = (l + 64 * k) / 3;
+        const int p = fold_pixel<DEFER>(l, k);
         const int x = tx + (p & 7), y = ty + (p >> 3);
         valid[k] = x >= rx0 && x < rx1 && y >= ry0 && y < ry1;
         const bool carry = valid[k] && s_begin > 0;
-        const size_t o = tile_base + l + 64 * k;
+        const size_t o = tile_base + fold_elem<DEFER>(l, k);
         acc[k] = carry ? sums[o] : R(0);
         mu[k] = carry ? mean[o] : 0.0;
         q[k] = carry ? m2[o] : 0.0;
     }
-    const R *row = samples + (size_t)entry * s_count * 192 + l;
-    for (int s = 0; s < s_count; ++s, row += 192) {
-        const R v[3] = {row[0], row[64], row[128]};
+    GradientU<R> gu = {};
+    if constexpr (DEFER) gu = gradient_rec_u<R>(grad, R(0.5));
+    const R *row = DEFER ? samples + ((size_t)entry * s_count * 64 + l) * 4 : samples + (size_t)entry * s_count * 192 + l;
+    for (int s = 0; s < s_count; ++s, row += DEFER ? 256 : 192) {
+        R v[3];
+        if constexpr (DEFER) fold_record4<R>(row, gu, valid[0], v);
+        else { v[0] = row[0]; v[1] = row[64]; v[2] = row[128]; }
         if (s_begin + s == 0) {
 #pragma unroll
             for (int k = 0; k < 3; ++k) { acc[k] = v[k]; mu[k] = (double)v[k]; q[k] = 0.0; }
@@ -787,7 +841,7 @@
     }
 #pragma unroll
     for (int k = 0; k < 3; ++k) {
-        const size_t o = tile_base + l + 64 * k;
+        const size_t o = tile_base + fold_elem<DEFER>(l, k);
         sums[o] = valid[k] ? acc[k] : R(0);
         mean[o] = valid[k] ? mu[k] : 0.0;
         m2[o] = valid[k] ? q[k] : 0.0;
@@ -1980,10 +2034,12 @@
     hipEvent_t ev_consumed = nullptr;
     int ev_consumed_device = -1;
     bool consume_pending = false;
+    int defer_emitters = 1;
     int fail_next_render = 0;
     int fail_allocs = 0;
     int last_accel = -1;
     int last_passes = 0;
+    int last_record_reals = 0;
     int last_grid = 0;
     std::map<std::pair<const void *, size_t>, int> occupancy;
     std::vector<int> tile_ids_host;
@@ -2193,8 +2249,14 @@
     return RTMI_OK;
 }
 
-struct LaunchKnobs { const char *flat_below, *suspend_lanes, *sphere_stash; };
-LaunchKnobs read_launch_knobs() { return {std::getenv("RTMI_FLAT_BELOW"), std::getenv("RTMI_SUSPEND_LANES"), std::getenv("RTMI_SPHERE_LDS_STASH")}; }
+struct LaunchKnobs { const char *flat_below, *suspend_lanes, *sphere_stash, *defer_emitters; };
+LaunchKnobs read_launch_knobs() {
+    return {std::getenv("RTMI_FLAT_BELOW"), std::getenv("RTMI_SUSPEND_LANES"), std::getenv("RTMI_SPHERE_LDS_STASH"), std::getenv("RTMI_DEFER_EMITTERS")};
+}
+int launch_defer_mat(const rtmi_scene *s, const rtmi_ctx *c, const LaunchKnobs &k) {
+    const bool on = k.defer_emitters ? k.defer_emitters[0] != '0' : c->defer_emitters != 0;
+    return (on && !s->dev.has_ext) ? s->dev.defer_mat : -1;
+}
 
 struct LdsLayout { int susp_off, stash_off; size_t bytes; };
 LdsLayout lds_layout(int levels, int susp_words, int stash_words) {
@@ -2206,10 +2268,11 @@
     LdsLayout lds{RTMI_BVH_STACK * RTMI_BVH_STRIDE, 0, 0};
     int suspend_lanes = 0;
     int accel = RTMI_ACCEL_BVH;
+    bool defers = false;
 };
 
 template <typename R>
-TracePlan choose_trace_kernel(const rtmi_scene *s, const rtmi_ctx *c, const LaunchKnobs &k, bool multi, size_t lds_bytes) {
+TracePlan choose_trace_kernel(const rtmi_scene *s, const rtmi_ctx *c, const LaunchKnobs &k, bool multi, size_t lds_bytes, int defer_mat) {
     const DevScene &d = s->dev;
     TracePlan p;
     int variant = c->accel == RTMI_ACCEL_BVH ? SCAN_BVH : c->scan_variant;
@@ -2241,7 +2304,13 @@
         const LdsLayout stash = lds_layout(levels, RTMI_BVH_SUSPEND_WORDS, stash_words);
         if (slice) p.kern = count ? trace_kernel<R, false, SCAN_BVH, false, true> : trace_kernel<R, false, SCAN_BVH>;
         else p.kern = count ? trace_kernel<R, false, SCAN_BVH, false, true, false> : trace_kernel<R, false, SCAN_BVH, false, false, false>;
-        if (slice && !count && !(k.sphere_stash && k.sphere_stash[0] == '0') && stash.bytes <= 40 * 1024) { p.kern = trace_kernel<R, false, SCAN_BVH, false, false, true, false, true>; p.lds = stash; }
+        const bool lst = slice && !count && !(k.sphere_stash && k.sphere_stash[0] == '0') && stash.bytes <= 40 * 1024;
+        if (lst) { p.kern = trace_kernel<R, false, SCAN_BVH, false, false, true, false, true>; p.lds = stash; }
+        if (defer_mat >= 0 && !count) {
+            p.defers = true;
+            p.kern = lst ? trace_kernel<R, false, SCAN_BVH, false, false, true, 0, true, true>
+                         : slice ? trace_kernel<R, false, SCAN_BVH, false, false, true, 0, false, true> : trace_kernel<R, false, SCAN_BVH, false, false, false, 0, false, true>;
+        }
     } else if (variant == SCAN_SGPR_CULL) p.kern = trace_kernel<R, false, SCAN_SGPR_CULL>;
     else if (variant == SCAN_SGPR) p.kern = trace_kernel<R, false, SCAN_SGPR>;
     else {
@@ -2350,9 +2419,10 @@
     return RTMI_OK;
 }
 
-int size_sample_passes(rtmi_ctx *c, int n_local, int ns, size_t real_bytes, int *out_s_per_pass) {
-    const size_t per_sample = (size_t)n_local * 64 * 3 * real_bytes;
-    int s_per_pass = (int)std::max<int64_t>(1, std::min<int64_t>(ns, c->workspace_bytes / (int64_t)per_sample));
+int size_sample_passes(rtmi_ctx *c, int n_local, int ns, size_t real_bytes, int record_reals, int *out_s_per_pass) {
+    const size_t budgeted = (size_t)n_local * 64 * 3 * real_bytes;
+    const size_t per_sample = (size_t)n_local * 64 * (size_t)record_reals * real_bytes;
+    int s_per_pass = (int)std::max<int64_t>(1, std::min<int64_t>(ns, c->workspace_bytes / (int64_t)budgeted));
     while (s_per_pass > 1 && (long long)n_local * s_per_pass * 64 >= 0xf0000000ll) s_per_pass /= 2;
     if ((long long)n_local * s_per_pass * 64 >= 0xf0000000ll) return fail(RTMI_E_ARG, "frame too large for one pass: %d tiles per rank", n_local);
     if (per_sample * (size_t)s_per_pass > c->samples.bytes) {
@@ -2408,27 +2478,28 @@
 }
 
 template <typename R>
-int launch_fold(rtmi_ctx *c, const TraceParams &tp, int ns, int s_end, void *d_tiles_linear, bool count_pixels, ProgFrame *prog, const AdaptiveCall *ad,
-                hipEvent_t e1, hipStream_t st) {
+int launch_fold(rtmi_ctx *c, const TraceParams &tp, const double *defer_grad, int ns, int s_end, void *d_tiles_linear, bool count_pixels, ProgFrame *prog,
+                const AdaptiveCall *ad, hipEvent_t e1, hipStream_t st) {
     const long long npx = (long long)tp.n_local_tiles * 64;
     const dim3 grid((unsigned)((npx + kBlock - 1) / kBlock));
     const R *samples = reinterpret_cast<const R *>(c->samples.p);
+    const bool defer = tp.defer_mat >= 0;
     if (ad) {
         FoldRetire rt;
         rt.act_slots = reinterpret_cast<const int *>(prog->act_slots[prog->cur].p);
         rt.last = tp.s_begin + tp.s_count == s_end ? 1 : 0; rt.eps = ad->eps;
         rt.keep = reinterpret_cast<int *>(prog->keep.p); rt.n_t = reinterpret_cast<int *>(prog->n_t.p);
-        hipLaunchKernelGGL((frame_fold_kernel<R, true>), grid, dim3(kBlock), 0, st, samples, reinterpret_cast<R *>(prog->sums.p),
+        hipLaunchKernelGGL((defer ? frame_fold_kernel<R, true, true> : frame_fold_kernel<R, true>), grid, dim3(kBlock), 0, st, samples, reinterpret_cast<R *>(prog->sums.p),
                            reinterpret_cast<double *>(prog->mean.p), reinterpret_cast<double *>(prog->m2.p), tp.tile_ids, tp.tiles_x, tp.n_local_tiles,
-                           tp.s_begin, tp.s_count, tp.counters, (u64)c->tile_valid_pixels, tp.rx0, tp.ry0, tp.rx1, tp.ry1, rt);
+                           tp.s_begin, tp.s_count, tp.counters, (u64)c->tile_valid_pixels, tp.rx0, tp.ry0, tp.rx1, tp.ry1, rt, defer_grad);
     } else if (prog)
-        hipLaunchKernelGGL((frame_fold_kernel<R, false>), grid, dim3(kBlock), 0, st, samples, reinterpret_cast<R *>(prog->sums.p),
+        hipLaunchKernelGGL((defer ? frame_fold_kernel<R, false, true> : frame_fold_kernel<R, false>), grid, dim3(kBlock), 0, st, samples, reinterpret_cast<R *>(prog->sums.p),
                            reinterpret_cast<double *>(prog->mean.p), reinterpret_cast<double *>(prog->m2.p), tp.tile_ids, tp.tiles_x, tp.n_local_tiles,
-                           tp.s_begin, tp.s_count, tp.counters, (u64)c->tile_valid_pixels, tp.rx0, tp.ry0, tp.rx1, tp.ry1, FoldRetire{});
+                           tp.s_begin, tp.s_count, tp.counters, (u64)c->tile_valid_pixels, tp.rx0, tp.ry0, tp.rx1, tp.ry1, FoldRetire{}, defer_grad);
     else
-        hipLaunchKernelGGL((reduce_kernel<R>), grid, dim3(kBlock), 0, st, samples, reinterpret_cast<R *>(c->accum.p),
+        hipLaunchKernelGGL((defer ? reduce_kernel<R, true> : reduce_kernel<R>), grid, dim3(kBlock), 0, st, samples, reinterpret_cast<R *>(c->accum.p),
                            reinterpret_cast<double *>(d_tiles_linear), tp.tile_ids, tp.tiles_x, tp.nx, tp.ny, tp.n_local_tiles, tp.s_begin, tp.s_count, ns,
-                           count_pixels ? tp.counters : nullptr, (u64)c->tile_valid_pixels, tp.rx0, tp.ry0, tp.rx1, tp.ry1);
+                           count_pixels ? tp.counters : nullptr, (u64)c->tile_valid_pixels, tp.rx0, tp.ry0, tp.rx1, tp.ry1, defer_grad);
     HIP_TRY(hipGetLastError());
     return e1 ? close_timed_fold(c, st) : RTMI_OK;
 }
@@ -2460,18 +2531,21 @@
 
     const int ns = s_end - s_first;
     int s_per_pass = 0;
-    rc = size_sample_passes(c, n_local, ns, sizeof(R), &s_per_pass);
-    if (rc) return rc;
+    const LaunchKnobs knobs = read_launch_knobs();
+    int ppt, nptiles;
+    size_t lds_bytes;
+    lds_plan(c, s->dev.n_static, sizeof(R), &ppt, &nptiles, &lds_bytes);
+    const TracePlan plan = choose_trace_kernel<R>(s, c, knobs, nptiles > 1, lds_bytes, launch_defer_mat(s, c, knobs));
+    const int defer_mat = plan.defers ? s->dev.defer_mat : -1;
+    rc = size_sample_passes(c, n_local, ns, sizeof(R), defer_mat >= 0 ? 4 : 3, &s_per_pass);
+    if (rc) return rc;
+    c->last_accel = plan.accel;
+    c->last_record_reals = defer_mat >= 0 ? 4 : 3;
     c->last_passes = (ns + s_per_pass - 1) / s_per_pass;
     if (!prog && s_per_pass < ns) {
         rc = c->accum.ensure((size_t)n_local * 64 * 3 * sizeof(R));
         if (rc) return rc;
     }
-    int ppt, nptiles;
-    size_t lds_bytes;
-    lds_plan(c, s->dev.n_static, sizeof(R), &ppt, &nptiles, &lds_bytes);
-    const TracePlan plan = choose_trace_kernel<R>(s, c, read_launch_knobs(), nptiles > 1, lds_bytes);
-    c->last_accel = plan.accel;
 
     TraceParams tp;
     tp.nx = nx; tp.ny = ny; tp.depth = depth; tp.seed = seed; tp.tiles_x = tiles_x_of(nx);
@@ -2485,10 +2559,12 @@
     tp.trav = reinterpret_cast<u64 *>(c->counters.p) + 3;
     tp.suspend_lanes = plan.suspend_lanes; tp.susp_off = plan.lds.susp_off; tp.stash_off = plan.lds.stash_off;
     tp.rnx = 1.0 / (double)nx; tp.rny = 1.0 / (double)ny; tp.fixed_rays = camera_fixed_rays(s->dev.cam_kind, s->dev.cam_fixed_origin, s->dev.cam);
+    tp.defer_mat = defer_mat;
+    const double *defer_grad = defer_mat >= 0 ? s->dev.mat_grad + (size_t)defer_mat * 12 : nullptr;
     for (int s_begin = s_first; s_begin < s_end; s_begin += s_per_pass) {
         hipEvent_t e1 = nullptr;
         rc = launch_trace_pass(s, plan, tp, s_begin, std::min(s_per_pass, s_end - s_begin), st, &e1);
-        if (!rc) rc = launch_fold<R>(c, tp, ns, s_end, d_tiles_linear, d_counters != nullptr, prog, ad, e1, st);
+        if (!rc) rc = launch_fold<R>(c, tp, defer_grad, ns, s_end, d_tiles_linear, d_counters != nullptr, prog, ad, e1, st);
         if (rc) return rc;
     }
 #ifdef RTMI_STAMPS
@@ -2684,6 +2760,7 @@
     if (!std::strcmp(name, "timing")) { if (value) c->flags |= RTMI_FLAG_TIMING; else c->flags &= ~RTMI_FLAG_TIMING; return RTMI_OK; }
     if (!std::strcmp(name, "scan_variant")) { if (value < 0 || value > 3) return fail(RTMI_E_ARG, "scan_variant must be 0..3"); c->scan_variant = (int)value; return RTMI_OK; }
     if (!std::strcmp(name, "count_traversal")) { c->count_traversal = value ? 1 : 0; return RTMI_OK; }
+    if (!std::strcmp(name, "defer_emitters")) { if (value < 0 || value > 1) return fail(RTMI_E_ARG, "defer_emitters must be 0 or 1"); c->defer_emitters = (int)value; return RTMI_OK; }
     if (!std::strcmp(name, "test_fail_next_render")) { c->fail_next_render = value ? 1 : 0; return RTMI_OK; }
     if (!std::strcmp(name, "test_fail_allocs")) { c->fail_allocs = (int)std::max<int64_t>(0, std::min<int64_t>(value, 64)); return RTMI_OK; }
     if (!std::strcmp(name, "flat_below")) { if (value < 0 || value > (1 << 20)) return fail(RTMI_E_ARG, "flat_below must be 0..2^20"); c->flat_below = (int)value; return RTMI_OK; }
@@ -3149,7 +3226,7 @@
 }
 void adopt_materials(rtmi_scene *s, const SceneArrays &a, PackedMaterials *M) {
     rtmi_scene::Args &A = s->args;
-    if (M) { s->uses_perlin = M->uses_perlin; s->max_image = M->max_image; s->mat = std::move(*M); }
+    if (M) { s->uses_perlin = M->uses_perlin; s->max_image = M->max_image; s->dev.defer_mat = M->defer_mat; s->mat = std::move(*M); }
     if (a.prim_mat != A.prim_mat.data()) A.prim_mat.assign(a.prim_mat, a.prim_mat + a.n_prims);
     A.mat_kind.assign(a.mat_kind, a.mat_kind + a.n_mats); A.mat_tex.assign(a.mat_tex, a.mat_tex + a.n_mats); A.mat_param.assign(a.mat_param, a.mat_param + a.n_mats);
     A.tex_kind.assign(a.tex_kind, a.tex_kind + a.n_tex); A.tex_param.assign(a.tex_param, a.tex_param + (size_t)a.n_tex * RTMI_TEX_STRIDE);
@@ -3167,7 +3244,7 @@
     if (prim_mat) a.prim_mat = prim_mat;
     rc = check_material_edit(a);
     if (rc) return rc;
-    M = pack_materials(a);
+    M = pack_materials(a, s->geom_ext);
     return RTMI_OK;
 }
 }
@@ -3266,7 +3343,7 @@
         if (!rc && (n_prims < 0 || (n_prims > 0 && (!prim_kind || !prim_mat)))) rc = fail(RTMI_E_ARG, "primitive arrays are NULL");
         if (!rc) rc = check_material_edit(a);
         if (rc) return rc;
-        M = pack_materials(a);
+        M = pack_materials(a, geometry_is_ext(a));
     }
     uint64_t h = 1469598103934665603ull;
     DevScene none{};
@@ -4622,6 +4699,13 @@
     return RTMI_OK;
 }
 
+RTMI_EXPORT int rtmi_last_record_reals(rtmi_ctx *c, int32_t *reals) {
+    if (!ctx_ok(c)) return fail(RTMI_E_STATE, "invalid context handle");
+    if (!reals) return fail(RTMI_E_ARG, "reals is NULL");
+    *reals = c->last_record_reals;
+    return RTMI_OK;
+}
+
 RTMI_EXPORT int rtmi_last_passes(rtmi_ctx *c, int32_t *passes) {
     if (!ctx_ok(c)) return fail(RTMI_E_STATE, "invalid context handle");
     if (passes) *passes = c->last_passes;
diff --git a/raytrace_clj_amd/csrc/rtmi_device.h b/raytrace_clj_amd/csrc/rtmi_device.h
--- a/raytrace_clj_amd/csrc/rtmi_device.h
+++ b/raytrace_clj_amd/csrc/rtmi_device.h
@@ -68,6 +68,7 @@
     const int *mat_tex;
     const double *mat_param;
     int n_tex;
+    int defer_mat;
     const int *tex_kind;
     const double *tex_param;
     const int *tex_child;
@@ -1752,7 +1753,8 @@
 #define RTMI_PRIM_NEEDS_U 32
 #define RTMI_PRIM_NEEDS_V 64
 #define RTMI_PRIM_NEEDS_UV (RTMI_PRIM_NEEDS_U | RTMI_PRIM_NEEDS_V)
-template <typename R> __device__ inline void resolve_hit(SceneRef sc, const Path<R> &P, R t, int orig, HitRec<R> &h, bool all_uv = true) {
+#define RTMI_PRIM_DEFERRED 128
+template <typename R> __device__ inline void resolve_hit(SceneRef sc, const Path<R> &P, R t, int orig, HitRec<R> &h, bool all_uv = true, bool defer = false) {
     const double *g = sc.exact12 + (size_t)orig * 12;
     R cx = (R)g[0], cy = (R)g[1], cz = (R)g[2];
     h.orig = orig;
@@ -1776,9 +1778,10 @@
     if (h.kind == RTMI_PRIM_UVSPHERE && (all_uv || (kind_flags & RTMI_PRIM_NEEDS_UV))) {
         h.u = h.v = R(0.5);
         if (all_uv || (kind_flags & RTMI_PRIM_NEEDS_U)) h.u = Real<R>::sphere_u(nx, nz);
-        if (all_uv || (kind_flags & RTMI_PRIM_NEEDS_V)) h.v = Real<R>::sphere_v(ny);
+        if (all_uv || ((kind_flags & RTMI_PRIM_NEEDS_V) && !(defer && (kind_flags & RTMI_PRIM_DEFERRED)))) h.v = Real<R>::sphere_v(ny);
         RTMI_PH(PH_UV)
     }
+    if (defer && (kind_flags & RTMI_PRIM_DEFERRED)) h.v = ny;
 }
 
 __device__ inline void leaf_xform_back(int xk, double a, double b, double c, double &px, double &py, double &pz, double &nx, double &nz) {
@@ -1883,10 +1886,41 @@
     }
     h.px = px; h.py = py; h.pz = pz; h.nx = nx; h.ny = ny; h.nz = nz;
 }
-template <typename R, bool EXT> __device__ inline void resolve_any(SceneRef sc, const Path<R> &P, R t, int orig, HitRec<R> &h, bool all_uv = true) { resolve_hit<R>(sc, P, t, orig, h, all_uv); }
-template <> __device__ inline void resolve_any<double, true>(SceneRef sc, const Path<double> &P, double t, int orig, HitRec<double> &h, bool all_uv) { resolve_hit_ext(sc, P, t, orig, h, all_uv); }
-
-template <typename R, bool F4 = false> __device__ inline bool scatter_emit(SceneRef sc, Path<R> &P, const HitRec<R> &h, R *att, R *emit, bool passenger = false) {
+template <typename R, bool EXT> __device__ inline void resolve_any(SceneRef sc, const Path<R> &P, R t, int orig, HitRec<R> &h, bool all_uv = true, bool defer = false) { resolve_hit<R>(sc, P, t, orig, h, all_uv, defer); }
+template <> __device__ inline void resolve_any<double, true>(SceneRef sc, const Path<double> &P, double t, int orig, HitRec<double> &h, bool all_uv, bool) { resolve_hit_ext(sc, P, t, orig, h, all_uv); }
+
+template <typename R> struct GradientU { R a0, a1, a2, b0, b1, b2; };
+template <typename R> __device__ inline GradientU<R> gradient_rec_u(const double *rec, R u) {
+    const double2 *gq = reinterpret_cast<const double2 *>(rec);
+    const double2 g0 = gq[0], g1 = gq[1], g2 = gq[2], g3 = gq[3], g4 = gq[4], g5 = gq[5];
+    const R omu = R(1.0) - u;
+    GradientU<R> q;
+    q.a0 = (R)g1.y * omu + (R)g0.x * u; q.a1 = (R)g2.x * omu + (R)g0.y * u; q.a2 = (R)g2.y * omu + (R)g1.x * u;
+    q.b0 = (R)g4.y * omu + (R)g3.x * u; q.b1 = (R)g5.x * omu + (R)g3.y * u; q.b2 = (R)g5.y * omu + (R)g4.x * u;
+    return q;
+}
+template <typename R> __device__ inline void gradient_rec_v(const GradientU<R> &q, R v, R &tr, R &tg, R &tb) {
+    const R omv = R(1.0) - v;
+    tr = q.b0 * omv + q.a0 * v; tg = q.b1 * omv + q.a1 * v; tb = q.b2 * omv + q.a2 * v;
+}
+
+template <typename R> struct SampleTag;
+template <> struct SampleTag<double> {
+    __device__ static inline double value() { return __longlong_as_double(0x7ff8000052544d49ll); }
+    __device__ static inline bool is(double x) { return __double_as_longlong(x) == 0x7ff8000052544d49ll; }
+};
+template <> struct SampleTag<float> {
+    __device__ static inline float value() { return __uint_as_float(0x7fc0524du); }
+    __device__ static inline bool is(float x) { return __float_as_uint(x) == 0x7fc0524du; }
+};
+template <typename R> __device__ inline void finish_deferred(const GradientU<R> &q, R ny, R &r, R &g, R &b) {
+    R tr, tg, tb;
+    gradient_rec_v(q, Real<R>::sphere_v(ny), tr, tg, tb);
+    r = R(0) + r * tr; g = R(0) + g * tg; b = R(0) + b * tb;
+}
+
+template <typename R, bool F4 = false, bool DEFER = false>
+__device__ inline bool scatter_emit(SceneRef sc, Path<R> &P, const HitRec<R> &h, R *att, R *emit, bool passenger = false, int defer_mat = -1, bool *out_deferred = nullptr) {
     const int mat = h.mat;
     const double2 *mq = reinterpret_cast<const double2 *>(sc.mat_rec + (size_t)mat * 12);
     const double2 m0 = mq[0], m1 = mq[1], m2 = mq[2];
@@ -1954,7 +1988,8 @@
         scat = true;
         RTMI_PH(PH_DIRS)
     }
-    const bool want_tex = is_light || is_lamb || is_iso || (is_metal && scat);
+    const bool deferred = DEFER && is_light && mat == defer_mat;
+    const bool want_tex = (is_light && !deferred) || is_lamb || is_iso || (is_metal && scat);
     double turb = 0.0, turb_p0 = 0.0;
     bool turb_done = false;
     if (F4 && sizeof(R) == sizeof(double)) {
@@ -1982,16 +2017,15 @@
             const bool neg = sx * sy * sz < 0;
             tr = neg ? (R)m1.y : (R)m3.y; tg = neg ? (R)m2.x : (R)m4.x; tb = neg ? (R)m2.y : (R)m4.y;
         } else if (mtk == RTMI_TEX_GRADIENT_REC) {
-            const double2 *gq = reinterpret_cast<const double2 *>(sc.mat_grad + (size_t)mat * 12);
-            const double2 g0 = gq[0], g1 = gq[1], g2 = gq[2], g3 = gq[3], g4 = gq[4], g5 = gq[5];
-            const R u = h.u, v = h.v, omu = R(1.0) - u, omv = R(1.0) - v;
-            const R a0 = (R)g1.y * omu + (R)g0.x * u, a1 = (R)g2.x * omu + (R)g0.y * u, a2 = (R)g2.y * omu + (R)g1.x * u;
-            const R b0 = (R)g4.y * omu + (R)g3.x * u, b1 = (R)g5.x * omu + (R)g3.y * u, b2 = (R)g5.y * omu + (R)g4.x * u;
-            tr = b0 * omv + a0 * v; tg = b1 * omv + a1 * v; tb = b2 * omv + a2 * v;
+            gradient_rec_v(gradient_rec_u<R>(sc.mat_grad + (size_t)mat * 12, h.u), h.v, tr, tg, tb);
         } else tex_sample<R, F4>(sc, mtex, h.u, h.v, px, py, pz, tr, tg, tb);
         if (is_light) { emit[0] = R(0) + P.ar * tr; emit[1] = R(0) + P.ag * tg; emit[2] = R(0) + P.ab * tb; }
         else { atr = tr; atg = tg; atb = tb; }
         RTMI_PH(PH_TEXTURE)
+    }
+    if (DEFER) {
+        *out_deferred = deferred;
+        if (deferred) { emit[0] = P.ar; emit[1] = P.ag; emit[2] = P.ab; }
     }
     if (!scat) return false;
     if (att) { att[0] = atr; att[1] = atg; att[2] = atb; }
@@ -2001,17 +2035,20 @@
     return true;
 }
 
-template <typename R, bool EXT = false>
-__device__ inline bool shade_segment(SceneRef sc, Path<R> &P, R t, int orig, SegLog *lg, R *emit, bool passenger = false) {
+template <typename R, bool EXT = false, bool DEFER = false>
+__device__ inline bool shade_segment(SceneRef sc, Path<R> &P, R t, int orig, SegLog *lg, R *emit, bool passenger = false, int defer_mat = -1, bool *out_deferred = nullptr,
+                                     R *out_ny = nullptr) {
     emit[0] = emit[1] = emit[2] = R(0);
+    if (DEFER) { *out_deferred = false; *out_ny = R(0); }
     if (!passenger && orig < 0) return false;
     HitRec<R> h;
     h.px = h.py = h.pz = h.nx = h.ny = h.nz = h.u = h.v = h.t = R(0); h.mat = 0; h.orig = 0; h.kind = 0;
     if (!passenger) {
-        resolve_any<R, EXT>(sc, P, t, orig, h, false);
+        resolve_any<R, EXT>(sc, P, t, orig, h, false, DEFER);
         RTMI_PH(PH_HITREC)
     }
-    const bool scat = scatter_emit<R, EXT>(sc, P, h, nullptr, emit, passenger);
+    const bool scat = scatter_emit<R, EXT, DEFER>(sc, P, h, nullptr, emit, passenger, defer_mat, out_deferred);
+    if (DEFER) *out_ny = h.v;
     if (lg && lg->n < lg->max_seg) {
         double *q = lg->rec + (size_t)lg->n * RTMI_SEG_REC;
         q[0] = h.orig; q[1] = h.t; q[2] = h.px; q[3] = h.py; q[4] = h.pz; q[5] = h.nx; q[6] = h.ny; q[7] = h.nz;
diff --git a/raytrace_clj_amd/csrc/scene_build.h b/raytrace_clj_amd/csrc/scene_build.h
--- a/raytrace_clj_amd/csrc/scene_build.h
+++ b/raytrace_clj_amd/csrc/scene_build.h
@@ -603,6 +603,7 @@
     bool has_ext = false;
     bool uses_perlin = false;
     int max_image = -1;
+    int defer_mat = -1;
 };
 
 struct PackedScene {
@@ -672,7 +673,15 @@
     t_hi = cam_kind == RTMI_CAM_THINLENS ? std::max(cam[22], cam[23]) : 0.0;
 }
 
-PackedMaterials pack_materials(const SceneArrays &a) {
+inline bool geometry_is_ext(const SceneArrays &a) {
+    for (int i = 0; i < a.n_prims; ++i) {
+        const int kind = a.prim_kind[i] & ~RTMI_PRIM_BOUNDARY;
+        if ((a.prim_kind[i] & RTMI_PRIM_BOUNDARY) || kind > RTMI_PRIM_MOVING || (a.prim_xform && a.prim_xform[2 * i + 1] != 0) || (a.prim_flip && a.prim_flip[i])) return true;
+    }
+    return false;
+}
+
+PackedMaterials pack_materials(const SceneArrays &a, bool geom_ext) {
     PackedMaterials M;
     const int n_prims = a.n_prims;
     for (int t = 0; t < a.n_tex; ++t) {
@@ -699,6 +708,26 @@
     }
     M.prim_km.assign((size_t)std::max(n_prims, 1) * 2, 0);
     for (int i = 0; i < n_prims; ++i) { M.prim_km[2 * (size_t)i] = M.prim_kind[(size_t)i]; M.prim_km[2 * (size_t)i + 1] = M.prim_mat[(size_t)i]; }
+    if (!M.has_ext && !geom_ext) {
+        std::vector<char> on_uv((size_t)std::max(a.n_mats, 1), 0), on_other((size_t)std::max(a.n_mats, 1), 0);
+        for (int i = 0; i < n_prims; ++i) {
+            const int m = M.prim_mat[(size_t)i];
+            if (m < 0 || m >= a.n_mats) continue;
+            ((M.prim_kind[(size_t)i] & 15) == RTMI_PRIM_UVSPHERE ? on_uv : on_other)[(size_t)m] = 1;
+        }
+        int n_cand = 0, cand = -1;
+        for (int m = 0; m < a.n_mats; ++m) {
+            const int t = a.mat_tex[m];
+            if (a.mat_kind[m] != RTMI_MAT_DIFFUSE_LIGHT || t < 0 || t >= a.n_tex || a.tex_kind[t] != RTMI_TEX_UVGRADIENT || uses[(size_t)t] != 2) continue;
+            if (!on_uv[(size_t)m] || on_other[(size_t)m]) continue;
+            ++n_cand; cand = m;
+        }
+        if (n_cand == 1) {
+            M.defer_mat = cand;
+            for (int i = 0; i < n_prims; ++i)
+                if (M.prim_mat[(size_t)i] == cand) M.prim_km[2 * (size_t)i] |= RTMI_PRIM_DEFERRED;
+        }
+    }
     M.mat_rec.assign((size_t)std::max(a.n_mats, 1) * 12, 0.0);
     M.mat_grad.assign((size_t)std::max(a.n_mats, 1) * 12, 0.0);
     for (int m = 0; m < a.n_mats; ++m) {
@@ -932,7 +961,6 @@
     DevScene &d = P.d;
     std::memset(&d, 0, sizeof d);
     const double *cam = a.cam;
-    P.M = pack_materials(a);
     d.n_tex = a.n_tex; d.cam_kind = a.cam_kind;
     std::memcpy(d.cam, cam, 24 * sizeof(double));
     d.cam_fixed_origin = camera_fixed_origin(a.cam_kind, cam);
@@ -940,10 +968,12 @@
     camera_shutter(a.cam_kind, cam, t_lo, t_hi);
     GeomExtras X;
     pack_geometry(a, K.box_leaf, t_lo, t_hi, P, X);
+    P.M = pack_materials(a, P.geom_ext);
     const int n_world = X.n_world;
     const bool has_ext = P.geom_ext || P.M.has_ext;
     build_trees(a, K, has_ext, X, P);
     d.has_ext = has_ext ? 1 : 0;
+    d.defer_mat = has_ext ? -1 : P.M.defer_mat;
     d.small_scan = (has_ext && n_world <= RTMI_SMALL_SCAN_MAX && K.small_scan) ? 1 : 0;
     return P;
 }
```

New measurement: 8194 Msamples/s, median of 6. 3.0% higher.
